# Dhia-naouali/dinov3-jax

Hardware: NVIDIA H100
Metric: global_crops_per_sec (higher is better)
Workload: dtype bf16

## Files before the change

dinov3-jax_b200/csrc/api.cu:

```cuda
#include <algorithm>
#include <atomic>
#include <cstdio>
#include <cstring>
#include "d3_internal.h"

namespace d3 {

static thread_local char g_err[512] = "";
static int g_sm_count = 0;
static std::atomic<long long> g_launches{0};
typedef CUresult (*EncodeTiledFn)(CUtensorMap*, CUtensorMapDataType, cuuint32_t, void*, const cuuint64_t*,
                                  const cuuint64_t*, const cuuint32_t*, const cuuint32_t*, CUtensorMapInterleave,
                                  CUtensorMapSwizzle, CUtensorMapL2promotion, CUtensorMapFloatOOBfill);
static EncodeTiledFn g_encode = nullptr;

int set_error(int code, const char* msg) {
  snprintf(g_err, sizeof(g_err), "%s", msg ? msg : "");
  return code;
}
int sm_count() { return g_sm_count > 0 ? g_sm_count : 132; }
void count_launch(int n) { g_launches.fetch_add(n, std::memory_order_relaxed); }

int encode_tensor_map_2d_bf16(CUtensorMap* map, const void* ptr, const cuuint64_t dims[2],
                              const cuuint64_t strides[1], const cuuint32_t box[2], const cuuint32_t estr[2]) {
// ... 69 lines not shown
    float tot = 0.f;
    for (int k = 0; k < slabs; ++k) tot += ws[k * stride + i];
    dst[r * ld + c] += tot;
  }
}
int slab_combine(const float* ws, int slabs, long long stride, long long rows, int cols, float* dst, long long ld,
                 cudaStream_t st) {
  if (!dst || rows <= 0 || cols <= 0) return D3_OK;
  const long long n = rows * cols;
  const int blocks = (int)std::min<long long>((n + 255) / 256, (long long)sm_count() * 8);
  slab_combine_kernel<<<blocks, 256, 0, st>>>(ws, slabs, stride, rows, cols, dst, ld);
  cudaError_t e = cudaPeekAtLastError();
  if (e != cudaSuccess) return set_error(D3_ERR_CUDA, cudaGetErrorString(e));
  count_launch();
  return D3_OK;
}

}

using namespace d3;

extern "C" {

int d3_abi_version(void) { return 7; }
const char* d3_last_error(void) { return g_err; }
long long d3_launch_count(void) { return g_launches.load(); }
void d3_reset_launch_count(void) { g_launches.store(0); }

int d3_init(int device) {
  cudaError_t e = cudaSetDevice(device);
  if (e != cudaSuccess) return set_error(D3_ERR_CUDA, cudaGetErrorString(e));
  cudaDeviceProp prop;
  e = cudaGetDeviceProperties(&prop, device);
  if (e != cudaSuccess) return set_error(D3_ERR_CUDA, cudaGetErrorString(e));
  if (prop.major != 9 || prop.minor != 0) {
    char buf[128];
    snprintf(buf, sizeof(buf), "device %d is sm_%d%d; this library only has sm_90a code (no fallback)", device,
             prop.major, prop.minor);
    return set_error(D3_ERR_DEVICE, buf);
  }
  g_sm_count = prop.multiProcessorCount;
  {
    cudaMemPool_t pool;
    if (cudaDeviceGetDefaultMemPool(&pool, device) == cudaSuccess) {
      uint64_t keep = UINT64_MAX;
      cudaMemPoolSetAttribute(pool, cudaMemPoolAttrReleaseThreshold, &keep);
    }
  }
  if (!g_encode) {
    void* fn = nullptr;
    cudaDriverEntryPointQueryResult q;
    e = cudaGetDriverEntryPoint("cuTensorMapEncodeTiled", &fn, cudaEnableDefault, &q);
    if (e != cudaSuccess || !fn) return set_error(D3_ERR_CUDA, "cannot resolve cuTensorMapEncodeTiled");
    g_encode = reinterpret_cast<EncodeTiledFn>(fn);
  }
  return D3_OK;
}

static int epilogue_from_abi(const d3_gemm_epilogue* ep, GemmEpilogue& g) {
  if ((ep->flags & D3_EP_ACCUM) && !(ep->flags & D3_EP_OUT_F32)) return set_error(D3_ERR_ARG, "ACCUM needs fp32 out");
  g.bias = ep->bias; g.gamma = ep->gamma; g.resid = ep->resid;
  g.aux_in = reinterpret_cast<const __nv_bfloat16*>(ep->aux_in);
  g.aux_out = reinterpret_cast<__nv_bfloat16*>(ep->aux_out);
  g.out = ep->out; g.ld_out = ep->ld_out; g.ld_aux = ep->ld_aux; g.ld_resid = ep->ld_resid;
  g.flags = ep->flags & 0x3FF; g.alpha = ep->alpha;
  for (int i = 0; i < 8; ++i) g.sc_peer[i] = ep->sc_peer[i];
  g.sc_off = ep->sc_off; g.sc_shard = ep->sc_shard; g.sc_world = ep->sc_world;
  if (g.flags & EP_SCATTER)
    for (int i = 0; i < g.sc_world && i < 8; ++i)
      if (!g.sc_peer[i]) return set_error(D3_ERR_ARG, "scatter flag without peer pointers");
  if ((g.flags & EP_BIAS) && !g.bias) return set_error(D3_ERR_ARG, "bias flag without pointer");
  if ((g.flags & EP_GAMMA) && !g.gamma) return set_error(D3_ERR_ARG, "gamma flag without pointer");
  if ((g.flags & EP_RESID) && !g.resid) return set_error(D3_ERR_ARG, "resid flag without pointer");
  if ((g.flags & EP_STORE_PRE) && !g.aux_out) return set_error(D3_ERR_ARG, "store_pre flag without pointer");
  if ((g.flags & EP_MUL_DGELU) && !g.aux_in) return set_error(D3_ERR_ARG, "mul_dgelu flag without pointer");
  return D3_OK;
}

int d3_gemm_bf16(const void* A, int lda, int a_major, const void* B, int ldb, int b_major, int M, int N, int K,
                 const d3_gemm_epilogue* ep, int tile_n, int split_k, void* stream) {
  if (!A || !B || !ep || !ep->out) return set_error(D3_ERR_ARG, "d3_gemm_bf16: null pointer");
  if (tile_n != 0 && tile_n != 64 && tile_n != 128 && tile_n != 256 && tile_n != 512) return set_error(D3_ERR_ARG, "tile_n");
  if (split_k < 0) return set_error(D3_ERR_ARG, "split_k");
  GemmEpilogue g;
  const int rc = epilogue_from_abi(ep, g);
  if (rc) return rc;
  return gemm_bf16(A, lda, a_major, B, ldb, b_major, M, N, K, g, tile_n, split_k, reinterpret_cast<cudaStream_t>(stream));
}

int d3_gemm_e4m3(const void* A_u8, int lda, const float* sa, const void* B_u8, int ldb, const float* sb, int M, int N,
                 int K, const d3_gemm_epilogue* ep, void* stream) {
  if (!A_u8 || !B_u8 || !sa || !sb || !ep || !ep->out) return set_error(D3_ERR_ARG, "d3_gemm_e4m3: null pointer");
  GemmEpilogue g;
  const int rc = epilogue_from_abi(ep, g);
  if (rc) return rc;
  return gemm_e4m3(A_u8, lda, sa, B_u8, ldb, sb, M, N, K, g, reinterpret_cast<cudaStream_t>(stream));
}

}
```

dinov3-jax_b200/csrc/attention.cu:

```cuda
#include "ptx.cuh"
#include <climits>
#include <cstdlib>
#include "d3_internal.h"

namespace d3 {

constexpr float LOG2E = 1.4426950408889634f;
constexpr int SMEM_ALIGN = 1024;

__device__ __forceinline__ uint8_t* smem_base_1024(uint8_t* raw) {
  return reinterpret_cast<uint8_t*>((reinterpret_cast<uintptr_t>(raw) + 1023) & ~uintptr_t(1023));
}

struct AttnShape {
  int G;
  int span;
  int n_crops;
  int N;
  int nkb;
  int D;
  int H;
  float scale;
  const float* sin_t;
  const float* cos_t;
  int prefix;
};

__device__ __forceinline__ uint32_t sw128_offset(int row, int col) {
  return (uint32_t)(row * 128 + ((((col >> 3) ^ (row & 7)) & 7) << 4) + (col & 7) * 2);
}

struct RowInfo { int g, klo, khi; bool ok; };
__device__ __forceinline__ RowInfo row_info(const AttnShape& sh, int c, int q) {
  RowInfo ri;
  ri.g = min(q / sh.N, sh.G - 1);
  ri.klo = ri.g * sh.N;
  ri.khi = ri.klo + sh.N;
  ri.ok = (q < sh.span) && (c * sh.G + ri.g < sh.n_crops);
  return ri;
}

template <int NI, int NO>
__device__ __forceinline__ void online_softmax(float (&s)[4 * NI], float (&o)[NO], float (&m)[2], float (&l)[2],
                                               const RowInfo (&ri)[2], int k0, int c2, float cs) {
  const int kb0 = k0 + c2;
  const bool full = k0 >= max(ri[0].klo, ri[1].klo) && k0 + 8 * NI <= min(ri[0].khi, ri[1].khi);
  float mx[2] = {-3.0e38f, -3.0e38f};
#pragma unroll
  for (int i = 0; i < NI; ++i)
#pragma unroll
    for (int j = 0; j < 4; ++j) {
      const int hh = j >> 1, kk = kb0 + 8 * i + (j & 1);
      if (full || (kk >= ri[hh].klo && kk < ri[hh].khi)) mx[hh] = fmaxf(mx[hh], s[4 * i + j]);
    }
  float corr[2], ms[2];
#pragma unroll
  for (int hh = 0; hh < 2; ++hh) {
    mx[hh] = fmaxf(mx[hh], __shfl_xor_sync(0xffffffffu, mx[hh], 1));
    mx[hh] = fmaxf(mx[hh], __shfl_xor_sync(0xffffffffu, mx[hh], 2));
    const float mn = fmaxf(m[hh], mx[hh]);
    corr[hh] = ex2_approx((m[hh] - mn) * cs);
    m[hh] = mn;
    ms[hh] = mn * cs;
    l[hh] *= corr[hh];
  }
#pragma unroll
  for (int i = 0; i < NI; ++i)
#pragma unroll
    for (int j = 0; j < 4; ++j) {
      const int hh = j >> 1, kk = kb0 + 8 * i + (j & 1);
      const float p = (full || (kk >= ri[hh].klo && kk < ri[hh].khi)) ? ex2_approx(fmaf(s[4 * i + j], cs, -ms[hh])) : 0.f;
      s[4 * i + j] = p;
      l[hh] += p;
      if (i < NO / 4) o[4 * i + j] *= corr[hh];
    }
}

template <int NO>
__device__ __forceinline__ void store_o_lse(const float (&o)[NO], float (&l)[2], const float (&m)[2], const RowInfo (&ri)[2],
                                            const AttnShape& sh, int c, int h, int row_base, int wq0, int r_in, int c2,
                                            __nv_bfloat16* O, float* LSE) {
#pragma unroll
  for (int hh = 0; hh < 2; ++hh) {
// ... 146 lines not shown
  const FwdRing ring(sQ + 16384);
  uint64_t* bar_q = ring.end();

  const int wg = threadIdx.x >> 7, t = threadIdx.x & 127;
  const int qt = blockIdx.x, h = blockIdx.y, c = blockIdx.z;
  const int q0 = qt * 128, row_base = c * sh.N, nkb = (sh.N + 127) >> 7;
  const int n_wg = (q0 + 64 < sh.N) ? 2 : 1;
  if (threadIdx.x == 0) {
    tma_prefetch_desc(&tmQKV);
    ring.init(4 * n_wg);
    mbar_init(bar_q, 1);
    fence_mbar_init();
  }
  __syncthreads();
  if (ring_producer(wg, [&] {
        mbar_expect_tx(bar_q, 16384);
        tma_load_2d(&tmQKV, bar_q, sQ, h * 64, row_base + q0);
        ring.fill(nkb, [&](uint64_t* bar, uint8_t* dst, int b) {
          tma_load_2d(&tmQKV, bar, dst, sh.D + h * 64, row_base + b * 128);
          tma_load_2d(&tmQKV, bar, dst + 16384, 2 * sh.D + h * 64, row_base + b * 128);
        });
      }))
    return;
  const int wq0 = q0 + wg * 64;
  if (wq0 >= sh.N) return;
  mbar_wait(bar_q, 0);

  const int r_in = 16 * (t >> 5) + ((t & 31) >> 2), c2 = 2 * (t & 3);
  RowInfo ri[2];
  ri[0] = row_info(sh, c, wq0 + r_in);
  ri[1] = row_info(sh, c, wq0 + r_in + 8);
  const float cs = sh.scale * LOG2E;
  float m[2] = {-3.0e38f, -3.0e38f}, l[2] = {0.f, 0.f};
  float o[32];
#pragma unroll
  for (int i = 0; i < 32; ++i) o[i] = 0.f;
  const uint64_t qd = gmma_desc_sw128(smem_u32(sQ + wg * 8192), 16, 1024);

#pragma unroll 1
  for (int b = 0; b < nkb; ++b) {
    const uint8_t* sK = ring.wait(b);
    float s[64];
    const uint64_t kd = gmma_desc_sw128(smem_u32(sK), 16, 1024);
    fence_regs(o);
    wgmma_fence();
#pragma unroll
    for (int k = 0; k < 4; ++k) wgmma_m64n128k16_ss<0, 0>(s, qd + 2 * k, kd + 2 * k, k > 0 ? 1u : 0u);
    wgmma_commit();
    wgmma_wait<0>();
    fence_regs(s);
    online_softmax<16>(s, o, m, l, ri, b * 128, c2, cs);
    uint32_t a[8][4];
#pragma unroll
    for (int kk = 0; kk < 8; ++kk)
#pragma unroll
      for (int e = 0; e < 4; ++e) a[kk][e] = pack_bf16(s[8 * kk + 2 * e], s[8 * kk + 2 * e + 1]);
    const uint64_t vd = gmma_desc_sw128(smem_u32(sK + 16384), 8192, 1024);
    fence_regs(o);
    wgmma_fence();
#pragma unroll
    for (int kk = 0; kk < 8; ++kk) wgmma_m64n64k16_rs<1>(o, a[kk], vd + 128 * kk, 1u);
    wgmma_commit();
    wgmma_wait<0>();
    fence_regs(o);
    ring.release(b);
  }
  store_o_lse(o, l, m, ri, sh, c, h, row_base, wq0, r_in, c2, O, LSE);
}

template <int HD>
__global__ void attn_delta_kernel(const __nv_bfloat16* __restrict__ O, const __nv_bfloat16* __restrict__ dO,
                                  float* __restrict__ delta, long T, int N, int D, int H) {
  constexpr int LANES = HD / 8;
  static_assert(LANES == 8 || LANES == 16, "head_dim 64 or 128");
  const long g = blockIdx.x * (long)blockDim.x + threadIdx.x;
  const int per_row = D >> 3;
  const bool ok = g < T * per_row;
  float s = 0.f;
  long row = 0;
  int c8 = 0;
  if (ok) {
    row = g / per_row;
    c8 = (int)(g % per_row);
    const uint4 a = *reinterpret_cast<const uint4*>(O + row * D + c8 * 8);
    const uint4 b = *reinterpret_cast<const uint4*>(dO + row * D + c8 * 8);
    const float2 a0 = unpack_bf16(a.x), a1 = unpack_bf16(a.y), a2 = unpack_bf16(a.z), a3 = unpack_bf16(a.w);
    const float2 b0 = unpack_bf16(b.x), b1 = unpack_bf16(b.y), b2 = unpack_bf16(b.z), b3 = unpack_bf16(b.w);
    s = a0.x * b0.x + a0.y * b0.y + a1.x * b1.x + a1.y * b1.y + a2.x * b2.x + a2.y * b2.y + a3.x * b3.x + a3.y * b3.y;
  }
  if (LANES == 16) s += __shfl_xor_sync(0xffffffffu, s, 8);
  s += __shfl_xor_sync(0xffffffffu, s, 4);
  s += __shfl_xor_sync(0xffffffffu, s, 2);
  s += __shfl_xor_sync(0xffffffffu, s, 1);
  if (ok && (c8 & (LANES - 1)) == 0) delta[((row / N) * H + (c8 >> (LANES == 16 ? 4 : 3))) * N + (row % N)] = s;
}

template <int NA>
__device__ __forceinline__ void store_grad_rows(float (&a)[NA], const AttnShape& sh, int c, int row_base, int tile_row0,
                                                int r_in, int c2, int h, int third, bool rope, __nv_bfloat16* dQKV) {
  constexpr int HD = 2 * NA;
#pragma unroll
  for (int hh = 0; hh < 2; ++hh) {
    const int row = tile_row0 + r_in + 8 * hh;
    const RowInfo ri = row_info(sh, c, row);
    if (!ri.ok) continue;
    const int tok = row - ri.klo;
    float v[NA / 2];
#pragma unroll
    for (int i = 0; i < NA / 4; ++i) { v[2 * i] = a[4 * i + 2 * hh]; v[2 * i + 1] = a[4 * i + 2 * hh + 1]; }
    if (rope && sh.sin_t && tok >= sh.prefix) {
      const float* sn = sh.sin_t + (size_t)(tok - sh.prefix) * HD;
      const float* cn = sh.cos_t + (size_t)(tok - sh.prefix) * HD;
#pragma unroll
      for (int i = 0; i < NA / 8; ++i)
#pragma unroll
        for (int j = 0; j < 2; ++j) {
          const int d = 8 * i + c2 + j;
          const float lo = v[2 * i + j], hi = v[2 * (i + NA / 8) + j];
          v[2 * i + j] = lo * cn[d] + hi * sn[d];
          v[2 * (i + NA / 8) + j] = hi * cn[d] - lo * sn[d];
        }
    }
    __nv_bfloat16* dst = dQKV + (size_t)(row_base + row) * (3 * sh.D) + third * sh.D + h * HD + c2;
#pragma unroll
    for (int i = 0; i < NA / 4; ++i) *reinterpret_cast<uint32_t*>(dst + 8 * i) = pack_bf16(v[2 * i], v[2 * i + 1]);
  }
}

__device__ __forceinline__ void row_stats(const AttnShape& sh, const float* __restrict__ LSE, const float* __restrict__ Delta,
                                          int c, int h, int q, float& lse2, float& dl) {
  const RowInfo ri = row_info(sh, c, q);
  const size_t stat = ((size_t)(c * sh.G + ri.g) * sh.H + h) * sh.N + (ri.ok ? q - ri.klo : 0);
  lse2 = ri.ok ? LSE[stat] * LOG2E : 0.f;
  dl = ri.ok ? Delta[stat] : 0.f;
}

__device__ __forceinline__ void p_ds_tile(const AttnShape& sh, const float* __restrict__ LSE, const float* __restrict__ Delta,
                                          int c, int h, int q0, int kt, const uint8_t* sQw, const uint8_t* sDOw,
                                          const uint8_t* sK, const uint8_t* sV, int r_in, int c2, float (&s)[64],
                                          float (&dp)[64]) {
  const float cs = sh.scale * LOG2E;
  const uint64_t qd = gmma_desc_sw128(smem_u32(sQw), 16, 1024);
  const uint64_t dod = gmma_desc_sw128(smem_u32(sDOw), 16, 1024);
  const uint64_t kd = gmma_desc_sw128(smem_u32(sK), 16, 1024);
  const uint64_t vd = gmma_desc_sw128(smem_u32(sV), 16, 1024);
  wgmma_fence();
#pragma unroll
  for (int k = 0; k < 4; ++k) {
    wgmma_m64n128k16_ss<0, 0>(s, qd + 2 * k, kd + 2 * k, k > 0 ? 1u : 0u);
    wgmma_m64n128k16_ss<0, 0>(dp, dod + 2 * k, vd + 2 * k, k > 0 ? 1u : 0u);
  }
  wgmma_commit();
  wgmma_wait<0>();
  fence_regs(s);
  fence_regs(dp);
#pragma unroll
  for (int hh = 0; hh < 2; ++hh) {
    const int q = q0 + r_in + 8 * hh;
    const RowInfo ri = row_info(sh, c, q);
    float lse2, dl;
    row_stats(sh, LSE, Delta, c, h, q, lse2, dl);
    const int lo = ri.ok ? ri.klo - kt * 128 : 0, hi = ri.ok ? ri.khi - kt * 128 : 0;
#pragma unroll
    for (int i = 0; i < 16; ++i)
#pragma unroll
      for (int j = 0; j < 2; ++j) {
        const int e = 4 * i + 2 * hh + j, col = 8 * i + c2 + j;
        const bool ok = col >= lo && col < hi;
        const float p = ok ? ex2_approx(fmaf(s[e], cs, -lse2)) : 0.f;
        dp[e] = ok ? (p * sh.scale) * (dp[e] - dl) : 0.f;
        s[e] = p;
      }
  }
}

__device__ __forceinline__ void stash_p_ds(const float (&s)[64], const float (&dp)[64], uint8_t* sP, uint8_t* sDS, int row,
// ... 641 lines not shown
      wgmma_fence();
#pragma unroll
      for (int kk = 0; kk < 4; ++kk) wgmma_m64n128k16_rs<1>(dq, da[kk], kd + 128 * kk, 1u);
      wgmma_commit();
      wgmma_wait<0>();
      fence_regs(dq);
      fence_frag(da);
    }
    ring.release(kt);
  }
  store_grad_rows(dq, sh, c, row_base, wq0, r_in, c2, h, 0, true, dQKV);
}

static int make_map(CUtensorMap* map, const void* ptr, long rows, int cols, int ld, int box_rows) {
  cuuint64_t dims[2] = {(cuuint64_t)cols, (cuuint64_t)rows};
  cuuint64_t strides[1] = {(cuuint64_t)ld * 2};
  cuuint32_t box[2] = {64, (cuuint32_t)box_rows};
  cuuint32_t estr[2] = {1, 1};
  return encode_tensor_map_2d_bf16(map, ptr, dims, strides, box, estr);
}

constexpr int ATTN_MAX_TOKENS = 32768;
constexpr int ATTN_FWD_RESIDENT_SPAN = 448;
constexpr int ATTN_BWD_RESIDENT_SPAN = 256;

static int attn_shape(AttnShape* s, int n_crops, int N, int D, int H) {
  if (D != H * 64 && D != H * 128) return set_error(D3_ERR_ARG, "attention: head_dim must be 64 or 128");
  if (N <= 0 || n_crops <= 0) return set_error(D3_ERR_ARG, "attention: empty problem");
  if (N > ATTN_MAX_TOKENS) return set_error(D3_ERR_ARG, "attention: N > 32768 tokens per crop");
  if ((long)n_crops * N > INT_MAX) return set_error(D3_ERR_ARG, "attention: n_crops * N must be below 2^31 token rows");
  s->N = N; s->D = D; s->H = H; s->n_crops = n_crops;
  s->scale = (D == H * 64) ? 0.125f : 0.08838834764831845f;
  s->sin_t = nullptr; s->cos_t = nullptr; s->prefix = 0;
  s->G = (N <= 64) ? (128 / N) : 1;
  if (s->G > n_crops) s->G = n_crops;
  s->span = s->G * N;
  s->nkb = (s->span + 63) / 64;
  return D3_OK;
}

static int tile_grid(const AttnShape& s, dim3* grid) {
  const int groups = (s.n_crops + s.G - 1) / s.G;
  if (s.H > 65535 || groups > 65535) return set_error(D3_ERR_ARG, "attention: H and crop groups must be <= 65535");
  *grid = dim3((s.span + 127) / 128, s.H, groups);
  return D3_OK;
}

template <auto kernel, class... Args>
static int launch(dim3 grid, int threads, int smem, int smem_max, cudaStream_t st, const Args&... args) {
  static const cudaError_t cfg = cudaFuncSetAttribute(kernel, cudaFuncAttributeMaxDynamicSharedMemorySize, smem_max);
  (void)cfg;
  kernel<<<grid, threads, smem, st>>>(args...);
  D3_CHECK_LAUNCH();
  return D3_OK;
}

}

using namespace d3;

extern "C" {

int d3_attn_fwd(const void* qkv, void* o, float* lse, int n_crops, int N, int D, int H, void* stream) {
  AttnShape s;
  int rc = attn_shape(&s, n_crops, N, D, H);
  if (rc) return rc;
  dim3 grid;
  if ((rc = tile_grid(s, &grid))) return rc;
  const long T = (long)n_crops * N;
  cudaStream_t st = reinterpret_cast<cudaStream_t>(stream);
  __nv_bfloat16* out = (__nv_bfloat16*)o;
  CUtensorMap tqkv;
  if ((rc = make_map(&tqkv, qkv, T, 3 * D, 3 * D, 128))) return rc;
  if (D == H * 128)
    return launch<attn_fwd_hd128_kernel>(grid, RING_THREADS, HD128_FWD_SMEM, HD128_FWD_SMEM, st, tqkv, out, lse, s);
  if (s.span > ATTN_FWD_RESIDENT_SPAN)
    return launch<attn_fwd_stream_kernel>(grid, RING_THREADS, FWD_STREAM_SMEM, FWD_STREAM_SMEM, st, tqkv, out, lse, s);
  CUtensorMap tkv;
  if ((rc = make_map(&tkv, qkv, T, 3 * D, 3 * D, 64))) return rc;
  return launch<attn_fwd_kernel>(grid, 256, fwd_smem(s.nkb), fwd_smem((ATTN_FWD_RESIDENT_SPAN + 63) / 64), st, tqkv, tkv,
                                 out, lse, s);
}

int d3_attn_bwd(const void* qkv, const void* o, const void* d_o, const float* lse, float* delta_scratch, void* dqkv,
                int n_crops, int N, int D, int H, const float* rope_sin, const float* rope_cos, int rope_prefix,
                void* stream) {
  AttnShape s;
  int rc = attn_shape(&s, n_crops, N, D, H);
  if (rc) return rc;
  if ((rope_sin == nullptr) != (rope_cos == nullptr)) return set_error(D3_ERR_ARG, "d3_attn_bwd: sin/cos tables");
  if (!delta_scratch) return set_error(D3_ERR_ARG, "d3_attn_bwd: delta scratch buffer");
  const bool hd128 = D == H * 128;
  const bool streamed = s.span > ATTN_BWD_RESIDENT_SPAN;
  dim3 grid;
  if ((hd128 || streamed) && (rc = tile_grid(s, &grid))) return rc;
  s.sin_t = rope_sin; s.cos_t = rope_cos; s.prefix = rope_prefix;
  const long T = (long)n_crops * N;
  cudaStream_t st = reinterpret_cast<cudaStream_t>(stream);
  const long threads = T * (D / 8);
  if (hd128)
    attn_delta_kernel<128><<<(int)((threads + 255) / 256), 256, 0, st>>>((const __nv_bfloat16*)o, (const __nv_bfloat16*)d_o,
                                                                       delta_scratch, T, N, D, H);
  else
    attn_delta_kernel<64><<<(int)((threads + 255) / 256), 256, 0, st>>>((const __nv_bfloat16*)o, (const __nv_bfloat16*)d_o,
                                                                      delta_scratch, T, N, D, H);
  D3_CHECK_LAUNCH();
  CUtensorMap tqkv, tdo;
  if ((rc = make_map(&tqkv, qkv, T, 3 * D, 3 * D, 128))) return rc;
  if ((rc = make_map(&tdo, d_o, T, D, D, 128))) return rc;
  __nv_bfloat16* dq = (__nv_bfloat16*)dqkv;
  if (hd128) {
    if ((rc = launch<attn_bwd_dkdv_hd128_kernel>(grid, RING_THREADS, HD128_BWD_SMEM, HD128_BWD_SMEM, st, tqkv, tdo, lse,
                                                 delta_scratch, dq, s)))
      return rc;
    return launch<attn_bwd_dq_hd128_kernel>(grid, RING_THREADS, HD128_BWD_SMEM, HD128_BWD_SMEM, st, tqkv, tdo, lse,
                                            delta_scratch, dq, s);
  }
  if (streamed) {
    if ((rc = launch<attn_bwd_dkdv_kernel>(grid, RING_THREADS, DKDV_SMEM, DKDV_SMEM, st, tqkv, tdo, lse, delta_scratch, dq,
                                           s)))
      return rc;
    return launch<attn_bwd_dq_kernel>(grid, RING_THREADS, DQ_SMEM, DQ_SMEM, st, tqkv, tdo, lse, delta_scratch, dq, s);
  }
  return launch<attn_bwd_fused_kernel>(dim3(H, (n_crops + s.G - 1) / s.G), 256, bwd_fused_smem((s.span + 127) / 128),
                                       bwd_fused_smem(ATTN_BWD_RESIDENT_SPAN / 128), st, tqkv, tdo, lse, delta_scratch,
                                       dq, s);
}

}
```

dinov3-jax_b200/csrc/d3_internal.h:

```cpp
#pragma once
#include <cuda.h>
#include <cuda_runtime.h>
#include <cuda_bf16.h>
#include <stdint.h>
#include "../../include/dinov3_b200.h"

namespace d3 {

enum : int {
  EP_BIAS = D3_EP_BIAS,
  EP_GELU = D3_EP_GELU,
  EP_STORE_PRE = D3_EP_STORE_PRE,
  EP_MUL_DGELU = D3_EP_MUL_DGELU,
  EP_GAMMA = D3_EP_GAMMA,
  EP_RESID = D3_EP_RESID,
  EP_OUT_F32 = D3_EP_OUT_F32,
  EP_ACCUM = D3_EP_ACCUM,
  EP_SCATTER = D3_EP_SCATTER,
  EP_GELU_ERF = D3_EP_GELU_ERF,
  EP_SLOW = 1 << 30,
  EP_SLABS = 1 << 27,
};

struct GemmEpilogue {
  const float* bias;
  const float* gamma;
  const float* resid;
  const __nv_bfloat16* aux_in;
  __nv_bfloat16* aux_out;
  void* out;
  int ld_out, ld_aux, ld_resid;
  int flags;
  float alpha;
  float* sc_peer[8];
  long long sc_off;
  int sc_shard, sc_world;
};

int set_error(int code, const char* msg);
int sm_count();
void count_launch(int n = 1);
int encode_tensor_map_2d_bf16(CUtensorMap* map, const void* ptr, const cuuint64_t dims[2],
                              const cuuint64_t strides[1], const cuuint32_t box[2], const cuuint32_t estr[2]);
int encode_tensor_map_2d(CUtensorMap* map, const void* ptr, int elt_bytes, cuuint64_t cols, cuuint64_t rows,
                         cuuint64_t row_stride_bytes, cuuint32_t box_cols, cuuint32_t box_rows, int swizzle_bytes);
int encode_tensor_map_2d_u8(CUtensorMap* map, const void* ptr, cuuint64_t cols, cuuint64_t rows, cuuint64_t ld_bytes,
                            cuuint32_t box_cols, cuuint32_t box_rows);

float* slab_workspace(size_t floats, cudaStream_t st);
void slab_release(float* ws, cudaStream_t st);
int slab_combine(const float* ws, int slabs, long long stride, long long rows, int cols, float* dst, long long ld,
                 cudaStream_t st);

int gemm_bf16(const void* A, int lda, int a_mn, const void* B, int ldb, int b_mn, int M, int N, int K,
              GemmEpilogue ep, int tile_n, int split_k, cudaStream_t stream);
int gemm_e4m3(const void* A, int lda, const float* sa, const void* B, int ldb, const float* sb, int M, int N, int K,
              GemmEpilogue ep, cudaStream_t stream);

#define D3_CHECK_LAUNCH()                                               \
  do {                                                                  \
    cudaError_t e__ = cudaPeekAtLastError();                            \
    if (e__ != cudaSuccess) return d3::set_error(D3_ERR_CUDA, cudaGetErrorString(e__)); \
    d3::count_launch();                                                 \
  } while (0)

}
```

dinov3-jax_b200/csrc/elementwise.cu:

```cuda
#include "ptx.cuh"
#include "d3_internal.h"
#include "layernorm.cuh"

namespace d3 {

__global__ void im2col_kernel(const __nv_bfloat16* __restrict__ img, __nv_bfloat16* __restrict__ out, int n, int H,
                              int W, int p, int ld) {
  const int Hp = H / p, Wp = W / p;
  const int rowlen = p * 3;
  const long total = (long)n * Hp * Wp * p;
  for (long w = blockIdx.x * (long)blockDim.x / 32 + threadIdx.x / 32; w < total; w += (long)gridDim.x * blockDim.x / 32) {
    const int a = (int)(w % p);
    long r = w / p;
    const int j = (int)(r % Wp);
    const int i = (int)((r / Wp) % Hp);
    const long c = r / ((long)Wp * Hp);
    const __nv_bfloat16* src = img + ((c * H + (long)i * p + a) * W + (long)j * p) * 3;
    __nv_bfloat16* dst = out + r * (long)ld + (long)a * rowlen;
    for (int e = threadIdx.x & 31; e < rowlen; e += 32) dst[e] = src[e];
    if (a == p - 1)
      for (int e = p * rowlen + (threadIdx.x & 31); e < ld; e += 32) out[r * (long)ld + e] = __float2bfloat16(0.f);
  }
}

__global__ void assemble_tokens_kernel(const float* __restrict__ tok, const float* __restrict__ cls,
                                       const float* __restrict__ storage, const float* __restrict__ mask_token,
                                       const uint8_t* __restrict__ masks, float* __restrict__ X, int n, int P, int R,
                                       int D) {
  const int N = P + 1 + R;
  const long rows = (long)n * N;
  const int D4 = D / 4;
  for (long r = blockIdx.x; r < rows; r += gridDim.x) {
    const long c = r / N;
    const int t = (int)(r % N);
    const float4* src;
    if (t == 0) src = reinterpret_cast<const float4*>(cls);
    else if (t <= R) src = reinterpret_cast<const float4*>(storage + (long)(t - 1) * D);
    else if (masks && masks[c * P + (t - 1 - R)]) src = reinterpret_cast<const float4*>(mask_token);
    else src = reinterpret_cast<const float4*>(tok + (c * P + (t - 1 - R)) * (long)D);
    float4* dst = reinterpret_cast<float4*>(X + r * (long)D);
    for (int e = threadIdx.x; e < D4; e += blockDim.x) dst[e] = src[e];
  }
}
__global__ void assemble_tokens_bwd_kernel(const float* __restrict__ dX, const uint8_t* __restrict__ masks,
                                           __nv_bfloat16* __restrict__ dTok, float* __restrict__ ws, int n, int P, int R,
                                           int D) {
  const int col = blockIdx.x * blockDim.x + threadIdx.x;
  const int N = P + 1 + R;
  const long slab = ((long)n + gridDim.y - 1) / gridDim.y;
  const long c0 = blockIdx.y * slab, c1 = min((long)n, c0 + slab);
  if (col >= D) return;
  float acc_cls = 0.f, acc_mask = 0.f;
  float* slab_ws = ws + (long)blockIdx.y * (2 + R) * D;
  for (int t = 1; t <= R; ++t) {
    float acc = 0.f;
    for (long c = c0; c < c1; ++c) acc += dX[c * N * (long)D + (long)t * D + col];
    slab_ws[(long)(1 + t) * D + col] = acc;
  }
  for (long c = c0; c < c1; ++c) {
    const float* row = dX + c * N * (long)D + col;
    acc_cls += row[0];
    for (int t = 0; t < P; ++t) {
      const float g = row[(long)(1 + R + t) * D];
      const bool m = masks && masks[c * P + t];
      if (m) acc_mask += g;
      dTok[(c * P + t) * (long)D + col] = __float2bfloat16(m ? 0.f : g);
    }
  }
  slab_ws[col] = acc_cls;
  slab_ws[D + col] = acc_mask;
}


template <int VPL, typename OutT>
__global__ void __launch_bounds__(256)
layernorm_fwd_kernel(const float* __restrict__ x, const float* __restrict__ scale, const float* __restrict__ bias,
                     OutT* __restrict__ y, float* __restrict__ mean_out, float* __restrict__ rstd_out, int T, float eps,
                     int width) {
  const int D = VPL > 0 ? VPL * 128 : width;
  const int warps = blockDim.x >> 5, lane = threadIdx.x & 31;
  for (long row = (long)blockIdx.x * warps + (threadIdx.x >> 5); row < T; row += (long)gridDim.x * warps) {
    const float4* xr = reinterpret_cast<const float4*>(x + row * (long)D);
    float4 v[VPL > 0 ? VPL : 1];
// ... 397 lines not shown
  }

  float* slab = reinterpret_cast<float*>(ring);
  const int ct = threadIdx.x;
#define LNR_REDUCE(ACC, DST, Q)                                                                      \
  {                                                                                                  \
    float* dst__ = (DST);                                                                            \
    asm volatile("bar.sync 1, %0;" ::"n"(32 * LNR_CONSUMERS) : "memory");                           \
    if (dst__) {                                                                                     \
      _Pragma("unroll") for (int c = 0; c < VPL; ++c)                                                \
        *reinterpret_cast<float4*>(slab + warp * D + (c * 32 + lane) * 4) =                          \
            make_float4(ACC[c][0], ACC[c][1], ACC[c][2], ACC[c][3]);                                 \
    }                                                                                                \
    asm volatile("bar.sync 1, %0;" ::"n"(32 * LNR_CONSUMERS) : "memory");                           \
    if (dst__) {                                                                                     \
      for (int e = ct; e < D; e += 32 * LNR_CONSUMERS) {                                             \
        float tot = 0.f;                                                                             \
        _Pragma("unroll") for (int w = 0; w < LNR_CONSUMERS; ++w) tot += slab[w * D + e];            \
        ws[((long)blockIdx.x * 4 + (Q)) * D + e] = tot;                                              \
      }                                                                                              \
    }                                                                                                \
  }
  LNR_REDUCE(ads, dscale, 0)
  LNR_REDUCE(adb, dscale ? dbias : nullptr, 1)
  LNR_REDUCE(tdg, (tail && uB) ? ls_dgamma : nullptr, 2)
  LNR_REDUCE(tdb, tail ? ls_dbias : nullptr, 3)
#undef LNR_REDUCE
}

__global__ void ls_gamma_from_wgrad_kernel(const __nv_bfloat16* __restrict__ W, const float* __restrict__ dW,
                                           const float* __restrict__ bias, const float* __restrict__ dbias,
                                           const float* __restrict__ gamma, float* __restrict__ ws, int K, int N) {
  __shared__ float acc[8][64];
  const int lane = threadIdx.x & 31, wy = threadIdx.x >> 5;
  const int col = blockIdx.x * 64 + lane * 2;
  const int slab = (K + gridDim.y - 1) / gridDim.y;
  const int r0 = blockIdx.y * slab, r1 = min(K, r0 + slab);
  float s0 = 0.f, s1 = 0.f;
  if (col < N) {
    for (int i = r0 + wy; i < r1; i += 8) {
      const float2 w = unpack_bf16(*reinterpret_cast<const uint32_t*>(W + (long)i * N + col));
      const float2 g = *reinterpret_cast<const float2*>(dW + (long)i * N + col);
      s0 += w.x * g.x; s1 += w.y * g.y;
    }
  }
  acc[wy][lane * 2] = s0; acc[wy][lane * 2 + 1] = s1;
  __syncthreads();
  if (threadIdx.x < 64) {
    const int c = blockIdx.x * 64 + threadIdx.x;
    if (c < N) {
      float tot = 0.f;
#pragma unroll
      for (int k = 0; k < 8; ++k) tot += acc[k][threadIdx.x];
      if (blockIdx.y == 0) tot += bias[c] * dbias[c];
      const float g = gamma[c];
      if (g != 0.f) ws[(long)blockIdx.y * N + c] = tot / g;
    }
  }
}

__global__ void rope_kernel(__nv_bfloat16* __restrict__ qkv, const float* __restrict__ sin_t,
                            const float* __restrict__ cos_t, long T, int Ntok, int prefix, int D, int hd, int inverse) {
  const int half = hd / 2;
  const int groups = half / 8;
  const int H = D / hd;
  const int items_per_row = 2 * H * groups;
  const long total = T * (long)items_per_row;
  for (long w = blockIdx.x * (long)blockDim.x + threadIdx.x; w < total; w += (long)gridDim.x * blockDim.x) {
    const long row = w / items_per_row;
    int r = (int)(w % items_per_row);
    const int t = (int)(row % Ntok);
    if (t < prefix) continue;
    const int which = r / (H * groups);
    r -= which * H * groups;
    const int head = r / groups, i0 = (r % groups) * 8;
    const float* sp = sin_t + (long)(t - prefix) * hd + i0;
    const float* cp = cos_t + (long)(t - prefix) * hd + i0;
    float sn[8], cs[8];
    *reinterpret_cast<float4*>(sn) = *reinterpret_cast<const float4*>(sp);
    *reinterpret_cast<float4*>(sn + 4) = *reinterpret_cast<const float4*>(sp + 4);
    *reinterpret_cast<float4*>(cs) = *reinterpret_cast<const float4*>(cp);
    *reinterpret_cast<float4*>(cs + 4) = *reinterpret_cast<const float4*>(cp + 4);
    __nv_bfloat16* base = qkv + row * (long)(3 * D) + which * D + head * hd + i0;
    const uint4 lo = *reinterpret_cast<const uint4*>(base);
    const uint4 hi = *reinterpret_cast<const uint4*>(base + half);
    const uint32_t lw[4] = {lo.x, lo.y, lo.z, lo.w}, hw[4] = {hi.x, hi.y, hi.z, hi.w};
    uint32_t ol[4], oh[4];
#pragma unroll
    for (int j = 0; j < 4; ++j) {
      const float2 a = unpack_bf16(lw[j]), b = unpack_bf16(hw[j]);
      float y1a, y1b, y2a, y2b;
      if (!inverse) {
        y1a = a.x * cs[2 * j] - b.x * sn[2 * j];          y2a = b.x * cs[2 * j] + a.x * sn[2 * j];
        y1b = a.y * cs[2 * j + 1] - b.y * sn[2 * j + 1];  y2b = b.y * cs[2 * j + 1] + a.y * sn[2 * j + 1];
      } else {
        y1a = a.x * cs[2 * j] + b.x * sn[2 * j];          y2a = b.x * cs[2 * j] - a.x * sn[2 * j];
        y1b = a.y * cs[2 * j + 1] + b.y * sn[2 * j + 1];  y2b = b.y * cs[2 * j + 1] - a.y * sn[2 * j + 1];
      }
      ol[j] = pack_bf16(y1a, y1b);
      oh[j] = pack_bf16(y2a, y2b);
    }
    *reinterpret_cast<uint4*>(base) = make_uint4(ol[0], ol[1], ol[2], ol[3]);
    *reinterpret_cast<uint4*>(base + half) = make_uint4(oh[0], oh[1], oh[2], oh[3]);
  }
}

__global__ void token_rows_kernel(const long long* __restrict__ idx, int* __restrict__ rows, int count, int P, int prefix,
                                  int mode) {
  const int i = blockIdx.x * blockDim.x + threadIdx.x;
  if (i >= count) return;
  if (mode == 0) {
    const long long m = idx[i];
    rows[i] = (int)(m / P * (P + prefix) + prefix + m % P);
  } else {
    rows[i] = i * (P + prefix);
  }
}
__global__ void gather_rows_kernel(const float* __restrict__ src, const int* __restrict__ rows,
                                   __nv_bfloat16* __restrict__ dst_bf16, float* __restrict__ dst_f32, int R, int D) {
  for (int r = blockIdx.x; r < R; r += gridDim.x) {
    const float* s = src + (long)rows[r] * D;
    for (int e = threadIdx.x; e < D; e += blockDim.x) {
      const float v = s[e];
      if (dst_bf16) dst_bf16[(long)r * D + e] = __float2bfloat16(v);
      if (dst_f32) dst_f32[(long)r * D + e] = v;
    }
  }
}
template <typename InT>
__global__ void scatter_add_rows_kernel(const InT* __restrict__ src, const int* __restrict__ rows,
                                        float* __restrict__ dst, int R, int D) {
  for (int r = blockIdx.x; r < R; r += gridDim.x) {
    float* d = dst + (long)rows[r] * D;
    for (int e = threadIdx.x; e < D; e += blockDim.x) {
      float v;
      if constexpr (sizeof(InT) == 2) v = __bfloat162float(src[(long)r * D + e]); else v = src[(long)r * D + e];
      d[e] += v;
    }
  }
}

__global__ void l2norm_fwd_kernel(const float* __restrict__ u, __nv_bfloat16* __restrict__ y, float* __restrict__ nrm,
                                  int R, int C, float eps) {
  const int warps = blockDim.x >> 5, lane = threadIdx.x & 31;
  for (long row = (long)blockIdx.x * warps + (threadIdx.x >> 5); row < R; row += (long)gridDim.x * warps) {
    const float* ur = u + row * C;
    float s = 0.f;
    for (int e = lane; e < C; e += 32) s += ur[e] * ur[e];
    s = warp_sum(s);
    const float n = sqrtf(s);
    const float inv = 1.f / (n + eps);
    if (lane == 0) nrm[row] = n;
    for (int e = lane; e < C; e += 32) y[row * C + e] = __float2bfloat16(ur[e] * inv);
  }
}
__global__ void l2norm_bwd_kernel(const __nv_bfloat16* __restrict__ g, const float* __restrict__ u,
                                  const float* __restrict__ nrm, __nv_bfloat16* __restrict__ du, int R, int C, float eps) {
  const int warps = blockDim.x >> 5, lane = threadIdx.x & 31;
  for (long row = (long)blockIdx.x * warps + (threadIdx.x >> 5); row < R; row += (long)gridDim.x * warps) {
    const float* ur = u + row * C;
    const __nv_bfloat16* gr = g + row * C;
    float dot = 0.f;
    for (int e = lane; e < C; e += 32) dot += ur[e] * __bfloat162float(gr[e]);
    dot = warp_sum(dot);
    const float n = nrm[row];
    const float inv = 1.f / (n + eps);
    const float coef = (n > 0.f) ? dot * inv * inv / n : 0.f;
    for (int e = lane; e < C; e += 32)
      du[row * C + e] = __float2bfloat16(__bfloat162float(gr[e]) * inv - ur[e] * coef);
  }
}

__global__ void ls_act_bwd_kernel(const float* __restrict__ dX, const __nv_bfloat16* __restrict__ u,
                                  const float* __restrict__ gamma, __nv_bfloat16* __restrict__ du,
                                  float* __restrict__ ws, int T, int D, int use_gelu) {
  const int col = (blockIdx.x * blockDim.x + threadIdx.x) * 4;
  const long slab = ((long)T + gridDim.y - 1) / gridDim.y;
  const long r0 = blockIdx.y * slab, r1 = min((long)T, r0 + slab);
  if (col >= D) return;
  float gm[4], ag[4] = {0.f, 0.f, 0.f, 0.f}, ab[4] = {0.f, 0.f, 0.f, 0.f};
  load4(gamma + col, gm);
  for (long r = r0; r < r1; ++r) {
    float o[4];
    load4(dX + r * D + col, o);
    *reinterpret_cast<uint2*>(du + r * D + col) = ls_tail4(o, gm, true, u + r * D + col, use_gelu, ag, ab);
  }
// ... 606 lines not shown
```

dinov3-jax_b200/csrc/gemm_tc.cu:

```cuda
#include <cstdlib>
#include <cstring>
#include "ptx.cuh"
#include "d3_internal.h"

namespace d3 {

constexpr int BM = 128;
constexpr int BK = 64;
constexpr int GEMM_THREADS = 384;

constexpr int EPI_RUNTIME = -1;
constexpr int EPI_FLAGS = EP_BIAS | EP_GELU | EP_STORE_PRE | EP_MUL_DGELU | EP_GAMMA | EP_RESID | EP_OUT_F32 | EP_ACCUM |
                          EP_SLABS | EP_GELU_ERF;

template <int EF>
constexpr bool kStaged = EF != EPI_RUNTIME && (EF & (EP_SLABS | EP_ACCUM)) == 0;

template <int EF>
__device__ __forceinline__ bool epi_has(const GemmEpilogue& ep, int f) {
  return EF == EPI_RUNTIME ? (ep.flags & f) != 0 : (EF & f) != 0;
}

__device__ __forceinline__ float gelu_grad_epi(float u) {
  const float u2 = __fmul_rn(u, u);
  const float t = tanh_approx(__fmul_rn(u, fmaf(0.0356774081363001f, u2, 0.7978845608028654f)));
  const float dz = fmaf(0.1070322244089003f, u2, 0.7978845608028654f);
  return fmaf(__fmul_rn(__fmul_rn(0.5f, u), fmaf(-t, t, 1.0f)), dz, __fmul_rn(0.5f, __fadd_rn(1.0f, t)));
}

__device__ __forceinline__ float gelu_erf_epi(float u) {
  return __fmul_rn(__fmul_rn(0.5f, u), __fadd_rn(1.0f, erff(__fmul_rn(u, 0.70710678118654752f))));
}

template <int EF>
__device__ __forceinline__ float epi_value(const GemmEpilogue& ep, float acc, float bias, float u, float gamma,
                                           float resid, float old, float& pre) {
  float v = __fmul_rn(acc, ep.alpha);
  if (epi_has<EF>(ep, EP_BIAS)) v = __fadd_rn(v, bias);
  pre = v;
  if (epi_has<EF>(ep, EP_GELU)) v = gelu_tanh_fast(v);
  if (epi_has<EF>(ep, EP_GELU_ERF)) v = gelu_erf_epi(v);
  if (epi_has<EF>(ep, EP_MUL_DGELU)) v = __fmul_rn(v, gelu_grad_epi(u));
  if (epi_has<EF>(ep, EP_GAMMA)) v = __fmul_rn(v, gamma);
  if (epi_has<EF>(ep, EP_RESID)) v = __fadd_rn(v, resid);
  if (epi_has<EF>(ep, EP_ACCUM)) v = __fadd_rn(v, old);
  return v;
}

__device__ __forceinline__ float2 ld_pair(const float* p, bool vec, bool two) {
  if (vec) return *reinterpret_cast<const float2*>(p);
  return make_float2(p[0], two ? p[1] : 0.f);
}
__device__ __forceinline__ float2 ld_pair(const __nv_bfloat16* p, bool vec, bool two) {
  if (vec) return unpack_bf16(*reinterpret_cast<const uint32_t*>(p));
  return make_float2(__bfloat162float(p[0]), two ? __bfloat162float(p[1]) : 0.f);
}
__device__ __forceinline__ void st_pair(float* p, float a, float b, bool vec, bool two) {
  if (vec) {
    *reinterpret_cast<float2*>(p) = make_float2(a, b);
  } else {
    p[0] = a;
    if (two) p[1] = b;
  }
}
__device__ __forceinline__ void st_pair(__nv_bfloat16* p, float a, float b, bool vec, bool two) {
  if (vec) {
    *reinterpret_cast<uint32_t*>(p) = pack_bf16(a, b);
  } else {
    p[0] = __float2bfloat16(a);
    if (two) p[1] = __float2bfloat16(b);
  }
}

template <int BN>
__device__ __forceinline__ void epilogue_tile_runtime(const GemmEpilogue& ep, float (&acc)[2][BN / 2], int m0, int n0,
                                                      int M, int N, size_t slab_row0, int r_in, int c_in) {
  float* const out_f = reinterpret_cast<float*>(ep.out);
  __nv_bfloat16* const out_h = reinterpret_cast<__nv_bfloat16*>(ep.out);
  const bool aligned = (ep.flags & EP_SLOW) == 0;
#pragma unroll
  for (int mh = 0; mh < 2; ++mh)
#pragma unroll
    for (int h = 0; h < 2; ++h) {
      const size_t row = (size_t)(m0 + mh * 64 + r_in + 8 * h);
      if (row >= (size_t)M) continue;
      const size_t orow = slab_row0 + row;
#pragma unroll
      for (int i = 0; i < BN / 8; ++i) {
        const int n = n0 + 8 * i + c_in;
        if (n >= N) break;
        const bool two = n + 1 < N, vec = aligned && two;
        float2 b{}, u{}, g{}, x{}, o{};
        if (epi_has<EPI_RUNTIME>(ep, EP_BIAS)) b = ld_pair(ep.bias + n, vec, two);
        if (epi_has<EPI_RUNTIME>(ep, EP_MUL_DGELU)) u = ld_pair(ep.aux_in + row * ep.ld_aux + n, vec, two);
        if (epi_has<EPI_RUNTIME>(ep, EP_GAMMA)) g = ld_pair(ep.gamma + n, vec, two);
        if (epi_has<EPI_RUNTIME>(ep, EP_RESID)) x = ld_pair(ep.resid + row * ep.ld_resid + n, vec, two);
        if (epi_has<EPI_RUNTIME>(ep, EP_ACCUM)) o = ld_pair(out_f + orow * ep.ld_out + n, vec, two);
        float p0, p1;
        const float v0 = epi_value<EPI_RUNTIME>(ep, acc[mh][4 * i + 2 * h], b.x, u.x, g.x, x.x, o.x, p0);
        const float v1 = epi_value<EPI_RUNTIME>(ep, acc[mh][4 * i + 2 * h + 1], b.y, u.y, g.y, x.y, o.y, p1);
        if (epi_has<EPI_RUNTIME>(ep, EP_SCATTER)) {
          const unsigned long long g_idx = (unsigned long long)ep.sc_off + orow * ep.ld_out + n;
          const unsigned long long shard = (unsigned long long)ep.sc_shard;
          const unsigned r = (unsigned)(g_idx / shard);
          float* const dst = ep.sc_peer[r] + (g_idx - r * shard);
          if (!two) atomicAdd(dst, v0);
          else atomicAdd(reinterpret_cast<float2*>(dst), make_float2(v0, v1));
          continue;
        }
        if (epi_has<EPI_RUNTIME>(ep, EP_STORE_PRE)) st_pair(ep.aux_out + row * ep.ld_aux + n, p0, p1, vec, two);
        if (epi_has<EPI_RUNTIME>(ep, EP_OUT_F32)) st_pair(out_f + orow * ep.ld_out + n, v0, v1, vec, two);
        else st_pair(out_h + orow * ep.ld_out + n, v0, v1, vec, two);
      }
    }
}

constexpr int STG_BOX = 64 * 128;
constexpr int STG_BYTES = 3 * STG_BOX;
__device__ __forceinline__ uint32_t sw128(int r, int byte) {
  return r * 128 + ((((byte >> 4) ^ r) & 7) << 4) + (byte & 15);
}

template <int MH, int BN, int EF>
__device__ __forceinline__ void epilogue_tile(const GemmEpilogue& ep, const CUtensorMap* tm_out,
                                              const CUtensorMap* tm_pre, float (&acc)[MH][BN / 2], const float* s_bias,
                                              const float* s_gamma, uint8_t* stg, int& seq, int bar, int t, int m0,
                                              int n0, int M, int N, size_t slab_row0, int r_in, int c_in) {
  constexpr bool STAGED = kStaged<EF>;
  constexpr bool F32 = (EF & EP_OUT_F32) != 0;
  constexpr int OUT_BOXES = F32 ? 2 : 1;
  constexpr int CHUNK = (OUT_BOXES + ((EF & EP_STORE_PRE) ? 1 : 0)) * STG_BOX;
  constexpr int NBUF = STG_BYTES / CHUNK;
  static_assert(NBUF >= 1, "a chunk must fit the staging area");
  float* const out_f = reinterpret_cast<float*>(ep.out);
  __nv_bfloat16* const out_h = reinterpret_cast<__nv_bfloat16*>(ep.out);
#pragma unroll
  for (int mh = 0; mh < MH; ++mh)
#pragma unroll
    for (int cb = 0; cb < BN / 64; ++cb) {
      const int row0 = m0 + mh * 64, col0 = n0 + cb * 64;
      if (row0 >= M || col0 >= N) continue;
      float2 xr[2][8], xo[2][8];
      uint32_t xu[2][8];
#pragma unroll
      for (int h = 0; h < 2; ++h) {
        const size_t row = (size_t)row0 + r_in + 8 * h;
#pragma unroll
        for (int i = 0; i < 8; ++i) {
          const int n = col0 + 8 * i + c_in;
          if (row < (size_t)M && n < N) {
            if (epi_has<EF>(ep, EP_RESID))
              xr[h][i] = *reinterpret_cast<const float2*>(ep.resid + row * ep.ld_resid + n);
            if (epi_has<EF>(ep, EP_MUL_DGELU))
              xu[h][i] = *reinterpret_cast<const uint32_t*>(ep.aux_in + row * ep.ld_aux + n);
            if (epi_has<EF>(ep, EP_ACCUM))
              xo[h][i] = *reinterpret_cast<const float2*>(out_f + (slab_row0 + row) * ep.ld_out + n);
          }
        }
      }
      uint8_t* const buf = stg + (seq % NBUF) * CHUNK;
      if constexpr (STAGED) {
        if (t == 0) tma_store_wait_read<NBUF - 1>();
        named_bar_sync(bar, 128);
      }
#pragma unroll
      for (int h = 0; h < 2; ++h) {
        const int r = r_in + 8 * h;
        const size_t row = (size_t)row0 + r;
#pragma unroll
        for (int i = 0; i < 8; ++i) {
          const int cl = cb * 64 + 8 * i + c_in;
          const int n = n0 + cl;
          const float2 b = epi_has<EF>(ep, EP_BIAS) ? *reinterpret_cast<const float2*>(s_bias + cl) : float2{};
          const float2 g = epi_has<EF>(ep, EP_GAMMA) ? *reinterpret_cast<const float2*>(s_gamma + cl) : float2{};
          const float2 u = epi_has<EF>(ep, EP_MUL_DGELU) ? unpack_bf16(xu[h][i]) : float2{};
          float p0, p1;
          const float v0 = epi_value<EF>(ep, acc[mh][4 * (cl >> 3) + 2 * h], b.x, u.x, g.x, xr[h][i].x, xo[h][i].x, p0);
          const float v1 = epi_value<EF>(ep, acc[mh][4 * (cl >> 3) + 2 * h + 1], b.y, u.y, g.y, xr[h][i].y, xo[h][i].y,
                                         p1);
          if constexpr (STAGED) {
            if (epi_has<EF>(ep, EP_STORE_PRE))
              *reinterpret_cast<uint32_t*>(buf + OUT_BOXES * STG_BOX + sw128(r, 16 * i + 2 * c_in)) = pack_bf16(p0, p1);
            if constexpr (F32) {
              *reinterpret_cast<float2*>(buf + (i >> 2) * STG_BOX + sw128(r, 32 * (i & 3) + 4 * c_in)) =
                  make_float2(v0, v1);
            } else {
              *reinterpret_cast<uint32_t*>(buf + sw128(r, 16 * i + 2 * c_in)) = pack_bf16(v0, v1);
            }
          } else if (row < (size_t)M && n < N) {
            if (epi_has<EF>(ep, EP_STORE_PRE)) st_pair(ep.aux_out + row * ep.ld_aux + n, p0, p1, true, true);
            if constexpr (F32) st_pair(out_f + (slab_row0 + row) * ep.ld_out + n, v0, v1, true, true);
            else st_pair(out_h + (slab_row0 + row) * ep.ld_out + n, v0, v1, true, true);
          }
        }
      }
      if constexpr (STAGED) {
        fence_proxy_async_smem();
        named_bar_sync(bar, 128);
        if (t == 0) {
          tma_store_2d(tm_out, buf, col0, row0);
          if (F32 && col0 + 32 < N) tma_store_2d(tm_out, buf + STG_BOX, col0 + 32, row0);
          if constexpr ((EF & EP_STORE_PRE) != 0) tma_store_2d(tm_pre, buf + OUT_BOXES * STG_BOX, col0, row0);
          tma_store_commit();
        }
        ++seq;
      }
    }
}

template <int BN, bool STAGED>
struct Cfg {
  static constexpr bool WIDE = BN == 256;
  static constexpr int STAGES = (BN == 256 ? 4 : BN == 128 ? 6 : 8) - (STAGED ? 1 : 0);
  static constexpr int A_BYTES = BM * BK * 2;
  static constexpr int B_BYTES = BN * BK * 2;
  static constexpr int STAGE_BYTES = A_BYTES + B_BYTES;
  static constexpr int BAR_BYTES = 256;
  static constexpr int VEC_BYTES = (WIDE ? 1 : 2) * 2 * BN * 4;
  static constexpr int VEC_END = STAGES * STAGE_BYTES + BAR_BYTES + VEC_BYTES;
  static constexpr int STG_OFF = (VEC_END + 1023) / 1024 * 1024;
  static constexpr int SMEM_BYTES = (STAGED ? STG_OFF + 2 * STG_BYTES : VEC_END) + 1024;
  static_assert(SMEM_BYTES <= 227 * 1024, "over the opt-in shared-memory limit");
};

struct WorkRange { int m0, n0, kb0, kb1, sp; };
template <int BN>
__device__ __forceinline__ WorkRange work_item(int w, int rank, int num_n, int num_tiles, int num_k, int splits) {
  const int tile = w % num_tiles, sp = w / num_tiles;
  const int per = (num_k + splits - 1) / splits;
  WorkRange r;
  if constexpr (BN == 256) {
    r.n0 = (tile % num_n) * BN;
    r.m0 = (2 * (tile / num_n) + rank) * BM;
  } else {
    r.n0 = (2 * (tile % num_n) + rank) * BN;
    r.m0 = (tile / num_n) * BM;
  }
  r.kb0 = sp * per;
  r.kb1 = min(num_k, r.kb0 + per);
  r.sp = sp;
  return r;
}

template <int MH, int BN, int A_MN, int B_MN>
__device__ __forceinline__ void mma_kblock(float (&acc)[MH][BN / 2], uint32_t sa, uint32_t sb, bool first) {
  const uint64_t bd = B_MN ? gmma_desc_sw128(sb, 8192, 1024) : gmma_desc_sw128(sb, 16, 1024);
  constexpr uint64_t a_adv = A_MN ? (2048 >> 4) : (32 >> 4);
  constexpr uint64_t b_adv = B_MN ? (2048 >> 4) : (32 >> 4);
#pragma unroll
  for (int k = 0; k < BK / 16; ++k) {
    const uint32_t sc = (first && k == 0) ? 0u : 1u;
#pragma unroll
    for (int mh = 0; mh < MH; ++mh) {
      const uint64_t ad = A_MN ? gmma_desc_sw128(sa + mh * 8192, 8192, 1024) : gmma_desc_sw128(sa + mh * 8192, 16, 1024);
      if constexpr (BN == 256) wgmma_m64n256k16_ss<A_MN, B_MN>(acc[mh], ad + k * a_adv, bd + k * b_adv, sc);
      else if constexpr (BN == 128) wgmma_m64n128k16_ss<A_MN, B_MN>(acc[mh], ad + k * a_adv, bd + k * b_adv, sc);
      else wgmma_m64n64k16_ss<A_MN, B_MN>(acc[mh], ad + k * a_adv, bd + k * b_adv, sc);
    }
  }
}

template <int MH, int BN>
__device__ __forceinline__ void mma_khalf_e4m3(float (&acc)[MH][BN / 2], uint32_t sa, uint32_t sb, int h) {
  static_assert(BN == 64, "the e4m3 GEMM runs 128 x 64 tiles");
  const uint64_t bd = gmma_desc_sw128(sb, 16, 1024);
#pragma unroll
  for (int k = 0; k < 2; ++k) {
#pragma unroll
    for (int mh = 0; mh < MH; ++mh) {
      const uint64_t ad = gmma_desc_sw128(sa + mh * 8192, 16, 1024);
      wgmma_m64n64k32_e4m3(acc[mh], ad + (2 * h + k) * (32 >> 4), bd + (2 * h + k) * (32 >> 4), k == 0 ? 0u : 1u);
    }
  }
}

template <int MH, int BN>
__device__ __forceinline__ void add_acc(float (&acc)[MH][BN / 2], const float (&part)[MH][BN / 2]) {
#pragma unroll
  for (int mh = 0; mh < MH; ++mh)
#pragma unroll
    for (int i = 0; i < BN / 2; ++i) acc[mh][i] = __fadd_rn(acc[mh][i], part[mh][i]);
}

template <int BN, int A_MN, int B_MN, int EF, bool E4M3 = false>
__global__ void __launch_bounds__(GEMM_THREADS, 1)
gemm_kernel(const __grid_constant__ CUtensorMap tmA, const __grid_constant__ CUtensorMap tmB,
            const __grid_constant__ CUtensorMap tmO, const __grid_constant__ CUtensorMap tmP, const GemmEpilogue ep,
            int M, int N, int K, int splits, const float* scale_a, const float* scale_b) {
  static_assert(!E4M3 || (BN == 64 && !A_MN && !B_MN), "e4m3: 128 x 64 tiles, both operands K-major");
  constexpr int KB = E4M3 ? 128 : BK;
// ... 25 lines not shown
  cluster_sync();

  const int num_m = (M + BM - 1) / BM;
  const int num_n = WIDE ? (N + BN - 1) / BN : ((N + BN - 1) / BN + 1) / 2;
  const int num_k = (K + KB - 1) / KB;
  const int num_tiles = (WIDE ? (num_m + 1) / 2 : num_m) * num_n;
  const int num_work = num_tiles * splits;

  if (wg == 0) {
    setmaxnreg_dec<40>();
    if (threadIdx.x < 32 && elect_one()) {
      int stage = 0;
      uint32_t phase = 0;
      for (int w = cluster; w < num_work; w += num_clusters) {
        const WorkRange wr = work_item<BN>(w, rank, num_n, num_tiles, num_k, splits);
        for (int kb = wr.kb0; kb < wr.kb1; ++kb) {
          mbar_wait(&empty_bar[stage], phase ^ 1);
          uint8_t* sa = smem + stage * C::STAGE_BYTES;
          uint8_t* sb = sa + C::A_BYTES;
          mbar_expect_tx(&full_bar[stage], C::STAGE_BYTES);
          if constexpr (WIDE) {
#pragma unroll
            for (int i = 0; i < 2; ++i) {
              if (A_MN) tma_load_2d(&tmA, &full_bar[stage], sa + i * 8192, wr.m0 + i * 64, kb * KB);
              else tma_load_2d(&tmA, &full_bar[stage], sa + i * 8192, kb * KB, wr.m0 + i * 64);
            }
            if (B_MN) {
#pragma unroll
              for (int i = 2 * rank; i < 2 * rank + 2; ++i)
                tma_load_2d_multicast(&tmB, &full_bar[stage], sb + i * 8192, wr.n0 + i * 64, kb * KB, 0b11);
            } else {
              tma_load_2d_multicast(&tmB, &full_bar[stage], sb + rank * 16384, kb * KB, wr.n0 + rank * 128, 0b11);
            }
          } else {
            if (A_MN) {
              tma_load_2d_multicast(&tmA, &full_bar[stage], sa + rank * 8192, wr.m0 + rank * 64, kb * KB, 0b11);
            } else {
              tma_load_2d_multicast(&tmA, &full_bar[stage], sa + rank * 8192, kb * KB, wr.m0 + rank * 64, 0b11);
            }
            if (B_MN) {
#pragma unroll
              for (int i = 0; i < BN / 64; ++i) tma_load_2d(&tmB, &full_bar[stage], sb + i * 8192, wr.n0 + i * 64, kb * KB);
            } else {
              tma_load_2d(&tmB, &full_bar[stage], sb, kb * KB, wr.n0);
            }
          }
          if (++stage == C::STAGES) { stage = 0; phase ^= 1; }
        }
      }
    }
  } else {
    setmaxnreg_inc<232>();
    const int cw = wg - 1;
    const int t = threadIdx.x & 127;
    const int r_in = 16 * (t >> 5) + ((t & 31) >> 2);
    const int c_in = 2 * (t & 3);
    float* const s_bias = vecs + (WIDE ? 0 : cw * 2 * BN);
    float* const s_gamma = s_bias + BN;
    constexpr bool stage_vecs = EF != EPI_RUNTIME && (EF & (EP_BIAS | EP_GAMMA)) != 0;
    constexpr int VEC_THREADS = WIDE ? 256 : 128;
    const int vt = WIDE ? threadIdx.x - 128 : t;
    uint8_t* const stg = smem + C::STG_OFF + cw * STG_BYTES;
    const uint32_t peer_empty = mapa_shared(smem_u32(empty_bar), rank ^ 1);
    int stg_seq = 0;
    int stage = 0;
    uint32_t phase = 0;
    int j = 0;
    for (int w = cluster; w < num_work; w += num_clusters, ++j) {
      const WorkRange wr = work_item<BN>(w, rank, num_n, num_tiles, num_k, splits);
      const int nkb = wr.kb1 > wr.kb0 ? wr.kb1 - wr.kb0 : 0;
      if (!WIDE && (j & 1) != cw) {
        stage += nkb;
        phase ^= (stage / C::STAGES) & 1;
        stage %= C::STAGES;
        continue;
      }
      if constexpr (stage_vecs) {
        named_bar_sync(3 + cw * !WIDE, VEC_THREADS);
        if (vt < BN && wr.n0 + vt < N) {
          if constexpr ((EF & EP_BIAS) != 0) cp_async_4(s_bias + vt, ep.bias + wr.n0 + vt);
          if constexpr ((EF & EP_GAMMA) != 0) cp_async_4(s_gamma + vt, ep.gamma + wr.n0 + vt);
        }
      }
      if (!WIDE && j > 0) named_bar_sync(1 + cw, 256);
      float acc[MH][BN / 2];
#pragma unroll
      for (int mh = 0; mh < MH; ++mh)
#pragma unroll
        for (int i = 0; i < BN / 2; ++i) acc[mh][i] = 0.f;
      if constexpr (E4M3) {
        float part[MH][BN / 2];
        for (int kb = wr.kb0; kb < wr.kb1; ++kb) {
          mbar_wait(&full_bar[stage], phase);
          const uint32_t sa = smem_u32(smem + stage * C::STAGE_BYTES);
#pragma unroll
          for (int h = 0; h < 2; ++h) {
#pragma unroll
            for (int mh = 0; mh < MH; ++mh) fence_regs(part[mh]);
            wgmma_fence();
            mma_khalf_e4m3<MH, BN>(part, sa, sa + C::A_BYTES, h);
            wgmma_commit();
            wgmma_wait<0>();
#pragma unroll
            for (int mh = 0; mh < MH; ++mh) fence_regs(part[mh]);
            if (h == 1 && t == 0) { mbar_arrive(&empty_bar[stage]); mbar_arrive_cluster(peer_empty + 8 * stage); }
            add_acc<MH, BN>(acc, part);
          }
          if (++stage == C::STAGES) { stage = 0; phase ^= 1; }
        }
        if (!WIDE && w + num_clusters < num_work) named_bar_arrive(1 + (cw ^ 1), 256);
#pragma unroll
        for (int mh = 0; mh < MH; ++mh)
#pragma unroll
          for (int h = 0; h < 2; ++h) {
            const int row = wr.m0 + mh * 64 + r_in + 8 * h;
            const float s_row = row < M ? scale_a[row] : 0.f;
#pragma unroll
            for (int i = 0; i < BN / 8; ++i) {
              const int n = wr.n0 + 8 * i + c_in;
              const float s0 = n < N ? scale_b[n] : 0.f, s1 = n + 1 < N ? scale_b[n + 1] : 0.f;
              acc[mh][4 * i + 2 * h] = __fmul_rn(__fmul_rn(acc[mh][4 * i + 2 * h], s_row), s0);
              acc[mh][4 * i + 2 * h + 1] = __fmul_rn(__fmul_rn(acc[mh][4 * i + 2 * h + 1], s_row), s1);
            }
          }
      } else {
        int prev = -1;
        for (int kb = wr.kb0; kb < wr.kb1; ++kb) {
          mbar_wait(&full_bar[stage], phase);
          const uint32_t sa = smem_u32(smem + stage * C::STAGE_BYTES);
#pragma unroll
          for (int mh = 0; mh < MH; ++mh) fence_regs(acc[mh]);
          wgmma_fence();
          mma_kblock<MH, BN, A_MN, B_MN>(acc, sa + (WIDE ? cw * 8192 : 0), sa + C::A_BYTES, kb == wr.kb0);
          wgmma_commit();
#pragma unroll
          for (int mh = 0; mh < MH; ++mh) fence_regs(acc[mh]);
          if (prev >= 0) {
            wgmma_wait<1>();
            if (t == 0) { mbar_arrive(&empty_bar[prev]); mbar_arrive_cluster(peer_empty + 8 * prev); }
          }
          prev = stage;
          if (++stage == C::STAGES) { stage = 0; phase ^= 1; }
        }
        if (!WIDE && w + num_clusters < num_work) named_bar_arrive(1 + (cw ^ 1), 256);
        wgmma_wait<0>();
#pragma unroll
        for (int mh = 0; mh < MH; ++mh) fence_regs(acc[mh]);
        if (prev >= 0 && t == 0) { mbar_arrive(&empty_bar[prev]); mbar_arrive_cluster(peer_empty + 8 * prev); }
      }
      if constexpr (stage_vecs) {
        cp_async_wait_all();
        named_bar_sync(3 + cw * !WIDE, VEC_THREADS);
      }
      if (nkb <= 0) continue;
      const size_t slab_row0 = epi_has<EF>(ep, EP_SLABS) ? (size_t)wr.sp * M : 0;
      if constexpr (EF == EPI_RUNTIME) {
        epilogue_tile_runtime<BN>(ep, acc, wr.m0, wr.n0, M, N, slab_row0, r_in, c_in);
      } else {
        epilogue_tile<MH, BN, EF>(ep, &tmO, &tmP, acc, s_bias, s_gamma, stg, stg_seq, 5 + cw, t,
                                  wr.m0 + (WIDE ? cw * 64 : 0), wr.n0, M, N, slab_row0, r_in, c_in);
      }
    }
    if (staged && t == 0) tma_store_wait_all();
  }
  cluster_sync();
}

static int make_operand_map(CUtensorMap* map, const void* ptr, int mn, int k, int ld, int is_mn_major, int box_mn) {
  cuuint64_t dims[2], strides[1];
  cuuint32_t box[2], estr[2] = {1, 1};
  if (is_mn_major) {
    dims[0] = (cuuint64_t)mn; dims[1] = (cuuint64_t)k; box[0] = 64; box[1] = 64;
  } else {
    dims[0] = (cuuint64_t)k; dims[1] = (cuuint64_t)mn; box[0] = 64; box[1] = (cuuint32_t)box_mn;
  }
  strides[0] = (cuuint64_t)ld * 2;
  return encode_tensor_map_2d_bf16(map, ptr, dims, strides, box, estr);
}

template <int BN, int A_MN, int B_MN, int EF, bool E4M3 = false>
static int launch(const CUtensorMap& ta, const CUtensorMap& tb, const GemmEpilogue& ep, int M, int N, int K,
                  int splits, cudaStream_t stream, const float* scale_a = nullptr, const float* scale_b = nullptr) {
  using C = Cfg<BN, kStaged<EF>>;
  auto kern = gemm_kernel<BN, A_MN, B_MN, EF, E4M3>;
  cudaLaunchAttribute attr{};
  attr.id = cudaLaunchAttributeClusterDimension;
  attr.val.clusterDim.x = 2;
  attr.val.clusterDim.y = 1;
  attr.val.clusterDim.z = 1;
  cudaLaunchConfig_t cfg{};
  cfg.blockDim = dim3(GEMM_THREADS);
  cfg.dynamicSmemBytes = C::SMEM_BYTES;
  cfg.stream = stream;
  cfg.attrs = &attr;
  cfg.numAttrs = 1;
  static int max_clusters = 0;
  if (max_clusters == 0) {
    cudaError_t e = cudaFuncSetAttribute(kern, cudaFuncAttributeMaxDynamicSharedMemorySize, C::SMEM_BYTES);
    if (e != cudaSuccess) return set_error(D3_ERR_CUDA, cudaGetErrorString(e));
    cfg.gridDim = dim3(2 * sm_count());
    e = cudaOccupancyMaxActiveClusters(&max_clusters, kern, &cfg);
    if (e != cudaSuccess) return set_error(D3_ERR_CUDA, cudaGetErrorString(e));
    if (max_clusters < 1) return set_error(D3_ERR_CUDA, "gemm: no 2-CTA cluster fits on the device");
  }
  CUtensorMap to{}, tp{};
  if constexpr (kStaged<EF>) {
    const int elt = (EF & EP_OUT_F32) ? 4 : 2;
    int rc = encode_tensor_map_2d(&to, ep.out, elt, N, M, (cuuint64_t)ep.ld_out * elt, 128 / elt, 64, 128);
    if (rc) return rc;
    if constexpr ((EF & EP_STORE_PRE) != 0) {
      rc = encode_tensor_map_2d(&tp, ep.aux_out, 2, N, M, (cuuint64_t)ep.ld_aux * 2, 64, 64, 128);
      if (rc) return rc;
    }
  }
  const int num_m = (M + BM - 1) / BM, num_n = (N + BN - 1) / BN;
  const int work = (BN == 256 ? (num_m + 1) / 2 * num_n : num_m * ((num_n + 1) / 2)) * splits;
  cfg.gridDim = dim3(2 * (work < max_clusters ? work : max_clusters));
  cudaError_t e = cudaLaunchKernelEx(&cfg, kern, ta, tb, to, tp, ep, M, N, K, splits, scale_a, scale_b);
  if (e == cudaSuccess) e = cudaPeekAtLastError();
  if (e != cudaSuccess) return set_error(D3_ERR_CUDA, cudaGetErrorString(e));
  count_launch();
  return D3_OK;
}

template <int BN>
static int dispatch(int a_mn, int b_mn, const CUtensorMap& ta, const CUtensorMap& tb, const GemmEpilogue& ep, int M,
                    int N, int K, int splits, cudaStream_t s) {
  if (!(ep.flags & (EP_SLOW | EP_SCATTER)) && N % 2 == 0) {
    const int f = ep.flags & EPI_FLAGS;
#define D3_EPI(A, B, F) \
    if (a_mn == A && b_mn == B && f == (F)) return launch<BN, A, B, (F)>(ta, tb, ep, M, N, K, splits, s);
    D3_EPI(0, 1, 0)
    D3_EPI(0, 1, EP_BIAS)
    D3_EPI(0, 1, EP_BIAS | EP_OUT_F32)
    D3_EPI(0, 1, EP_BIAS | EP_GELU)
    D3_EPI(0, 1, EP_BIAS | EP_GELU | EP_STORE_PRE)
    D3_EPI(0, 1, EP_BIAS | EP_GAMMA | EP_RESID | EP_OUT_F32)
    D3_EPI(0, 1, EP_BIAS | EP_STORE_PRE | EP_GAMMA | EP_RESID | EP_OUT_F32)
    D3_EPI(0, 1, EP_BIAS | EP_GELU | EP_GAMMA | EP_RESID | EP_OUT_F32)
    D3_EPI(0, 1, EP_BIAS | EP_GELU | EP_STORE_PRE | EP_GAMMA | EP_RESID | EP_OUT_F32)
    D3_EPI(0, 1, EP_OUT_F32)
    D3_EPI(0, 1, EP_BIAS | EP_GELU_ERF)
    D3_EPI(0, 0, 0)
    D3_EPI(0, 0, EP_MUL_DGELU)
    D3_EPI(0, 0, EP_OUT_F32)
    D3_EPI(1, 1, EP_OUT_F32 | EP_SLABS)
    D3_EPI(1, 1, EP_OUT_F32 | EP_ACCUM)
#undef D3_EPI
  }
  if constexpr (BN == 256) {
    return dispatch<128>(a_mn, b_mn, ta, tb, ep, M, N, K, splits, s);
  } else {
    if (!a_mn && !b_mn) return launch<BN, 0, 0, EPI_RUNTIME>(ta, tb, ep, M, N, K, splits, s);
    if (!a_mn && b_mn) return launch<BN, 0, 1, EPI_RUNTIME>(ta, tb, ep, M, N, K, splits, s);
    if (a_mn && !b_mn) return launch<BN, 1, 0, EPI_RUNTIME>(ta, tb, ep, M, N, K, splits, s);
    return launch<BN, 1, 1, EPI_RUNTIME>(ta, tb, ep, M, N, K, splits, s);
  }
}

int gemm_bf16(const void* A, int lda, int a_mn, const void* B, int ldb, int b_mn, int M, int N, int K,
              GemmEpilogue ep, int tile_n, int split_k, cudaStream_t stream) {
  if (M <= 0 || N <= 0 || K <= 0) return set_error(D3_ERR_ARG, "gemm: empty problem");
  if ((lda % 8) || (ldb % 8) || (reinterpret_cast<uintptr_t>(A) & 15) || (reinterpret_cast<uintptr_t>(B) & 15))
    return set_error(D3_ERR_ARG, "gemm: operands must be 16-byte aligned with ld % 8 == 0");
  const int sms = sm_count();
  const int num_k = (K + BK - 1) / BK;
  int bn = tile_n >= 256 ? 256 : tile_n;
  if (tile_n == 0) {
    const int cand[2] = {128, 64};
    long best = -1;
    for (int i = 0; i < 2; ++i) {
      const long tiles = (long)((M + BM - 1) / BM) * ((N + cand[i] - 1) / cand[i]);
      const long waves = (tiles + sms - 1) / sms;
      const long cost = waves * (cand[i] + 24);
      if (best < 0 || cost < best) { best = cost; bn = cand[i]; }
    }
  }
  const bool plain_f32 = (ep.flags & EP_OUT_F32) && !(ep.flags & (EP_BIAS | EP_GELU | EP_STORE_PRE | EP_MUL_DGELU |
                                                                  EP_GAMMA | EP_RESID | EP_GELU_ERF));
  int splits = 1;
  if (split_k >= 1) {
    splits = split_k;
  } else if (plain_f32 && (ep.flags & EP_ACCUM)) {
    const int unit_n = bn < 128 ? bn : 128;
    const long units = (long)((M + BM - 1) / BM) * ((N + unit_n - 1) / unit_n);
    if (units <= sms && num_k >= 16) {
      splits = units * 2 <= sms ? (int)(sms / units) : 1;
      if (splits < (num_k + 63) / 64) splits = (num_k + 63) / 64;
      if (splits > num_k / 4) splits = num_k / 4;
      if (splits < 1) splits = 1;
    }
  }
  if (tile_n == 0 && a_mn && b_mn) bn = 256;
  if (ep.flags & EP_SCATTER) {
    if (!plain_f32) return set_error(D3_ERR_ARG, "gemm: SCATTER needs a plain fp32 output");
    if (ep.sc_world < 1 || ep.sc_world > 8 || ep.sc_shard <= 0 || (ep.sc_shard % 4) || (ep.sc_off % 4) || (ep.ld_out % 4))
      return set_error(D3_ERR_ARG, "gemm: SCATTER needs 1..8 ranks and 4-element aligned shard / offset / ld_out");
    if ((unsigned long long)ep.sc_off + (unsigned long long)(M - 1) * ep.ld_out + N > (unsigned long long)ep.sc_shard * ep.sc_world)
      return set_error(D3_ERR_ARG, "gemm: SCATTER output exceeds the sharded range");
  }
  if (splits > 1) {
    if (!plain_f32) return set_error(D3_ERR_ARG, "gemm: split-K needs a plain fp32 output");
    if (!(ep.flags & EP_ACCUM)) return set_error(D3_ERR_ARG, "gemm: split-K accumulates into out (set ACCUM, zero it first)");
    if (splits > num_k) splits = num_k;
  }
  if (ep.flags & EP_SCATTER) ep.flags &= ~EP_ACCUM;
  const int out_elt = (ep.flags & EP_OUT_F32) ? 4 : 2;
  bool aligned = ((uintptr_t)ep.out % 16 == 0) && ((ep.ld_out * out_elt) % 16 == 0);
  if (ep.flags & EP_BIAS) aligned = aligned && ((uintptr_t)ep.bias % 16 == 0);
  if (ep.flags & EP_GAMMA) aligned = aligned && ((uintptr_t)ep.gamma % 16 == 0);
  if (ep.flags & EP_RESID) aligned = aligned && ((uintptr_t)ep.resid % 16 == 0) && (ep.ld_resid % 4 == 0);
  if (ep.flags & EP_STORE_PRE) aligned = aligned && ((uintptr_t)ep.aux_out % 16 == 0) && (ep.ld_aux % 8 == 0);
  if (ep.flags & EP_MUL_DGELU) aligned = aligned && ((uintptr_t)ep.aux_in % 16 == 0) && (ep.ld_aux % 8 == 0);
  if (!aligned) ep.flags |= EP_SLOW;

  CUtensorMap ta, tb;
  int rc = make_operand_map(&ta, A, M, K, lda, a_mn, 64);
  if (rc) return rc;
  rc = make_operand_map(&tb, B, N, K, ldb, b_mn, bn < 128 ? bn : 128);
  if (rc) return rc;
  float* ws = nullptr;
  GemmEpilogue out_ep = ep;
  if (splits > 1 && !(ep.flags & EP_SCATTER)) {
    ws = slab_workspace((size_t)splits * M * N, stream);
    if (!ws) return D3_ERR_CUDA;
    ep.out = ws;
    ep.ld_out = N;
    ep.flags = (ep.flags & ~(EP_ACCUM | EP_SLOW)) | EP_SLABS | (N % 4 ? EP_SLOW : 0);
  }
  switch (bn) {
    case 256: rc = dispatch<256>(a_mn, b_mn, ta, tb, ep, M, N, K, splits, stream); break;
    case 128: rc = dispatch<128>(a_mn, b_mn, ta, tb, ep, M, N, K, splits, stream); break;
    case 64: rc = dispatch<64>(a_mn, b_mn, ta, tb, ep, M, N, K, splits, stream); break;
    default: rc = set_error(D3_ERR_ARG, "gemm: bad tile N");
  }
  if (ws) {
    if (!rc) rc = slab_combine(ws, splits, (long long)M * N, M, N, reinterpret_cast<float*>(out_ep.out), out_ep.ld_out, stream);
    slab_release(ws, stream);
  }
  return rc;
}

static int dispatch_e4m3(const CUtensorMap& ta, const CUtensorMap& tb, const GemmEpilogue& ep, int M, int N, int K,
                         const float* sa, const float* sb, cudaStream_t s) {
  if (!(ep.flags & EP_SLOW) && N % 2 == 0) {
    const int f = ep.flags & EPI_FLAGS;
#define D3_EPI(F) \
    if (f == (F)) return launch<64, 0, 0, (F), true>(ta, tb, ep, M, N, K, 1, s, sa, sb);
    D3_EPI(0)
    D3_EPI(EP_BIAS)
    D3_EPI(EP_BIAS | EP_GELU)
    D3_EPI(EP_BIAS | EP_GELU | EP_STORE_PRE)
    D3_EPI(EP_BIAS | EP_GAMMA | EP_RESID | EP_OUT_F32)
    D3_EPI(EP_BIAS | EP_STORE_PRE | EP_GAMMA | EP_RESID | EP_OUT_F32)
    D3_EPI(EP_BIAS | EP_GELU | EP_GAMMA | EP_RESID | EP_OUT_F32)
    D3_EPI(EP_BIAS | EP_GELU | EP_STORE_PRE | EP_GAMMA | EP_RESID | EP_OUT_F32)
    D3_EPI(EP_MUL_DGELU)
    D3_EPI(EP_OUT_F32)
    D3_EPI(EP_OUT_F32 | EP_ACCUM)
#undef D3_EPI
  }
  return launch<64, 0, 0, EPI_RUNTIME, true>(ta, tb, ep, M, N, K, 1, s, sa, sb);
}

int gemm_e4m3(const void* A, int lda, const float* sa, const void* B, int ldb, const float* sb, int M, int N, int K,
              GemmEpilogue ep, cudaStream_t stream) {
  if (M <= 0 || N <= 0 || K <= 0) return set_error(D3_ERR_ARG, "gemm_e4m3: empty problem");
  if (K % 16) return set_error(D3_ERR_ARG, "gemm_e4m3: K must be a multiple of 16");
  if ((lda % 16) || (ldb % 16) || (reinterpret_cast<uintptr_t>(A) & 15) || (reinterpret_cast<uintptr_t>(B) & 15))
    return set_error(D3_ERR_ARG, "gemm_e4m3: operands must be 16-byte aligned with ld % 16 == 0");
  if (ep.flags & (EP_SCATTER | EP_GELU_ERF)) return set_error(D3_ERR_ARG, "gemm_e4m3: SCATTER / GELU_ERF not supported");
  const int out_elt = (ep.flags & EP_OUT_F32) ? 4 : 2;
  bool aligned = ((uintptr_t)ep.out % 16 == 0) && ((ep.ld_out * out_elt) % 16 == 0);
  if (ep.flags & EP_BIAS) aligned = aligned && ((uintptr_t)ep.bias % 16 == 0);
  if (ep.flags & EP_GAMMA) aligned = aligned && ((uintptr_t)ep.gamma % 16 == 0);
  if (ep.flags & EP_RESID) aligned = aligned && ((uintptr_t)ep.resid % 16 == 0) && (ep.ld_resid % 4 == 0);
  if (ep.flags & EP_STORE_PRE) aligned = aligned && ((uintptr_t)ep.aux_out % 16 == 0) && (ep.ld_aux % 8 == 0);
  if (ep.flags & EP_MUL_DGELU) aligned = aligned && ((uintptr_t)ep.aux_in % 16 == 0) && (ep.ld_aux % 8 == 0);
  if (!aligned) ep.flags |= EP_SLOW;
  CUtensorMap ta, tb;
  int rc = encode_tensor_map_2d_u8(&ta, A, K, M, lda, 128, 64);
  if (rc) return rc;
  rc = encode_tensor_map_2d_u8(&tb, B, K, N, ldb, 128, 64);
  if (rc) return rc;
  return dispatch_e4m3(ta, tb, ep, M, N, K, sa, sb, stream);
}

}
```

dinov3-jax_b200/dinov3_jax/_native.py:

```python
from __future__ import annotations

import ctypes as C
import os
from pathlib import Path

import torch

_LIB = None
_INIT_DEVICE = None

PKG_ROOT = Path(__file__).resolve().parent.parent
LIB_PATH = PKG_ROOT / "libdinov3_b200.so"

EP_BIAS, EP_GELU, EP_STORE_PRE, EP_MUL_DGELU, EP_GAMMA, EP_RESID, EP_OUT_F32, EP_ACCUM = 1, 2, 4, 8, 16, 32, 64, 128
EP_SCATTER, EP_GELU_ERF = 256, 512


class NativeError(RuntimeError):
    pass


class GemmEpilogue(C.Structure):
    _fields_ = [
        ("bias", C.c_void_p), ("gamma", C.c_void_p), ("resid", C.c_void_p), ("aux_in", C.c_void_p),
        ("aux_out", C.c_void_p), ("out", C.c_void_p),
        ("ld_out", C.c_int), ("ld_aux", C.c_int), ("ld_resid", C.c_int), ("flags", C.c_int), ("alpha", C.c_float),
        ("sc_peer", C.c_void_p * 8), ("sc_off", C.c_longlong), ("sc_shard", C.c_int), ("sc_world", C.c_int),
    ]


P, I, LL, F = C.c_void_p, C.c_int, C.c_longlong, C.c_float
SIGNATURES = {
    "d3_init": [I],
    "d3_gemm_bf16": [P, I, I, P, I, I, I, I, I, C.POINTER(GemmEpilogue), I, I, P],
    "d3_quant_rows_e4m3": [P, I, I, I, P, I, P, P],
    "d3_quant_cols_e4m3_t": [P, I, I, I, P, I, P, P],
    "d3_gemm_e4m3": [P, I, P, P, I, P, I, I, I, C.POINTER(GemmEpilogue), P],
    "d3_scatter_add_peers": [P, LL, P, I, LL, I, F, P],
    "d3_allreduce_peers": [P, I, P, LL, I, P],
    "d3_im2col": [P, P, I, I, I, I, I, P],
    "d3_assemble_tokens": [P, P, P, P, P, P, I, I, I, I, P],
    "d3_assemble_tokens_bwd": [P, P, P, P, P, P, I, I, I, I, P],
    "d3_layernorm_fwd": [P, P, P, P, I, P, P, I, I, F, P],
    "d3_layernorm_tokens_out": [P, P, P, P, P, F, I, I, I, I, I, I, P, P, P, I, I, P],
    "d3_layernorm_bwd_ls": [P, I, P, P, P, P, P, P, P, P, I, I, P, P, I, P, P, P, P],
    "d3_ls_gamma_from_wgrad": [P, P, P, P, P, P, I, I, P],
    "d3_rope": [P, P, P, LL, I, I, I, I, I, P],
    "d3_attn_fwd": [P, P, P, I, I, I, I, P],
    "d3_attn_bwd": [P, P, P, P, P, P, I, I, I, I, P, P, I, P],
    "d3_token_rows": [P, P, I, I, I, I, P],
    "d3_gather_rows": [P, P, P, P, I, I, P],
    "d3_scatter_add_rows": [P, I, P, P, I, I, P],
    "d3_l2norm_fwd": [P, P, P, I, I, F, P],
    "d3_l2norm_bwd": [P, P, P, P, I, I, F, P],
    "d3_ls_act_bwd": [P, P, P, P, P, P, I, I, I, P],
    "d3_colsum_bf16": [P, P, LL, I, I, P],
    "d3_cast_f32_bf16": [P, P, LL, P],
    "d3_swiglu_fwd": [P, P, LL, I, P],
    "d3_swiglu_bwd": [P, P, P, LL, I, P],
    "d3_absmax": [P, LL, P, P],
    "d3_colmax": [P, P, I, I, P],
    "d3_sinkhorn_colsum": [P, P, F, P, P, I, I, P],
    "d3_sinkhorn_rowsum": [P, P, F, P, P, P, I, I, P],
    "d3_sinkhorn_probs": [P, P, F, P, P, P, P, I, I, P],
    "d3_colsum_f32": [P, P, I, I, P],
    "d3_center_update": [P, P, P, F, F, P, I, P],
    "d3_ce_fwd_bwd": [P, F, P, P, F, P, P, P, P, P, P, P, P, P, P, I, I, P],
    "d3_gram_diff": [P, P, P, LL, I, F, P, I, I, P],
    "d3_resize_tokens_bicubic": [P, P, I, I, I, I, I, I, I, P],
    "d3_dwconv7_layernorm": [P, P, P, P, P, F, P, I, I, I, I, P],
    "d3_layernorm_patchify2": [P, P, P, F, P, I, I, I, I, P],
    "d3_pool_tokens": [P, P, I, I, I, I, I, P],
    "d3_resize_tokens_bilinear_aa": [P, P, I, I, I, I, I, I, I, P],
    "d3_koleo_fwd_bwd_rows": [P, P, P, P, P, P, P, I, I, I, I, F, F, F, P],
    "d3_aug_resized_crop": [P, I, I, I, P, I, P, I, P],
    "d3_aug_color": [P, P, I, I, P, P],
    "d3_aug_blur": [P, P, P, P, I, I, P],
    "d3_aug_finish": [P, P, P, I, I, C.POINTER(C.c_float), C.POINTER(C.c_float), P],
    "d3_aug_resized_crop_f32": [P, I, I, I, P, I, P, I, I, P],
    "d3_aug_color_images": [P, I, I, I, P, P, P, P],
    "d3_aug_solarize": [P, P, I, I, P],
    "d3_aug_local_windows": [P, I, I, P, P, I, I, P, P, P, P, P],
    "d3_eval_resize_crop": [P, P, I, I, I, I, C.POINTER(C.c_float), C.POINTER(C.c_float), P, I, P],
    "d3_knn_normalize": [P, I, I, I, P, P, I, P],
    "d3_topk_merge": [P, LL, I, I, I, P, P, I, I, I, P],
    "d3_knn_vote": [P, P, I, I, P, I, C.POINTER(C.c_int), I, F, I, P, P],
    "d3_train_resized_crop": [P, P, P, I, I, I, C.POINTER(C.c_float), C.POINTER(C.c_float), P, I, P],
    "d3_linear_inputs": [C.POINTER(C.c_void_p), I, I, I, P, I, P],
    "d3_linear_xent_fwd_bwd": [P, I, P, I, I, I, I, P, P, I, P],
    "d3_sumsq": [P, LL, P, P],
    "d3_ema": [P, P, P, LL, LL, F, P],
    "d3_adamw_ema": [P, P, P, P, P, P, P, LL, P, I, LL, P, F, F, F, F, F, F, F, I, F, P],
    "d3_sgd_momentum": [P, P, P, P, LL, I, P, I, F, F, I, P],
}
NO_ARG_SYMBOLS = ["d3_last_error", "d3_abi_version", "d3_launch_count", "d3_reset_launch_count"]


def lib() -> C.CDLL:
    global _LIB
    if _LIB is None:
        path = os.environ.get("DINOV3_B200_LIB", str(LIB_PATH))
        if not os.path.exists(path):
            raise NativeError(
                f"{path} not found: build it with `python __graft_entry__.py` (nvcc, sm_90a). "
                "There is no CPU / PyTorch fallback for the training hot path.")
        _LIB = C.CDLL(path)
        _LIB.d3_last_error.restype = C.c_char_p
        _LIB.d3_launch_count.restype = C.c_longlong
        for name, args in SIGNATURES.items():
            fn = getattr(_LIB, name)
            fn.argtypes = args
            fn.restype = C.c_int
    return _LIB


def check(rc: int, what: str = "") -> None:
    if rc != 0:
        raise NativeError(f"{what} failed ({rc}): {lib().d3_last_error().decode()}")


def init(device: int | None = None) -> C.CDLL:
    global _INIT_DEVICE
    l = lib()
    if not torch.cuda.is_available():
        raise NativeError("no CUDA device: the dinov3 GPU engine has no CPU fallback")
    if device is None:
        device = torch.cuda.current_device()
    if _INIT_DEVICE != device:
        check(l.d3_init(int(device)), "d3_init")
        _INIT_DEVICE = device
    return l

# ... 16 lines not shown
```

dinov3-jax_b200/dinov3_jax/engine/core.py:

```python
from __future__ import annotations

import math
import os

import torch

from .. import ops
from .config import EngineConfig
from .forward import CropSet, HeadBufs, Net, Stream, backbone_fwd, block_fwd, dgrad, head_fwd
from .forward import rope_tables
from .gram import GramAnchor
from .losses import SinkhornBufs, SmallReduce, sinkhorn, softmax_center
from .params import FrozenStore, ParamStore, backbone_spec, head_spec

f32, bf16 = torch.float32, torch.bfloat16


class Engine:

    def __init__(self, cfg: EngineConfig, B: int, device="cuda", max_masked: int | None = None, comm=None,
                 centering: str = "sinkhorn_knopp", center_momentum: float = 0.9, remat: bool = False,
                 distill: EngineConfig | None = None, fp8: bool = False):
        for c in (cfg, distill):
            if c is not None:
# ... 205 lines not shown
        ops.colsum_bf16(r(hb.dUb), gv("mlp/layers_2/bias"))
        ops.gemm(r(hb.H1), r(hb.dUb), gw("mlp/layers_2/kernel"), a_mn=True, b_mn=True, accum=True)
        ops.gemm(r(hb.dUb), w("mlp/layers_2/kernel"), r(hb.dUa), dgelu_of=r(hb.Ua))
        ops.colsum_bf16(r(hb.dUa), gv("mlp/layers_0/bias"))
        ops.gemm(r(hb.A0), r(hb.dUa), gw("mlp/layers_0/kernel"), a_mn=True, b_mn=True, accum=True)
        ops.gemm(r(hb.dUa), w("mlp/layers_0/kernel"), r(hb.dA0))
        self.fsdp.grads_ready(module, "head")

    def _ls_tail(self, i: int):
        cfg, bb, st = self.cfg, self.params.mods["backbone"], self.student
        p = f"blocks_{i}/"
        par = (i & 1) if self.wgrad_overlap else 0
        if self.wgrad_overlap and self._ev_done_live[par]:
            torch.cuda.current_stream().wait_event(self._ev_done[par])
            self._ev_done_live[par] = False
        out_bias = "mlp/w3/bias" if self.swiglu else "mlp/Dense_1/bias"
        return dict(ls_gamma=bb.vec(p + "ls2/gamma"), ls_u=st.b(st.U2, i), ls_gelu=cfg.mlp_second_act and not self.swiglu,
                    ls_du=self.dU2[par], ls_dgamma=bb.gv(p + "ls2/gamma"), ls_dbias=bb.gv(p + out_bias))

    def _block_bwd(self, i: int, dX, dXprev):
        cfg, bb, st = self.cfg, self.params.mods["backbone"], self.student
        D, H = cfg.embed_dim, cfg.heads
        p = f"blocks_{i}/"
        v, w, gw, gv = (lambda n: bb.vec(p + n)), (lambda n: bb.w(p + n)), (lambda n: bb.gw(p + n)), (lambda n: bb.gv(p + n))
        m1, r1, m2, r2 = st.b(st.stats, i)
        par = (i & 1) if self.wgrad_overlap else 0
        dU2, dU1, dP, dQKV = self.dU2[par], self.dU1[par], self.dP[par], self.dQKV[par]
        main = torch.cuda.current_stream()
        dg = lambda dy, n, out, **ep: dgrad(self.student_net, dy, w(n), out, **ep)
        if self.remat:
            block_fwd(self.student_net, st, i)
            t = self._ls_tail(i)
            ops.ls_act_bwd(dX, t["ls_u"], t["ls_gamma"], t["ls_du"], t["ls_dgamma"], t["ls_dbias"], t["ls_gelu"])

        def on_wstream(slot, fn):
            if not self.wgrad_overlap:
                fn()
                return
            ev = self._ev_in[par][slot]
            ev.record(main)
            self.wstream.wait_event(ev)
            with torch.cuda.stream(self.wstream):
                fn()

        big = ("mlp/w3/kernel", "mlp/w1/kernel", "mlp/w2/kernel", "attn/qkv/kernel") if self.swiglu else \
              ("mlp/Dense_1/kernel", "mlp/Dense_0/kernel", "attn/qkv/kernel")
        fused = big if self.fsdp.push else ()
        inv_world = 1.0 / self.fsdp.world

        def wgrad(slot, a, b, name):
            spec = self.fsdp.scatter_spec("backbone", f"blocks_{i}", p + name) if name in fused else None
            on_wstream(slot, lambda: ops.gemm(a, b, gw(name), a_mn=True, b_mn=True, accum=True, scatter=spec,
                                              alpha=inv_world if spec else 1.0))
        if self.swiglu:
            Hs = cfg.swiglu_hidden
            X12, dX12 = st.b(st.U1, i), dU1
            wgrad(0, st.b(st.Hh, i), dU2, "mlp/w3/kernel")
            dg(dU2, "mlp/w3/kernel", self.dH)
            ops.swiglu_bwd(X12, self.dH, dX12)
            wgrad(1, st.b(st.Z, i), dX12[:, :Hs], "mlp/w1/kernel")
            wgrad(1, st.b(st.Z, i), dX12[:, Hs:], "mlp/w2/kernel")
            on_wstream(1, lambda: (ops.colsum_bf16(dX12[:, :Hs], gv("mlp/w1/bias")), ops.colsum_bf16(dX12[:, Hs:], gv("mlp/w2/bias"))))
            dg(dX12[:, :Hs], "mlp/w1/kernel", self.dZ32)
            dg(dX12[:, Hs:], "mlp/w2/kernel", self.dZ32, accum=True)
            dZ = self.dZ32
        else:
            wgrad(0, st.b(st.Hh, i), dU2, "mlp/Dense_1/kernel")
            dg(dU2, "mlp/Dense_1/kernel", dU1, dgelu_of=st.b(st.U1, i))
            wgrad(1, st.b(st.Z, i), dU1, "mlp/Dense_0/kernel")
            on_wstream(1, lambda: ops.colsum_bf16(dU1, gv("mlp/Dense_0/bias")))
            dg(dU1, "mlp/Dense_0/kernel", self.dZ)
            dZ = self.dZ
        ls1 = dict(ls_u=st.b(st.Pa, i), ls_dgamma=gv("ls1/gamma")) if self.fp8 else {}
        ops.layernorm_bwd_ls(dZ, st.b(st.Xmid, i), m2, r2, v("norm2/scale"), self.dXmid, dx_add=dX,
                             dscale=gv("norm2/scale"), dbias=gv("norm2/bias"),
                             ls_gamma=v("ls1/gamma"), ls_du=dP, ls_dbias=gv("attn/proj/bias"), **ls1)

        def proj_wgrad():
            ops.gemm(st.b(st.O, i), dP, gw("attn/proj/kernel"), a_mn=True, b_mn=True, accum=True)
            if not self.fp8:
                ops.ls_gamma_from_wgrad(w("attn/proj/kernel"), gw("attn/proj/kernel"), v("attn/proj/bias"),
                                        gv("attn/proj/bias"), v("ls1/gamma"), gv("ls1/gamma"))
        on_wstream(2, proj_wgrad)
        dg(dP, "attn/proj/kernel", self.dO)
        for cs, lse, delta in zip(st.sets, st.b(st.LSE, i), self.delta):
            sl = slice(cs.row0, cs.row0 + cs.T)
            ops.attn_bwd(st.b(st.QKV, i)[sl], st.b(st.O, i)[sl], self.dO[sl], lse, delta, dQKV[sl], cs.n, cs.N, D, H,
                         rope_sin=cs.sin, rope_cos=cs.cos, rope_prefix=cfg.prefix)
        wgrad(3, st.b(st.Y, i), dQKV, "attn/qkv/kernel")

        def qkv_bias_grad():
            if cfg.mask_k_bias:
                gb = gv("attn/qkv/bias")
                ops.colsum_bf16(dQKV[:, :D], gb[:D])
                ops.colsum_bf16(dQKV[:, 2 * D:], gb[2 * D:])
            else:
                ops.colsum_bf16(dQKV, gv("attn/qkv/bias"))
        on_wstream(3, qkv_bias_grad)
        dg(dQKV, "attn/qkv/kernel", self.dY)
        tail = self._ls_tail(i - 1) if (i > 0 and not self.remat) else {}
        ops.layernorm_bwd_ls(self.dY, st.X[i], m1, r1, v("norm1/scale"), dXprev, dx_add=self.dXmid,
                             dscale=gv("norm1/scale"), dbias=gv("norm1/bias"), **tail)
        scattered = tuple(p + n for n in fused)
        if self.wgrad_overlap:
            if self.fsdp.push:
                on_wstream(0, lambda: self.fsdp.grads_ready("backbone", f"blocks_{i}", scattered=scattered))
                self._ev_done[par].record(self.wstream)
            else:
                self._ev_done[par].record(self.wstream)
                self.fsdp.grads_ready("backbone", f"blocks_{i}", also_after=self._ev_done[par])
            self._ev_done_live[par] = True
        else:
            self.fsdp.grads_ready("backbone", f"blocks_{i}", scattered=scattered)

    def _gather_schedule(self):
        items = []
        for teacher in ((False,) if self.distill is not None else (True, False)):
            bb = self.params.mods["backbone"].layout
            items += [("backbone", u, teacher) for u in bb.units]
            for m in (("dino_head", "ibot_head") if teacher else ("dino_head", "ibot_head")):
                items += [(m, u, teacher) for u in self.params.mods[m].layout.units]
        return items

    def set_batch(self, batch: dict):
        dev = self.device
        to = lambda t, dt=None: t.to(device=dev, dtype=dt, non_blocking=True)
        self.g_img = to(batch["collated_global_crops"], bf16).contiguous()
        self.l_img = to(batch["collated_local_crops"], bf16).contiguous()
        masks = batch["collated_masks"]
        self.masks_u8.copy_(masks.to(torch.uint8) if masks.dtype != torch.uint8 else masks, non_blocking=True)
        idx = batch["mask_indices_list"]
        self.M = int(idx.shape[0])
        assert self.M <= self.max_masked, f"M={self.M} exceeds max_masked={self.max_masked}"
        self.mask_idx[: self.M].copy_(idx, non_blocking=True)
        ops.token_rows(self.mask_idx, self.rows_masked_t, self.M, self.s_sets[0].P, 0, prefix=self.cfg.prefix)
        if self.distill is not None:
            ops.token_rows(self.mask_idx, self.rows_masked_tt, self.M, self.s_sets[0].P, 0, prefix=self.distill.prefix)
        if self._gram is not None:
            self._gram.set_batch(batch, self.rows_masked_t, self.M, self.masks_u8)

    def teacher_pass(self, teacher_temp: float):
        ng, M, T_ = self.cfg.n_global * self.B, self.M, self.teacher
        Dt = self.t_net.cfg.embed_dim
        backbone_fwd(self.t_net, T_, [self.g_img], [None])
        ops.gather_rows(T_.Xn, self.rows_cls_t, ng, Dt, dst_bf16=self.h_t_dino.A0)
        ops.gather_rows(T_.Xn, self.rows_masked_tt, M, Dt, dst_bf16=self.h_t_ibot.A0)
        head_fwd(self.t_net, self.h_t_dino, "dino_head", ng, stash=False)
        head_fwd(self.t_net, self.h_t_ibot, "ibot_head", M, stash=False)
        heads = [(self.h_t_dino.logits[:ng], self.sk_dino), (self.h_t_ibot.logits[:M], self.sk_ibot)]
        if self.centering == "sinkhorn_knopp":
            sinkhorn(heads, teacher_temp, 3, self.reduce)
        else:
            for (L, sk), center in zip(heads, (self.center_dino, self.center_ibot)):
                softmax_center(L, sk, center, teacher_temp, self.center_momentum, self.reduce)
        if self._gram is not None:
            self._gram.teacher_targets(T_, self.g_img, self.params.mods["backbone"])

    def forward_backward(self, teacher_temp: float):
        cfg, B, M = self.cfg, self.B, self.M
        D = cfg.embed_dim
        ng = cfg.n_global * B
        self.metrics.zero_()
        for st in self.params.mods.values():
            st.zero_grads()
        self.fsdp.begin_step()
        self.fsdp.prefetch(self._gather_schedule())
        if self.fwd_overlap:
            main = torch.cuda.current_stream()
            self._ev_fwd[0].record(main)
            self.tstream.wait_event(self._ev_fwd[0])
            with torch.cuda.stream(self.tstream):
# ... 112 lines not shown
```

dinov3-jax_b200/dinov3_jax/engine/forward.py:

```python
from __future__ import annotations

import math

import torch

from .. import ops
from .config import EngineConfig

f32, bf16, u8 = torch.float32, torch.bfloat16, torch.uint8


def rope_tables(Hp: int, Wp: int, head_dim: int, base: float, device):
    dt = torch.float64
    periods = base ** (2.0 * torch.arange(head_dim // 4, dtype=dt) / (head_dim // 2))
    ch = torch.arange(0.5, Hp, dtype=dt) / Hp
    cw = torch.arange(0.5, Wp, dtype=dt) / Wp
    coords = torch.stack(torch.meshgrid(ch, cw, indexing="ij"), dim=-1).reshape(-1, 2)
    coords = 2.0 * coords - 1.0
    ang = 2 * math.pi * coords[:, :, None] / periods[None, None, :]
    ang = ang.reshape(ang.shape[0], -1)
    ang = torch.cat([ang, ang], dim=-1)
    return (torch.sin(ang).to(f32).to(device).contiguous(), torch.cos(ang).to(f32).to(device).contiguous())


# ... 14 lines not shown

class Stream:

    def __init__(self, cfg: EngineConfig, sets, device, stash: bool, remat: bool = False, fp8: bool = False):
        D, Hd, L = cfg.embed_dim, cfg.ffn_width, cfg.depth
        swiglu = cfg.ffn_layer == "swiglu"
        self.sets = sets
        T = self.T = sum(s.T for s in sets)
        self.stash = stash
        self.per_block = stash and not remat
        nb = L if self.per_block else 1
        e = lambda *shape, dt=bf16: torch.empty(*shape, dtype=dt, device=device)
        self.X = [e(T, D, dt=f32) for _ in range(L + 1)] if stash else [e(T, D, dt=f32), e(T, D, dt=f32)]
        self.Xmid = [e(T, D, dt=f32) for _ in range(nb)]
        self.Y = [e(T, D) for _ in range(nb)]
        self.QKV = [e(T, 3 * D) for _ in range(nb)]
        self.O = [e(T, D) for _ in range(nb)]
        self.Z = [e(T, D) for _ in range(nb)]
        self.Hh = [e(T, Hd) for _ in range(nb)]
        self.Xn = e(T, D, dt=f32) if stash else self.X[(L + 1) % 2]
        self.Pa = None
        self.X12 = e(T, 2 * Hd) if (swiglu and not stash) else None
        self.LSE = [[e(s.n, cfg.heads, s.N, dt=f32) for s in sets] for _ in range(nb)]
        if stash:
            self.U1 = [e(T, 2 * Hd if swiglu else Hd) for _ in range(nb)]
            self.U2 = [e(T, D) for _ in range(nb)]
            self.Pa = [e(T, D) for _ in range(nb)] if fp8 else None
            self.stats = [[e(T, dt=f32) for _ in range(4)] for _ in range(nb)]
            self.fstats = [e(T, dt=f32), e(T, dt=f32)]

    def x_in(self, i):
        return self.X[i] if self.stash else self.X[i % 2]

    def x_out(self, i):
        return self.X[i + 1] if self.stash else self.X[(i + 1) % 2]

    def b(self, lst, i):
        return lst[i] if self.per_block else lst[0]


class HeadBufs:
    def __init__(self, cfg: EngineConfig, module: str, R: int, device, stash: bool):
        D = cfg.embed_dim
        Hh, Bn, K = cfg.head_dims(module)
        e = lambda *shape, dt=bf16: torch.empty(*shape, dtype=dt, device=device)
        self.A0 = e(R, D)
        self.H1, self.H2 = e(R, Hh), e(R, Hh)
        self.U3 = e(R, Bn, dt=f32)
        self.nrm = e(R, dt=f32)
        self.Yn = e(R, Bn)
        self.logits = e(R, K, dt=f32)
        if stash:
            self.Ua, self.Ub = e(R, Hh), e(R, Hh)
            self.dS = e(R, K)
            self.dYn, self.dU3 = e(R, Bn), e(R, Bn)
            self.dUb, self.dUa = e(R, Hh), e(R, Hh)
            self.dA0 = e(R, D, dt=f32)


class Net:

    def __init__(self, cfg: EngineConfig, mods: dict, teacher: bool, fsdp=None, fp8: bool = False):
        self.cfg, self.mods, self.teacher, self.fsdp = cfg, mods, teacher, fsdp
        self.fp8 = bool(fp8)
        self._scratch = {}

    def acquire(self, module: str, unit: str):
        if self.fsdp is not None:
            self.fsdp.acquire(module, unit, self.teacher)

    def scratch(self, key: str, shape, dtype, device):
        n = math.prod(shape)
        b = self._scratch.get(key)
        if b is None or b.numel() < n:
            b = self._scratch[key] = torch.empty(n, dtype=dtype, device=device)
        return b[:n].view(*shape)


def _e4m3_rows(net: Net, which: str, x):
    R, C = x.shape
    return ops.quant_rows(x, net.scratch("q" + which, (R, C), u8, x.device), net.scratch("s" + which, (R,), f32, x.device))


def linear(net: Net, x, W, out, **ep):
    if not net.fp8:
        return ops.gemm(x, W, out, b_mn=True, **ep)
    qx, sx = _e4m3_rows(net, "a", x)
    K, Nn = W.shape
    qw, sw = ops.quant_cols_t(W, net.scratch("qb", (Nn, K), u8, W.device), net.scratch("sb", (Nn,), f32, W.device))
    return ops.gemm_e4m3(qx, sx, qw, sw, out, **ep)


def dgrad(net: Net, dy, W, out, **ep):
    if not net.fp8:
        return ops.gemm(dy, W, out, **ep)
    qd, sd = _e4m3_rows(net, "a", dy)
    qw, sw = _e4m3_rows(net, "b", W)
    return ops.gemm_e4m3(qd, sd, qw, sw, out, **ep)


def embed(net: Net, st: Stream, images, masks_list):
    cfg, bb, teacher = net.cfg, net.mods["backbone"], net.teacher
    net.acquire("backbone", "embed")
    X0 = st.x_in(0)
    Wpe = bb.w("patch_embed/proj/kernel", teacher)
    for cs, img, masks in zip(st.sets, images, masks_list):
        tok = st.b(st.Xmid, 0)[cs.row0: cs.row0 + cs.n * cs.P]
        ops.im2col(img, cs.patches, cfg.patch)
        ops.gemm(cs.patches, Wpe, tok, b_mn=True, bias=bb.vec("patch_embed/proj/bias", teacher))
        ops.assemble_tokens(tok, bb.vec("cls_token", teacher), bb.vec("mask_token", teacher), masks,
                            X0[cs.row0: cs.row0 + cs.T], cs.n, cs.P, cfg.embed_dim,
                            storage=bb.vec("storage_tokens", teacher) if cfg.n_storage else None)


def block_fwd(net: Net, st: Stream, i: int):
    cfg, bb, teacher = net.cfg, net.mods["backbone"], net.teacher
    D, H = cfg.embed_dim, cfg.heads
    net.acquire("backbone", f"blocks_{i}")
    p = f"blocks_{i}/"
    v = lambda n: bb.vec(p + n, teacher)
    lin = lambda x, n, out, **ep: linear(net, x, bb.w(p + n, teacher), out, **ep)
    X, Xmid, Xo = st.x_in(i), st.b(st.Xmid, i), st.x_out(i)
    Y, QKV, O, Z, Hh = st.b(st.Y, i), st.b(st.QKV, i), st.b(st.O, i), st.b(st.Z, i), st.b(st.Hh, i)
    stats = st.b(st.stats, i) if st.stash else [None] * 4
    ops.layernorm_fwd(X, v("norm1/scale"), v("norm1/bias"), Y, stats[0], stats[1], cfg.ln_eps)
    lin(Y, "attn/qkv/kernel", QKV, bias=v("attn/qkv/bias") if cfg.qkv_bias else None)
    lses = st.b(st.LSE, i)
    for cs, lse in zip(st.sets, lses):
        q = QKV[cs.row0: cs.row0 + cs.T]
        ops.rope(q, cs.sin, cs.cos, cs.N, cfg.prefix, D, cfg.head_dim)
        ops.attn_fwd(q, O[cs.row0: cs.row0 + cs.T], lse if st.stash else None, cs.n, cs.N, D, H)
    lin(O, "attn/proj/kernel", Xmid, bias=v("attn/proj/bias"), gamma=v("ls1/gamma"), resid=X,
        store_pre=st.b(st.Pa, i) if st.Pa is not None else None)
    ops.layernorm_fwd(Xmid, v("norm2/scale"), v("norm2/bias"), Z, stats[2], stats[3], cfg.ln_eps)
    if cfg.ffn_layer == "swiglu":
        Hs = cfg.swiglu_hidden
        X12 = st.b(st.U1, i) if st.stash else st.X12
        lin(Z, "mlp/w1/kernel", X12[:, :Hs], bias=v("mlp/w1/bias"))
        lin(Z, "mlp/w2/kernel", X12[:, Hs:], bias=v("mlp/w2/bias"))
        ops.swiglu_fwd(X12, Hh)
        lin(Hh, "mlp/w3/kernel", Xo, bias=v("mlp/w3/bias"), store_pre=st.b(st.U2, i) if st.stash else None,
            gamma=v("ls2/gamma"), resid=Xmid)
        return
    lin(Z, "mlp/Dense_0/kernel", Hh, bias=v("mlp/Dense_0/bias"), gelu=True, store_pre=st.b(st.U1, i) if st.stash else None)
    lin(Hh, "mlp/Dense_1/kernel", Xo, bias=v("mlp/Dense_1/bias"), gelu=cfg.mlp_second_act,
        store_pre=st.b(st.U2, i) if st.stash else None, gamma=v("ls2/gamma"), resid=Xmid)


def backbone_fwd(net: Net, st: Stream, images, masks_list):
    cfg, bb, teacher = net.cfg, net.mods["backbone"], net.teacher
    embed(net, st, images, masks_list)
    for i in range(cfg.depth):
        block_fwd(net, st, i)
    XL = st.x_in(cfg.depth)
    net.acquire("backbone", "norm")
    fs = st.fstats if st.stash else [None, None]
    ops.layernorm_fwd(XL, bb.vec("norm/scale", teacher), bb.vec("norm/bias", teacher), st.Xn, fs[0], fs[1], cfg.ln_eps)


def head_fwd(net: Net, hb: HeadBufs, module: str, R: int, stash: bool):
    hd, teacher = net.mods[module], net.teacher
    w = lambda n: hd.w(n, teacher)
    v = lambda n: hd.vec(n, teacher)
    r = lambda t: t[:R]
    net.acquire(module, "head")
    if R == 0:
        return
    ops.gemm(r(hb.A0), w("mlp/layers_0/kernel"), r(hb.H1), b_mn=True, bias=v("mlp/layers_0/bias"), gelu=True,
             store_pre=r(hb.Ua) if stash else None)
    ops.gemm(r(hb.H1), w("mlp/layers_2/kernel"), r(hb.H2), b_mn=True, bias=v("mlp/layers_2/bias"), gelu=True,
             store_pre=r(hb.Ub) if stash else None)
    ops.gemm(r(hb.H2), w("mlp/layers_4/kernel"), r(hb.U3), b_mn=True, bias=v("mlp/layers_4/bias"))
    ops.l2norm_fwd(r(hb.U3), r(hb.Yn), r(hb.nrm), 1e-12)
    ops.gemm(r(hb.Yn), w("last_layer/kernel"), r(hb.logits), b_mn=True)
```

dinov3-jax_b200/dinov3_jax/ops.py:

```python
from __future__ import annotations

import ctypes as C
import math

import torch

from . import _native as N

bf16 = torch.bfloat16
f32 = torch.float32

PROFILE: list | None = None


def _ld(t: torch.Tensor) -> int:
    assert t.dim() == 2 and t.stride(1) == 1, "expect 2-D row-major (unit inner stride)"
    return t.stride(0)


def _epilogue(out, Nn, bias, gelu, gelu_erf, store_pre, dgelu_of, gamma, resid, accum, alpha, scatter):
    flags = 0
    ep = N.GemmEpilogue()
    ep.out = out.data_ptr(); ep.ld_out = _ld(out)
    if out.dtype == f32:
        flags |= N.EP_OUT_F32
    if bias is not None:
        assert bias.dtype == f32 and bias.numel() == Nn
        flags |= N.EP_BIAS; ep.bias = bias.data_ptr()
    if gelu:
        flags |= N.EP_GELU
    if gelu_erf:
        flags |= N.EP_GELU_ERF
    if store_pre is not None:
        assert store_pre.dtype == bf16 and store_pre.shape == out.shape
        flags |= N.EP_STORE_PRE; ep.aux_out = store_pre.data_ptr(); ep.ld_aux = _ld(store_pre)
    if dgelu_of is not None:
        assert dgelu_of.dtype == bf16 and dgelu_of.shape == out.shape and store_pre is None
        flags |= N.EP_MUL_DGELU; ep.aux_in = dgelu_of.data_ptr(); ep.ld_aux = _ld(dgelu_of)
    if gamma is not None:
        assert gamma.dtype == f32 and gamma.numel() == Nn
        flags |= N.EP_GAMMA; ep.gamma = gamma.data_ptr()
    if resid is not None:
        assert resid.dtype == f32 and resid.shape == out.shape
        flags |= N.EP_RESID; ep.resid = resid.data_ptr(); ep.ld_resid = _ld(resid)
    if accum:
        assert out.dtype == f32
        flags |= N.EP_ACCUM
    if scatter is not None:
        peers, sc_off, sc_shard = scatter
        assert out.dtype == f32 and out.is_contiguous() and 1 <= len(peers) <= 8
        flags |= N.EP_SCATTER
        for i, ptr in enumerate(peers):
            ep.sc_peer[i] = ptr
        ep.sc_off, ep.sc_shard, ep.sc_world = int(sc_off), int(sc_shard), len(peers)
    ep.flags = flags
    ep.alpha = float(alpha)
    return ep


def gemm(A: torch.Tensor, B: torch.Tensor, out: torch.Tensor, *, a_mn: bool = False, b_mn: bool = False,
         bias: torch.Tensor | None = None, gelu: bool = False, gelu_erf: bool = False,
         store_pre: torch.Tensor | None = None,
         dgelu_of: torch.Tensor | None = None, gamma: torch.Tensor | None = None,
         resid: torch.Tensor | None = None, accum: bool = False, alpha: float = 1.0, tile_n: int = 0,
         split_k: int = 0, scatter=None) -> torch.Tensor:
    l = N.init()
    assert A.dtype == bf16 and B.dtype == bf16
    M, K = (A.shape[1], A.shape[0]) if a_mn else (A.shape[0], A.shape[1])
    Nn, Kb = (B.shape[1], B.shape[0]) if b_mn else (B.shape[0], B.shape[1])
    assert K == Kb, f"contraction mismatch {K} vs {Kb}"
    assert out.shape[0] == M and out.shape[1] == Nn and out.dtype in (bf16, f32)
    ep = _epilogue(out, Nn, bias, gelu, gelu_erf, store_pre, dgelu_of, gamma, resid, accum, alpha, scatter)
    if PROFILE is not None:
        e0, e1 = torch.cuda.Event(enable_timing=True), torch.cuda.Event(enable_timing=True)
        e0.record()
    N.check(l.d3_gemm_bf16(N.ptr(A), _ld(A), int(a_mn), N.ptr(B), _ld(B), int(b_mn), M, Nn, K, C.byref(ep),
                           int(tile_n), int(split_k), N.stream_ptr()), "d3_gemm_bf16")
    if PROFILE is not None:
        e1.record()
        PROFILE.append(("gemm", 2.0 * M * Nn * K, e0, e1, (M, Nn, K, int(a_mn), int(b_mn))))
    return out


def quant_rows(x: torch.Tensor, q: torch.Tensor, scale: torch.Tensor):
    l = N.init()
    R, Cc = x.shape
    assert x.dtype == bf16 and q.dtype == torch.uint8 and scale.dtype == f32 and scale.is_contiguous()
    assert q.shape[0] == R and q.shape[1] >= Cc and scale.numel() == R
    N.check(l.d3_quant_rows_e4m3(N.ptr(x), _ld(x), R, Cc, N.ptr(q), _ld(q), N.ptr(scale), N.stream_ptr()),
            "d3_quant_rows_e4m3")
    return q, scale


def quant_cols_t(W: torch.Tensor, qt: torch.Tensor, scale: torch.Tensor):
    l = N.init()
    R, Cc = W.shape
    assert W.dtype == bf16 and qt.dtype == torch.uint8 and scale.dtype == f32 and scale.is_contiguous()
    assert qt.shape[0] == Cc and qt.shape[1] >= R and scale.numel() == Cc
    N.check(l.d3_quant_cols_e4m3_t(N.ptr(W), _ld(W), R, Cc, N.ptr(qt), _ld(qt), N.ptr(scale), N.stream_ptr()),
            "d3_quant_cols_e4m3_t")
    return qt, scale


def gemm_e4m3(A: torch.Tensor, sa: torch.Tensor, B: torch.Tensor, sb: torch.Tensor, out: torch.Tensor, *,
              bias: torch.Tensor | None = None, gelu: bool = False, store_pre: torch.Tensor | None = None,
              dgelu_of: torch.Tensor | None = None, gamma: torch.Tensor | None = None,
              resid: torch.Tensor | None = None, accum: bool = False, alpha: float = 1.0) -> torch.Tensor:
    l = N.init()
    assert A.dtype == torch.uint8 and B.dtype == torch.uint8 and sa.dtype == f32 and sb.dtype == f32
    M, K = A.shape
    Nn, Kb = B.shape
    assert K == Kb, f"contraction mismatch {K} vs {Kb}"
    assert sa.numel() == M and sb.numel() == Nn and sa.is_contiguous() and sb.is_contiguous()
    assert out.shape[0] == M and out.shape[1] == Nn and out.dtype in (bf16, f32)
    ep = _epilogue(out, Nn, bias, gelu, False, store_pre, dgelu_of, gamma, resid, accum, alpha, None)
    if PROFILE is not None:
        e0, e1 = torch.cuda.Event(enable_timing=True), torch.cuda.Event(enable_timing=True)
        e0.record()
    N.check(l.d3_gemm_e4m3(N.ptr(A), _ld(A), N.ptr(sa), N.ptr(B), _ld(B), N.ptr(sb), M, Nn, K, C.byref(ep),
                           N.stream_ptr()), "d3_gemm_e4m3")
    if PROFILE is not None:
        e1.record()
        PROFILE.append(("gemm_e4m3", 2.0 * M * Nn * K, e0, e1, (M, Nn, K, 0, 0)))
    return out


def _p(t):
    return None if t is None else t.data_ptr()


def _s():
    return torch.cuda.current_stream().cuda_stream


def im2col(img: torch.Tensor, out: torch.Tensor, patch: int) -> torch.Tensor:
    n, H, W, c = img.shape
    assert c == 3 and img.dtype == bf16 and img.is_contiguous() and out.dtype == bf16 and out.stride(1) == 1
    N.check(N.init().d3_im2col(_p(img), _p(out), out.stride(0), n, H, W, patch, _s()), "d3_im2col")
    return out


def assemble_tokens(tok, cls, mask_token, masks_u8, X, n, P, D, storage=None):
    assert tok.dtype == f32 and X.dtype == f32 and (masks_u8 is None or masks_u8.dtype == torch.uint8)
    R = 0 if storage is None else storage.numel() // D
    N.check(N.init().d3_assemble_tokens(_p(tok), _p(cls), _p(storage), _p(mask_token), _p(masks_u8), _p(X), n, P, R, D, _s()),
            "d3_assemble_tokens")
    return X


def assemble_tokens_bwd(dX, masks_u8, dTok, dcls, dmask, n, P, D, dstorage=None):
    assert dX.dtype == f32 and dTok.dtype == bf16 and dcls.dtype == f32
    R = 0 if dstorage is None else dstorage.numel() // D
    N.check(N.init().d3_assemble_tokens_bwd(_p(dX), _p(masks_u8), _p(dTok), _p(dcls), _p(dstorage), _p(dmask), n, P, R, D,
                                            _s()), "d3_assemble_tokens_bwd")


def layernorm_fwd(x, scale, bias, y, mean=None, rstd=None, eps=1e-6):
    T, D = x.shape
    assert x.dtype == f32 and x.is_contiguous() and y.shape == x.shape and y.is_contiguous()
    N.check(N.init().d3_layernorm_fwd(_p(x), _p(scale), _p(bias), _p(y), int(y.dtype == f32), _p(mean), _p(rstd), T, D,
# ... 34 lines not shown
    N.check(N.init().d3_scatter_add_peers(_p(src), src.numel(), arr, len(peers), int(off), int(shard), float(alpha), _s()),
            "d3_scatter_add_peers")


GRAM_MODES = {(False, False): 0, (True, False): 1, (False, True): 2}


def gram_diff(Ss, St, G, mode: int, inv_count: float, loss, block: int = 0):
    assert Ss.dtype == f32 and St.dtype == f32 and Ss.is_contiguous() and St.is_contiguous() and Ss.numel() == St.numel()
    assert G is None or (G.dtype == bf16 and G.is_contiguous() and G.numel() == Ss.numel())
    N.check(N.init().d3_gram_diff(_p(Ss), _p(St), _p(G), Ss.numel(), int(mode), float(inv_count), _p(loss), int(Ss.shape[0]),
                                  int(block), _s()), "d3_gram_diff")


def resize_tokens_bicubic(src, dst, n, Hs, Ws, Hd, Wd, D, antialias: bool):
    assert src.dtype == f32 and dst.dtype == f32 and src.is_contiguous() and dst.is_contiguous()
    assert src.numel() == n * Hs * Ws * D and dst.numel() == n * Hd * Wd * D
    N.check(N.init().d3_resize_tokens_bicubic(_p(src), _p(dst), n, Hs, Ws, Hd, Wd, D, int(bool(antialias)), _s()),
            "d3_resize_tokens_bicubic")


def dwconv7_layernorm(X, w, wb, scale, bias, Y, eps=1e-6):
    n, H, W, Cc = X.shape
    assert X.dtype == f32 and X.is_contiguous() and Y.dtype == bf16 and Y.is_contiguous() and Y.shape == (n * H * W, Cc)
    assert w.dtype == f32 and w.is_contiguous() and w.shape == (49, Cc)
    N.check(N.init().d3_dwconv7_layernorm(_p(X), _p(w), _p(wb), _p(scale), _p(bias), float(eps), _p(Y), n, H, W, Cc, _s()),
            "d3_dwconv7_layernorm")
    return Y


def layernorm_patchify2(X, scale, bias, Y, eps=1e-6):
    n, H, W, Cc = X.shape
    assert X.dtype == f32 and X.is_contiguous() and Y.dtype == bf16 and Y.is_contiguous()
    assert Y.shape == (n * (H // 2) * (W // 2), 4 * Cc)
    N.check(N.init().d3_layernorm_patchify2(_p(X), _p(scale), _p(bias), float(eps), _p(Y), n, H, W, Cc, _s()),
            "d3_layernorm_patchify2")
    return Y


def pool_tokens(X, out, copy_tokens: bool = True):
    n, P, Cc = X.shape
    assert X.dtype == f32 and X.is_contiguous() and out.dtype == f32 and out.is_contiguous()
    assert out.dim() == 3 and out.shape[0] == n and out.shape[2] == Cc
    N.check(N.init().d3_pool_tokens(_p(X), _p(out), n, P, Cc, out.shape[1], int(bool(copy_tokens)), _s()), "d3_pool_tokens")
    return out


def resize_tokens_bilinear_aa(src, dst, Hd, Wd, prefix: int = 0):
    n, Hs, Ws, Cc = src.shape
    assert src.dtype == f32 and dst.dtype == f32 and src.is_contiguous() and dst.is_contiguous()
    assert dst.shape == (n, prefix + Hd * Wd, Cc)
    N.check(N.init().d3_resize_tokens_bilinear_aa(_p(src), _p(dst), n, Hs, Ws, Hd, Wd, Cc, int(prefix), _s()),
            "d3_resize_tokens_bilinear_aa")
    return dst


def allreduce_peers(peers, out, n, op="sum"):
    assert out.dtype == f32 and out.is_contiguous() and out.numel() >= n
    arr = (C.c_void_p * len(peers))(*peers)
    N.check(N.init().d3_allreduce_peers(arr, len(peers), _p(out), int(n), {"sum": 0, "max": 1}[op], _s()), "d3_allreduce_peers")


def ls_gamma_from_wgrad(W, dW, bias, dbias, gamma, dgamma):
    K, Nn = W.shape
    assert W.dtype == bf16 and dW.dtype == f32 and W.is_contiguous() and dW.is_contiguous()
    N.check(N.init().d3_ls_gamma_from_wgrad(_p(W), _p(dW), _p(bias), _p(dbias), _p(gamma), _p(dgamma), K, Nn, _s()),
            "d3_ls_gamma_from_wgrad")


def rope(qkv, sin_t, cos_t, tokens_per_crop, prefix, D, head_dim, inverse=False):
    T = qkv.shape[0]
    assert qkv.dtype == bf16 and qkv.shape[1] == 3 * D and qkv.is_contiguous() and sin_t.dtype == f32
    N.check(N.init().d3_rope(_p(qkv), _p(sin_t), _p(cos_t), T, tokens_per_crop, prefix, D, head_dim, int(inverse),
                             _s()), "d3_rope")
    return qkv


def attn_fwd(qkv, o, lse, n_crops, Ntok, D, H):
    assert qkv.dtype == bf16 and o.dtype == bf16 and qkv.is_contiguous() and o.is_contiguous()
    N.check(N.init().d3_attn_fwd(_p(qkv), _p(o), _p(lse), n_crops, Ntok, D, H, _s()), "d3_attn_fwd")
    return o


def attn_bwd(qkv, o, do, lse, delta, dqkv, n_crops, Ntok, D, H, rope_sin=None, rope_cos=None, rope_prefix=0):
    assert all(t.dtype == bf16 and t.is_contiguous() for t in (qkv, o, do, dqkv))
    N.check(N.init().d3_attn_bwd(_p(qkv), _p(o), _p(do), _p(lse), _p(delta), _p(dqkv), n_crops, Ntok, D, H,
                                 _p(rope_sin), _p(rope_cos), rope_prefix, _s()), "d3_attn_bwd")
    return dqkv


def token_rows(mask_indices, rows, count, P, mode, prefix=1):
    assert rows.dtype == torch.int32 and (mask_indices is None or mask_indices.dtype == torch.int64)
    N.check(N.init().d3_token_rows(_p(mask_indices), _p(rows), count, P, prefix, mode, _s()), "d3_token_rows")
    return rows


def gather_rows(src, rows, R, D, dst_bf16=None, dst_f32=None):
    assert src.dtype == f32 and rows.dtype == torch.int32
    N.check(N.init().d3_gather_rows(_p(src), _p(rows), _p(dst_bf16), _p(dst_f32), R, D, _s()), "d3_gather_rows")


def scatter_add_rows(src, rows, dst, R, D):
    assert dst.dtype == f32
    N.check(N.init().d3_scatter_add_rows(_p(src), int(src.dtype == f32), _p(rows), _p(dst), R, D, _s()),
            "d3_scatter_add_rows")


def l2norm_fwd(u, y, nrm, eps=1e-12):
    R, Cc = u.shape
    assert u.dtype == f32 and y.dtype == bf16
    N.check(N.init().d3_l2norm_fwd(_p(u), _p(y), _p(nrm), R, Cc, eps, _s()), "d3_l2norm_fwd")
    return y


def l2norm_bwd(g, u, nrm, du, eps=1e-12):
    R, Cc = u.shape
    assert g.dtype == bf16 and du.dtype == bf16
    N.check(N.init().d3_l2norm_bwd(_p(g), _p(u), _p(nrm), _p(du), R, Cc, eps, _s()), "d3_l2norm_bwd")
    return du


def ls_act_bwd(dX, u, gamma, du, dgamma, dbias, use_gelu: bool):
    T, D = dX.shape
    assert dX.dtype == f32 and u.dtype == bf16 and du.dtype == bf16
    N.check(N.init().d3_ls_act_bwd(_p(dX), _p(u), _p(gamma), _p(du), _p(dgamma), _p(dbias), T, D, int(use_gelu), _s()),
            "d3_ls_act_bwd")


def colsum_bf16(x, out):
    T, Nn = x.shape
    assert x.dtype == bf16 and out.dtype == f32
    N.check(N.init().d3_colsum_bf16(_p(x), _p(out), T, Nn, x.stride(0), _s()), "d3_colsum_bf16")


def cast_f32_bf16(src, dst):
    assert src.dtype == f32 and dst.dtype == bf16 and src.numel() == dst.numel()
    N.check(N.init().d3_cast_f32_bf16(_p(src), _p(dst), src.numel(), _s()), "d3_cast_f32_bf16")


def absmax(L, out):
    N.check(N.init().d3_absmax(_p(L), L.numel(), _p(out), _s()), "d3_absmax")


def colmax(L, cm):
    R, K = L.shape
    N.check(N.init().d3_colmax(_p(L), _p(cm), R, K, _s()), "d3_colmax")


def sinkhorn_colsum(L, mx, temp, a, s):
    R, K = L.shape
    N.check(N.init().d3_sinkhorn_colsum(_p(L), _p(mx), temp, _p(a), _p(s), R, K, _s()), "d3_sinkhorn_colsum")


def sinkhorn_rowsum(L, mx, temp, s, btot, a):
    R, K = L.shape
    N.check(N.init().d3_sinkhorn_rowsum(_p(L), _p(mx), temp, _p(s), _p(btot), _p(a), R, K, _s()), "d3_sinkhorn_rowsum")


def sinkhorn_probs(L, mx, temp, s, a, btot, Q):
    R, K = L.shape
    N.check(N.init().d3_sinkhorn_probs(_p(L), _p(mx), temp, _p(s), _p(a), _p(btot), _p(Q), R, K, _s()),
            "d3_sinkhorn_probs")


def colsum_f32(L, out):
    R, K = L.shape
    N.check(N.init().d3_colsum_f32(_p(L), _p(out), R, K, _s()), "d3_colsum_f32")


def center_update(center, colsum, total_rows, momentum, temp, s_out):
    N.check(N.init().d3_center_update(_p(center), _p(colsum), _p(total_rows), momentum, temp, _p(s_out), center.numel(), _s()),
# ... 156 lines not shown
```

include/dinov3_b200.h:

```cpp
#ifndef DINOV3_B200_H
#define DINOV3_B200_H
#ifdef __cplusplus
extern "C" {
#endif

typedef enum {
  D3_OK = 0,
  D3_ERR_ARG = -1,
  D3_ERR_CUDA = -2,
  D3_ERR_DEVICE = -3,
} d3_status;

int d3_init(int device);
const char* d3_last_error(void);
int d3_abi_version(void);
long long d3_launch_count(void);
void d3_reset_launch_count(void);

enum {
  D3_EP_BIAS = 1,
  D3_EP_GELU = 2,
  D3_EP_STORE_PRE = 4,
  D3_EP_MUL_DGELU = 8,
  D3_EP_GAMMA = 16,
  D3_EP_RESID = 32,
  D3_EP_OUT_F32 = 64,
  D3_EP_ACCUM = 128,
  D3_EP_SCATTER = 256,
  D3_EP_GELU_ERF = 512,
};
typedef struct {
  const float* bias;
  const float* gamma;
  const float* resid;
  const void* aux_in;
  void* aux_out;
  void* out;
  int ld_out, ld_aux, ld_resid;
  int flags;
  float alpha;
  float* sc_peer[8];
  long long sc_off;
  int sc_shard, sc_world;
} d3_gemm_epilogue;
int d3_gemm_bf16(const void* A, int lda, int a_major, const void* B, int ldb, int b_major, int M, int N, int K,
                 const d3_gemm_epilogue* ep, int tile_n, int split_k, void* stream);

int d3_quant_rows_e4m3(const void* src_bf16, int ld, int R, int C, void* dst_u8, int ld_dst, float* scale,
                       void* stream);
int d3_quant_cols_e4m3_t(const void* src_bf16, int ld, int R, int C, void* dst_u8, int ld_dst, float* scale,
                         void* stream);
int d3_gemm_e4m3(const void* A_u8, int lda, const float* sa, const void* B_u8, int ldb, const float* sb, int M, int N,
                 int K, const d3_gemm_epilogue* ep, void* stream);

int d3_im2col(const void* img_bf16 , void* out_bf16 ,
              int ld_out, int n, int H, int W, int p, void* stream);
int d3_assemble_tokens(const float* tok , const float* cls , const float* storage ,
                       const float* mask_token , const unsigned char* masks ,
                       float* X , int n, int P, int R, int D, void* stream);
int d3_assemble_tokens_bwd(const float* dX, const unsigned char* masks, void* dTok_bf16 ,
                           float* dcls , float* dstorage , float* dmask_token ,
                           int n, int P, int R, int D, void* stream);

int d3_layernorm_fwd(const float* x , const float* scale, const float* bias, void* y, int y_is_f32,
                     float* mean , float* rstd, int T, int D, float eps, void* stream);
int d3_layernorm_tokens_out(const float* X, const float* scale, const float* bias, const float* pre_scale,
                            const float* pre_bias, float eps, int n, int N, int R, int Hp, int Wp, int D, void* cls,
                            void* storage, void* patches, int out_f32, int channels_first, void* stream);
int d3_layernorm_bwd_ls(const void* dy, int dy_is_f32, const float* x, const float* mean, const float* rstd,
                        const float* scale, const float* dx_add , float* dx,
                        float* dscale , float* dbias , int T, int D,
                        const float* ls_gamma , const void* ls_u_bf16 , int ls_gelu,
                        void* ls_du_bf16 , float* ls_dgamma , float* ls_dbias ,
                        void* stream);
int d3_ls_gamma_from_wgrad(const void* W_bf16, const float* dW, const float* bias, const float* dbias,
                           const float* gamma, float* dgamma, int K, int N, void* stream);

int d3_scatter_add_peers(const float* src, long long n, float* const* peers , int world,
                         long long off, int shard, float alpha, void* stream);

int d3_allreduce_peers(const float* const* peers , int world, float* out, long long n, int op,
                       void* stream);

int d3_rope(void* qkv_bf16, const float* sin_t , const float* cos_t, long long T, int tokens_per_crop,
            int prefix, int D, int head_dim, int inverse, void* stream);

int d3_attn_fwd(const void* qkv_bf16 , void* o_bf16 , float* lse ,
                int n_crops, int N, int D, int H, void* stream);
int d3_attn_bwd(const void* qkv_bf16, const void* o_bf16, const void* do_bf16, const float* lse,
                float* delta_scratch , void* dqkv_bf16 , int n_crops, int N, int D, int H,
                const float* rope_sin, const float* rope_cos, int rope_prefix, void* stream);

int d3_token_rows(const long long* mask_indices , int* rows , int count,
                  int P, int prefix ,
                  int mode , void* stream);
int d3_gather_rows(const float* src , const int* rows, void* dst_bf16 , float* dst_f32 ,
                   int R, int D, void* stream);
int d3_scatter_add_rows(const void* src, int src_is_f32, const int* rows, float* dst , int R, int D, void* stream);

int d3_l2norm_fwd(const float* u , void* y_bf16, float* nrm , int R, int C, float eps, void* stream);
int d3_l2norm_bwd(const void* g_bf16, const float* u, const float* nrm, void* du_bf16, int R, int C, float eps,
                  void* stream);

int d3_ls_act_bwd(const float* dX , const void* u_bf16, const float* gamma, void* du_bf16, float* dgamma,
                  float* dbias, int T, int D, int use_gelu, void* stream);
int d3_colsum_bf16(const void* x_bf16 , float* out , long long T, int N, int ld,
                   void* stream);
int d3_cast_f32_bf16(const float* src, void* dst_bf16, long long n, void* stream);

int d3_swiglu_fwd(const void* x12_bf16 , void* h_bf16 , long long T, int Hs, void* stream);
int d3_swiglu_bwd(const void* x12_bf16, const void* dh_bf16 , void* dx12_bf16 , long long T, int Hs,
                  void* stream);

int d3_absmax(const float* L, long long n, float* out , void* stream);
int d3_colmax(const float* L , float* cm , int R, int K, void* stream);
int d3_sinkhorn_colsum(const float* L , const float* mx, float temp, const float* a ,
                       float* s , int R, int K, void* stream);
int d3_sinkhorn_rowsum(const float* L, const float* mx, float temp, const float* s, const float* btot ,
                       float* a , int R, int K, void* stream);
int d3_sinkhorn_probs(const float* L, const float* mx, float temp, const float* s, const float* a, const float* btot,
                      float* Q , int R, int K, void* stream);

int d3_colsum_f32(const float* L , float* out , int R, int K, void* stream);
int d3_center_update(float* center , const float* colsum , const float* total_rows ,
                     float momentum, float temp, float* s_out , int K, void* stream);

int d3_ce_fwd_bwd(const float* S , float student_temp, const float* Lt ,
                  const float* mx, float teacher_temp, const float* s_t , const float* a_t ,
                  const float* btot, const int* t0, const int* t1, const float* wm, const float* wg, const int* slot,
                  float* metric, void* dS_bf16, int Rs, int K, void* stream);

int d3_gram_diff(const float* Ss, const float* St, void* G_bf16, long long n_elems, int mode, float inv_count, float* loss,
                 int n, int block, void* stream);

int d3_resize_tokens_bicubic(const float* src, float* dst, int n, int Hs, int Ws, int Hd, int Wd, int D, int antialias,
                             void* stream);

int d3_dwconv7_layernorm(const float* X, const float* w, const float* wb, const float* scale, const float* bias, float eps,
                         void* Y_bf16, int n, int H, int W, int C, void* stream);
int d3_layernorm_patchify2(const float* X, const float* scale, const float* bias, float eps, void* Y_bf16, int n, int H,
                           int W, int C, void* stream);
int d3_pool_tokens(const float* X, float* out, int n, int P, int C, int rows, int copy_tokens, void* stream);
int d3_resize_tokens_bilinear_aa(const float* src, float* dst, int n, int Hs, int Ws, int Hd, int Wd, int C, int prefix,
                                 void* stream);

int d3_koleo_fwd_bwd_rows(const float* x , float* xn_scratch , float* nrm_scratch ,
                          int* nn_scratch , float* coef_scratch , float* metric, float* dx ,
                          int B, int D, int row0, int nrows, float eps, float w_metric, float w_grad, void* stream);

int d3_sumsq(const float* g, long long n, float* out , void* stream);
int d3_adamw_ema(float* p, const float* g, float* m, float* v, float* teacher, void* p_bf16, void* t_bf16,
                 long long n_bf16, const void* segs, int nseg, long long n, const float* sumsq ,
                 float max_norm, float lr, float last_layer_lr, float wd, float b1, float b2, float eps, int step,
                 float momentum, void* stream);
int d3_ema(float* teacher, const float* student, void* t_bf16, long long n_bf16, long long n, float momentum,
           void* stream);

int d3_aug_resized_crop(const void* src_u8 , int n_img, int H, int W, const void* crops ,
                        int n_crops, float* out , int S, void* stream);
int d3_aug_color(float* x , const void* crops, int n_crops, int S,
                 float* gray_sum , void* stream);
int d3_aug_blur(const float* x, float* tmp, float* y, const void* blur ,
                int n_crops, int S, void* stream);
int d3_aug_finish(const float* x, void* out_bf16 , const void* crops, int n_crops, int S,
                  const float* mean3 , const float* std3 , void* stream);
int d3_aug_resized_crop_f32(const float* src , int n_img, int H, int W, const void* crops,
                            int n_crops, float* out , int S, int clamp, void* stream);
int d3_aug_color_images(const void* src_u8 , int n_img, int H, int W, const void* recs ,
                        float* x , float* gray_sum , void* stream);
int d3_aug_solarize(float* x , const void* crops, int n_crops, int S, void* stream);
int d3_aug_local_windows(const float* base , int n_base, int M, const void* crops, const void* blur,
                         int n_crops, int L, float* win, float* tmp, float* y ,
                         float* gray_sum , void* stream);

// ... 22 lines not shown
```

Measured before the change: 543.3.

## Fuse RoPE into QKV GEMM epilogue and attention delta into dO GEMM

Adds an attention-aware GEMM epilogue that applies rotary embedding to Q/K columns directly after the QKV projection, and computes the backward delta (rowsum of O·dO) in the epilogue of the dgrad GEMM producing dO. This removes the separate rope and delta kernels and their extra read/write passes over QKV and O/dO. In exchange the GEMM epilogue carries more registers and prefetched sin/cos and O tiles, which can reduce occupancy or add epilogue latency. It also adds split API entry points for backward with a precomputed delta.

Result: no change. 548.2 (median of 6 runs) (+0.9%).

```diff
diff --git a/dinov3-jax_b200/csrc/api.cu b/dinov3-jax_b200/csrc/api.cu
--- a/dinov3-jax_b200/csrc/api.cu
+++ b/dinov3-jax_b200/csrc/api.cu
@@ -175,16 +175,51 @@
   if (!A || !B || !ep || !ep->out) return set_error(D3_ERR_ARG, "d3_gemm_bf16: null pointer");
   if (tile_n != 0 && tile_n != 64 && tile_n != 128 && tile_n != 256 && tile_n != 512) return set_error(D3_ERR_ARG, "tile_n");
   if (split_k < 0) return set_error(D3_ERR_ARG, "split_k");
-  GemmEpilogue g;
+  GemmEpilogue g{};
   const int rc = epilogue_from_abi(ep, g);
   if (rc) return rc;
   return gemm_bf16(A, lda, a_major, B, ldb, b_major, M, N, K, g, tile_n, split_k, reinterpret_cast<cudaStream_t>(stream));
 }
 
+int d3_gemm_bf16_attn(const void* A, int lda, int a_major, const void* B, int ldb, int b_major, int M, int N, int K,
+                      const d3_gemm_epilogue* ep, const d3_attn_epilogue* at, int tile_n, void* stream) {
+  if (!A || !B || !ep || !ep->out || !at) return set_error(D3_ERR_ARG, "d3_gemm_bf16_attn: null pointer");
+  if (tile_n != 0 && tile_n != 64 && tile_n != 128 && tile_n != 256 && tile_n != 512) return set_error(D3_ERR_ARG, "tile_n");
+  GemmEpilogue g{};
+  int rc = epilogue_from_abi(ep, g);
+  if (rc) return rc;
+  const bool rope = at->op == D3_ATTN_ROPE;
+  if (!rope && at->op != D3_ATTN_DELTA) return set_error(D3_ERR_ARG, "d3_gemm_bf16_attn: op");
+  if (at->D <= 0 || at->head_dim <= 0 || at->D % at->head_dim)
+    return set_error(D3_ERR_ARG, "d3_gemm_bf16_attn: D must be a multiple of head_dim");
+  const int width = rope ? 3 * at->D : at->D;
+  if (N != width || ep->ld_out != width || (g.flags & (EP_OUT_F32 | EP_ACCUM | EP_SCATTER)))
+    return set_error(D3_ERR_ARG, "d3_gemm_bf16_attn: out must be contiguous bf16 [M, 3D] (ROPE) / [M, D] (DELTA)");
+  if (!rope && !at->o) return set_error(D3_ERR_ARG, "d3_gemm_bf16_attn: DELTA without O");
+  if (reinterpret_cast<uintptr_t>(ep->out) % 16 || reinterpret_cast<uintptr_t>(at->o) % 16)
+    return set_error(D3_ERR_ARG, "d3_gemm_bf16_attn: out and O must be 16-byte aligned");
+  if (rope && (at->prefix < 0)) return set_error(D3_ERR_ARG, "d3_gemm_bf16_attn: prefix");
+  if (at->n_sets < 1 || at->n_sets > ATTN_EPI_SETS) return set_error(D3_ERR_ARG, "d3_gemm_bf16_attn: 1 to 4 crop sets");
+  AttnEpilogue& a = g.at;
+  a.op = at->op; a.n_sets = at->n_sets; a.D = at->D; a.H = at->D / at->head_dim; a.head_dim = at->head_dim;
+  a.prefix = at->prefix; a.o = reinterpret_cast<const __nv_bfloat16*>(at->o);
+  for (int s = 0; s < at->n_sets; ++s) {
+    const d3_crop_set& cs = at->sets[s];
+    if (cs.n_crops < 1 || cs.tokens_per_crop < 1 || cs.row0 < 0 ||
+        (long long)cs.n_crops * cs.tokens_per_crop > M - cs.row0)
+      return set_error(D3_ERR_ARG, "d3_gemm_bf16_attn: crop set outside the output rows");
+    if (rope && (!cs.sin_t || !cs.cos_t || at->prefix >= cs.tokens_per_crop))
+      return set_error(D3_ERR_ARG, "d3_gemm_bf16_attn: ROPE set without sin / cos tables or patch tokens");
+    if (!rope && !cs.delta) return set_error(D3_ERR_ARG, "d3_gemm_bf16_attn: DELTA set without its delta buffer");
+    a.set[s] = {cs.row0, cs.n_crops * cs.tokens_per_crop, cs.tokens_per_crop, cs.sin_t, cs.cos_t, cs.delta};
+  }
+  return gemm_bf16(A, lda, a_major, B, ldb, b_major, M, N, K, g, tile_n, 1, reinterpret_cast<cudaStream_t>(stream));
+}
+
 int d3_gemm_e4m3(const void* A_u8, int lda, const float* sa, const void* B_u8, int ldb, const float* sb, int M, int N,
                  int K, const d3_gemm_epilogue* ep, void* stream) {
   if (!A_u8 || !B_u8 || !sa || !sb || !ep || !ep->out) return set_error(D3_ERR_ARG, "d3_gemm_e4m3: null pointer");
-  GemmEpilogue g;
+  GemmEpilogue g{};
   const int rc = epilogue_from_abi(ep, g);
   if (rc) return rc;
   return gemm_e4m3(A_u8, lda, sa, B_u8, ldb, sb, M, N, K, g, reinterpret_cast<cudaStream_t>(stream));
diff --git a/dinov3-jax_b200/csrc/attention.cu b/dinov3-jax_b200/csrc/attention.cu
--- a/dinov3-jax_b200/csrc/attention.cu
+++ b/dinov3-jax_b200/csrc/attention.cu
@@ -1,4 +1,5 @@
 #include "ptx.cuh"
+#include "attn_epi.cuh"
 #include <climits>
 #include <cstdlib>
 #include "d3_internal.h"
@@ -311,16 +312,10 @@
   if (ok) {
     row = g / per_row;
     c8 = (int)(g % per_row);
-    const uint4 a = *reinterpret_cast<const uint4*>(O + row * D + c8 * 8);
-    const uint4 b = *reinterpret_cast<const uint4*>(dO + row * D + c8 * 8);
-    const float2 a0 = unpack_bf16(a.x), a1 = unpack_bf16(a.y), a2 = unpack_bf16(a.z), a3 = unpack_bf16(a.w);
-    const float2 b0 = unpack_bf16(b.x), b1 = unpack_bf16(b.y), b2 = unpack_bf16(b.z), b3 = unpack_bf16(b.w);
-    s = a0.x * b0.x + a0.y * b0.y + a1.x * b1.x + a1.y * b1.y + a2.x * b2.x + a2.y * b2.y + a3.x * b3.x + a3.y * b3.y;
-  }
-  if (LANES == 16) s += __shfl_xor_sync(0xffffffffu, s, 8);
-  s += __shfl_xor_sync(0xffffffffu, s, 4);
-  s += __shfl_xor_sync(0xffffffffu, s, 2);
-  s += __shfl_xor_sync(0xffffffffu, s, 1);
+    s = delta_dot8(*reinterpret_cast<const uint4*>(O + row * D + c8 * 8),
+                   *reinterpret_cast<const uint4*>(dO + row * D + c8 * 8));
+  }
+  s = delta_lane_sum<LANES>(s);
   if (ok && (c8 & (LANES - 1)) == 0) delta[((row / N) * H + (c8 >> (LANES == 16 ? 4 : 3))) * N + (row % N)] = s;
 }
 
@@ -1128,6 +1123,24 @@
                                  out, lse, s);
 }
 
+int d3_attn_delta(const void* o, const void* d_o, float* delta, int n_crops, int N, int D, int H, void* stream) {
+  AttnShape s;
+  int rc = attn_shape(&s, n_crops, N, D, H);
+  if (rc) return rc;
+  if (!o || !d_o || !delta) return set_error(D3_ERR_ARG, "d3_attn_delta: null pointer");
+  const long T = (long)n_crops * N;
+  cudaStream_t st = reinterpret_cast<cudaStream_t>(stream);
+  const long threads = T * (D / 8);
+  if (D == H * 128)
+    attn_delta_kernel<128><<<(int)((threads + 255) / 256), 256, 0, st>>>((const __nv_bfloat16*)o, (const __nv_bfloat16*)d_o,
+                                                                       delta, T, N, D, H);
+  else
+    attn_delta_kernel<64><<<(int)((threads + 255) / 256), 256, 0, st>>>((const __nv_bfloat16*)o, (const __nv_bfloat16*)d_o,
+                                                                      delta, T, N, D, H);
+  D3_CHECK_LAUNCH();
+  return D3_OK;
+}
+
 int d3_attn_bwd(const void* qkv, const void* o, const void* d_o, const float* lse, float* delta_scratch, void* dqkv,
                 int n_crops, int N, int D, int H, const float* rope_sin, const float* rope_cos, int rope_prefix,
                 void* stream) {
@@ -1136,6 +1149,21 @@
   if (rc) return rc;
   if ((rope_sin == nullptr) != (rope_cos == nullptr)) return set_error(D3_ERR_ARG, "d3_attn_bwd: sin/cos tables");
   if (!delta_scratch) return set_error(D3_ERR_ARG, "d3_attn_bwd: delta scratch buffer");
+  dim3 grid;
+  if ((D == H * 128 || s.span > ATTN_BWD_RESIDENT_SPAN) && (rc = tile_grid(s, &grid))) return rc;
+  if ((rc = d3_attn_delta(o, d_o, delta_scratch, n_crops, N, D, H, stream))) return rc;
+  return d3_attn_bwd_given_delta(qkv, d_o, lse, delta_scratch, dqkv, n_crops, N, D, H, rope_sin, rope_cos, rope_prefix,
+                                 stream);
+}
+
+int d3_attn_bwd_given_delta(const void* qkv, const void* d_o, const float* lse, const float* delta_scratch, void* dqkv,
+                            int n_crops, int N, int D, int H, const float* rope_sin, const float* rope_cos,
+                            int rope_prefix, void* stream) {
+  AttnShape s;
+  int rc = attn_shape(&s, n_crops, N, D, H);
+  if (rc) return rc;
+  if ((rope_sin == nullptr) != (rope_cos == nullptr)) return set_error(D3_ERR_ARG, "d3_attn_bwd: sin/cos tables");
+  if (!delta_scratch) return set_error(D3_ERR_ARG, "d3_attn_bwd: delta buffer");
   const bool hd128 = D == H * 128;
   const bool streamed = s.span > ATTN_BWD_RESIDENT_SPAN;
   dim3 grid;
@@ -1143,14 +1171,6 @@
   s.sin_t = rope_sin; s.cos_t = rope_cos; s.prefix = rope_prefix;
   const long T = (long)n_crops * N;
   cudaStream_t st = reinterpret_cast<cudaStream_t>(stream);
-  const long threads = T * (D / 8);
-  if (hd128)
-    attn_delta_kernel<128><<<(int)((threads + 255) / 256), 256, 0, st>>>((const __nv_bfloat16*)o, (const __nv_bfloat16*)d_o,
-                                                                       delta_scratch, T, N, D, H);
-  else
-    attn_delta_kernel<64><<<(int)((threads + 255) / 256), 256, 0, st>>>((const __nv_bfloat16*)o, (const __nv_bfloat16*)d_o,
-                                                                      delta_scratch, T, N, D, H);
-  D3_CHECK_LAUNCH();
   CUtensorMap tqkv, tdo;
   if ((rc = make_map(&tqkv, qkv, T, 3 * D, 3 * D, 128))) return rc;
   if ((rc = make_map(&tdo, d_o, T, D, D, 128))) return rc;
diff --git a/dinov3-jax_b200/csrc/attn_epi.cuh b/dinov3-jax_b200/csrc/attn_epi.cuh
--- /dev/null
+++ b/dinov3-jax_b200/csrc/attn_epi.cuh
@@ -0,0 +1,56 @@
+#pragma once
+#include "ptx.cuh"
+
+namespace d3 {
+
+__device__ __forceinline__ void rope_pair(float a, float b, float c, float s, bool inverse, bool first, float& y_lo,
+                                          float& y_hi) {
+  float bs = __fmul_rn(b, s), as = __fmul_rn(a, s);
+  if (inverse) as = -as; else bs = -bs;
+  y_lo = first ? __fadd_rn(__fmul_rn(a, c), bs) : __fmaf_rn(a, c, bs);
+  y_hi = __fmaf_rn(b, c, as);
+}
+
+__device__ __forceinline__ void rope_rotate2(uint32_t& lo, uint32_t& hi, float2 sn, float2 cs, bool inverse,
+                                             bool first) {
+  const float2 a = unpack_bf16(lo), b = unpack_bf16(hi);
+  float y1a, y1b, y2a, y2b;
+  rope_pair(a.x, b.x, cs.x, sn.x, inverse, first, y1a, y2a);
+  rope_pair(a.y, b.y, cs.y, sn.y, inverse, false, y1b, y2b);
+  lo = pack_bf16(y1a, y1b);
+  hi = pack_bf16(y2a, y2b);
+}
+
+__device__ __forceinline__ void rope_rotate8(uint4& lo, uint4& hi, const float (&sn)[8], const float (&cs)[8],
+                                             bool inverse) {
+  uint32_t lw[4] = {lo.x, lo.y, lo.z, lo.w}, hw[4] = {hi.x, hi.y, hi.z, hi.w};
+#pragma unroll
+  for (int j = 0; j < 4; ++j)
+    rope_rotate2(lw[j], hw[j], make_float2(sn[2 * j], sn[2 * j + 1]), make_float2(cs[2 * j], cs[2 * j + 1]), inverse,
+                 j == 0);
+  lo = make_uint4(lw[0], lw[1], lw[2], lw[3]);
+  hi = make_uint4(hw[0], hw[1], hw[2], hw[3]);
+}
+
+__device__ __forceinline__ float delta_dot8(const uint4& o, const uint4& d) {
+  const float2 a0 = unpack_bf16(o.x), a1 = unpack_bf16(o.y), a2 = unpack_bf16(o.z), a3 = unpack_bf16(o.w);
+  const float2 b0 = unpack_bf16(d.x), b1 = unpack_bf16(d.y), b2 = unpack_bf16(d.z), b3 = unpack_bf16(d.w);
+  float s = __fmaf_rn(a0.x, b0.x, __fmul_rn(a0.y, b0.y));
+  s = __fmaf_rn(a1.x, b1.x, s);
+  s = __fmaf_rn(a1.y, b1.y, s);
+  s = __fmaf_rn(a2.x, b2.x, s);
+  s = __fmaf_rn(a2.y, b2.y, s);
+  s = __fmaf_rn(a3.x, b3.x, s);
+  return __fmaf_rn(a3.y, b3.y, s);
+}
+
+template <int LANES>
+__device__ __forceinline__ float delta_lane_sum(float s) {
+  static_assert(LANES == 8 || LANES == 16, "head_dim 64 or 128");
+  if (LANES == 16) s = __fadd_rn(s, __shfl_xor_sync(0xffffffffu, s, 8));
+  s = __fadd_rn(s, __shfl_xor_sync(0xffffffffu, s, 4));
+  s = __fadd_rn(s, __shfl_xor_sync(0xffffffffu, s, 2));
+  return __fadd_rn(s, __shfl_xor_sync(0xffffffffu, s, 1));
+}
+
+}
diff --git a/dinov3-jax_b200/csrc/d3_internal.h b/dinov3-jax_b200/csrc/d3_internal.h
--- a/dinov3-jax_b200/csrc/d3_internal.h
+++ b/dinov3-jax_b200/csrc/d3_internal.h
@@ -20,6 +20,21 @@
   EP_GELU_ERF = D3_EP_GELU_ERF,
   EP_SLOW = 1 << 30,
   EP_SLABS = 1 << 27,
+  EP_ROPE = 1 << 28,
+  EP_DELTA = 1 << 29,
+};
+
+constexpr int ATTN_EPI_SETS = 4;
+struct AttnEpilogue {
+  struct Set {
+    int row0, rows, N;
+    const float* sin_t;
+    const float* cos_t;
+    float* delta;
+  } set[ATTN_EPI_SETS];
+  int op;
+  int n_sets, D, H, head_dim, prefix;
+  const __nv_bfloat16* o;
 };
 
 struct GemmEpilogue {
@@ -35,6 +50,7 @@
   float* sc_peer[8];
   long long sc_off;
   int sc_shard, sc_world;
+  AttnEpilogue at;
 };
 
 int set_error(int code, const char* msg);
diff --git a/dinov3-jax_b200/csrc/elementwise.cu b/dinov3-jax_b200/csrc/elementwise.cu
--- a/dinov3-jax_b200/csrc/elementwise.cu
+++ b/dinov3-jax_b200/csrc/elementwise.cu
@@ -1,4 +1,5 @@
 #include "ptx.cuh"
+#include "attn_epi.cuh"
 #include "d3_internal.h"
 #include "layernorm.cuh"
 
@@ -562,26 +563,11 @@
     *reinterpret_cast<float4*>(cs) = *reinterpret_cast<const float4*>(cp);
     *reinterpret_cast<float4*>(cs + 4) = *reinterpret_cast<const float4*>(cp + 4);
     __nv_bfloat16* base = qkv + row * (long)(3 * D) + which * D + head * hd + i0;
-    const uint4 lo = *reinterpret_cast<const uint4*>(base);
-    const uint4 hi = *reinterpret_cast<const uint4*>(base + half);
-    const uint32_t lw[4] = {lo.x, lo.y, lo.z, lo.w}, hw[4] = {hi.x, hi.y, hi.z, hi.w};
-    uint32_t ol[4], oh[4];
-#pragma unroll
-    for (int j = 0; j < 4; ++j) {
-      const float2 a = unpack_bf16(lw[j]), b = unpack_bf16(hw[j]);
-      float y1a, y1b, y2a, y2b;
-      if (!inverse) {
-        y1a = a.x * cs[2 * j] - b.x * sn[2 * j];          y2a = b.x * cs[2 * j] + a.x * sn[2 * j];
-        y1b = a.y * cs[2 * j + 1] - b.y * sn[2 * j + 1];  y2b = b.y * cs[2 * j + 1] + a.y * sn[2 * j + 1];
-      } else {
-        y1a = a.x * cs[2 * j] + b.x * sn[2 * j];          y2a = b.x * cs[2 * j] - a.x * sn[2 * j];
-        y1b = a.y * cs[2 * j + 1] + b.y * sn[2 * j + 1];  y2b = b.y * cs[2 * j + 1] - a.y * sn[2 * j + 1];
-      }
-      ol[j] = pack_bf16(y1a, y1b);
-      oh[j] = pack_bf16(y2a, y2b);
-    }
-    *reinterpret_cast<uint4*>(base) = make_uint4(ol[0], ol[1], ol[2], ol[3]);
-    *reinterpret_cast<uint4*>(base + half) = make_uint4(oh[0], oh[1], oh[2], oh[3]);
+    uint4 lo = *reinterpret_cast<const uint4*>(base);
+    uint4 hi = *reinterpret_cast<const uint4*>(base + half);
+    rope_rotate8(lo, hi, sn, cs, inverse != 0);
+    *reinterpret_cast<uint4*>(base) = lo;
+    *reinterpret_cast<uint4*>(base + half) = hi;
   }
 }
 
diff --git a/dinov3-jax_b200/csrc/gemm_tc.cu b/dinov3-jax_b200/csrc/gemm_tc.cu
--- a/dinov3-jax_b200/csrc/gemm_tc.cu
+++ b/dinov3-jax_b200/csrc/gemm_tc.cu
@@ -1,6 +1,7 @@
 #include <cstdlib>
 #include <cstring>
 #include "ptx.cuh"
+#include "attn_epi.cuh"
 #include "d3_internal.h"
 
 namespace d3 {
@@ -11,7 +12,7 @@
 
 constexpr int EPI_RUNTIME = -1;
 constexpr int EPI_FLAGS = EP_BIAS | EP_GELU | EP_STORE_PRE | EP_MUL_DGELU | EP_GAMMA | EP_RESID | EP_OUT_F32 | EP_ACCUM |
-                          EP_SLABS | EP_GELU_ERF;
+                          EP_SLABS | EP_GELU_ERF | EP_ROPE | EP_DELTA;
 
 template <int EF>
 constexpr bool kStaged = EF != EPI_RUNTIME && (EF & (EP_SLABS | EP_ACCUM)) == 0;
@@ -35,7 +36,8 @@
 template <int EF>
 __device__ __forceinline__ float epi_value(const GemmEpilogue& ep, float acc, float bias, float u, float gamma,
                                            float resid, float old, float& pre) {
-  float v = __fmul_rn(acc, ep.alpha);
+  constexpr bool ALPHA_ONE = EF != EPI_RUNTIME && (EF & (EP_ROPE | EP_DELTA)) != 0;
+  float v = ALPHA_ONE ? acc : __fmul_rn(acc, ep.alpha);
   if (epi_has<EF>(ep, EP_BIAS)) v = __fadd_rn(v, bias);
   pre = v;
   if (epi_has<EF>(ep, EP_GELU)) v = gelu_tanh_fast(v);
@@ -121,11 +123,104 @@
   return r * 128 + ((((byte >> 4) ^ r) & 7) << 4) + (byte & 15);
 }
 
+
+__device__ __forceinline__ AttnEpilogue::Set attn_set_of(const AttnEpilogue& at, int row, int& rel, bool& in) {
+  AttnEpilogue::Set s{};
+  in = false;
+  rel = 0;
+#pragma unroll
+  for (int i = 0; i < ATTN_EPI_SETS; ++i)
+    if (i < at.n_sets && row >= at.set[i].row0 && row - at.set[i].row0 < at.set[i].rows) {
+      s = at.set[i];
+      rel = row - at.set[i].row0;
+      in = true;
+    }
+  return s;
+}
+
+template <int MH, int BN>
+struct AttnRegs {
+  float2 sn[MH][2][4], cs[MH][2][4];
+  bool on[MH][2];
+  uint4 o[MH][BN / 64][4];
+};
+
+template <int EF, int MH, int BN>
+__device__ __forceinline__ void attn_prefetch(const AttnEpilogue& at, AttnRegs<MH, BN>& ar, int m0, int n0, int M,
+                                              int N, int t, int r_in, int c_in) {
+  if constexpr ((EF & EP_ROPE) != 0) {
+#pragma unroll
+    for (int mh = 0; mh < MH; ++mh)
+#pragma unroll
+      for (int h = 0; h < 2; ++h) {
+        const int row = m0 + mh * 64 + r_in + 8 * h;
+        int rel;
+        bool in;
+        const AttnEpilogue::Set s = attn_set_of(at, row, rel, in);
+        const int tok = in ? rel % s.N : 0;
+        ar.on[mh][h] = n0 < 2 * at.D && in && row < M && tok >= at.prefix;
+        if (ar.on[mh][h]) {
+          const size_t off = (size_t)(tok - at.prefix) * 64 + c_in;
+#pragma unroll
+          for (int i = 0; i < 4; ++i) {
+            ar.sn[mh][h][i] = __ldg(reinterpret_cast<const float2*>(s.sin_t + off + 8 * i));
+            ar.cs[mh][h][i] = __ldg(reinterpret_cast<const float2*>(s.cos_t + off + 8 * i));
+          }
+        }
+      }
+  }
+  if constexpr ((EF & EP_DELTA) != 0) {
+#pragma unroll
+    for (int mh = 0; mh < MH; ++mh)
+#pragma unroll
+      for (int cb = 0; cb < BN / 64; ++cb)
+#pragma unroll
+        for (int k = 0; k < 4; ++k) {
+          const int row = m0 + mh * 64 + (t >> 3) + 16 * k, col = n0 + cb * 64 + 8 * (t & 7);
+          if (row < M && col < N) ar.o[mh][cb][k] = __ldg(reinterpret_cast<const uint4*>(at.o + (size_t)row * at.D + col));
+        }
+  }
+}
+
+__device__ __forceinline__ void rope_fragment(uint32_t (&pk)[8], const float2 (&sn)[4], const float2 (&cs)[4],
+                                              int c_in) {
+#pragma unroll
+  for (int i = 0; i < 4; ++i) rope_rotate2(pk[i], pk[i + 4], sn[i], cs[i], false, c_in == 0);
+}
+
+__device__ __forceinline__ void delta_rows(const AttnEpilogue& at, float* (&dst)[4], int (&n)[4], int t, int row0,
+                                           int M) {
+#pragma unroll
+  for (int k = 0; k < 4; ++k) {
+    const int row = row0 + (t >> 3) + 16 * k;
+    int rel;
+    bool in;
+    const AttnEpilogue::Set cs = attn_set_of(at, row, rel, in);
+    dst[k] = in && row < M ? cs.delta + (size_t)(rel / cs.N) * at.H * cs.N + rel % cs.N : nullptr;
+    n[k] = cs.N;
+  }
+}
+
+__device__ __forceinline__ void delta_chunk(const uint4 (&o)[4], float* const (&dst)[4], const int (&n)[4],
+                                            const uint8_t* buf, int bar, int t, int row0, int col0, int M) {
+  named_bar_sync(bar, 128);
+  const int c8 = t & 7;
+#pragma unroll
+  for (int k = 0; k < 4; ++k) {
+    const int r = (t >> 3) + 16 * k;
+    float s = 0.f;
+    if (row0 + r < M) s = delta_dot8(o[k], *reinterpret_cast<const uint4*>(buf + sw128(r, 16 * c8)));
+    s = delta_lane_sum<8>(s);
+    if (dst[k] && c8 == 0) dst[k][(size_t)(col0 >> 6) * n[k]] = s;
+  }
+}
+
 template <int MH, int BN, int EF>
 __device__ __forceinline__ void epilogue_tile(const GemmEpilogue& ep, const CUtensorMap* tm_out,
                                               const CUtensorMap* tm_pre, float (&acc)[MH][BN / 2], const float* s_bias,
                                               const float* s_gamma, uint8_t* stg, int& seq, int bar, int t, int m0,
-                                              int n0, int M, int N, size_t slab_row0, int r_in, int c_in) {
+                                              int n0, int M, int N, size_t slab_row0, int r_in, int c_in,
+                                              const AttnRegs<MH, BN>& ar) {
   constexpr bool STAGED = kStaged<EF>;
   constexpr bool F32 = (EF & EP_OUT_F32) != 0;
   constexpr int OUT_BOXES = F32 ? 2 : 1;
@@ -135,7 +230,10 @@
   float* const out_f = reinterpret_cast<float*>(ep.out);
   __nv_bfloat16* const out_h = reinterpret_cast<__nv_bfloat16*>(ep.out);
 #pragma unroll
-  for (int mh = 0; mh < MH; ++mh)
+  for (int mh = 0; mh < MH; ++mh) {
+    float* d_dst[4];
+    int d_n[4];
+    if constexpr ((EF & EP_DELTA) != 0) delta_rows(ep.at, d_dst, d_n, t, m0 + mh * 64, M);
 #pragma unroll
     for (int cb = 0; cb < BN / 64; ++cb) {
       const int row0 = m0 + mh * 64, col0 = n0 + cb * 64;
@@ -167,34 +265,53 @@
       for (int h = 0; h < 2; ++h) {
         const int r = r_in + 8 * h;
         const size_t row = (size_t)row0 + r;
-#pragma unroll
-        for (int i = 0; i < 8; ++i) {
-          const int cl = cb * 64 + 8 * i + c_in;
-          const int n = n0 + cl;
-          const float2 b = epi_has<EF>(ep, EP_BIAS) ? *reinterpret_cast<const float2*>(s_bias + cl) : float2{};
-          const float2 g = epi_has<EF>(ep, EP_GAMMA) ? *reinterpret_cast<const float2*>(s_gamma + cl) : float2{};
-          const float2 u = epi_has<EF>(ep, EP_MUL_DGELU) ? unpack_bf16(xu[h][i]) : float2{};
-          float p0, p1;
-          const float v0 = epi_value<EF>(ep, acc[mh][4 * (cl >> 3) + 2 * h], b.x, u.x, g.x, xr[h][i].x, xo[h][i].x, p0);
-          const float v1 = epi_value<EF>(ep, acc[mh][4 * (cl >> 3) + 2 * h + 1], b.y, u.y, g.y, xr[h][i].y, xo[h][i].y,
-                                         p1);
-          if constexpr (STAGED) {
-            if (epi_has<EF>(ep, EP_STORE_PRE))
-              *reinterpret_cast<uint32_t*>(buf + OUT_BOXES * STG_BOX + sw128(r, 16 * i + 2 * c_in)) = pack_bf16(p0, p1);
-            if constexpr (F32) {
-              *reinterpret_cast<float2*>(buf + (i >> 2) * STG_BOX + sw128(r, 32 * (i & 3) + 4 * c_in)) =
-                  make_float2(v0, v1);
-            } else {
-              *reinterpret_cast<uint32_t*>(buf + sw128(r, 16 * i + 2 * c_in)) = pack_bf16(v0, v1);
+        if constexpr ((EF & EP_ROPE) != 0) {
+          uint32_t pk[8];
+#pragma unroll
+          for (int i = 0; i < 8; ++i) {
+            const int cl = cb * 64 + 8 * i + c_in;
+            const float2 b = epi_has<EF>(ep, EP_BIAS) ? *reinterpret_cast<const float2*>(s_bias + cl) : float2{};
+            float p0, p1;
+            const float v0 = epi_value<EF>(ep, acc[mh][4 * (cl >> 3) + 2 * h], b.x, 0.f, 0.f, 0.f, 0.f, p0);
+            const float v1 = epi_value<EF>(ep, acc[mh][4 * (cl >> 3) + 2 * h + 1], b.y, 0.f, 0.f, 0.f, 0.f, p1);
+            pk[i] = pack_bf16(v0, v1);
+          }
+          if (ar.on[mh][h] && col0 < 2 * ep.at.D) rope_fragment(pk, ar.sn[mh][h], ar.cs[mh][h], c_in);
+#pragma unroll
+          for (int i = 0; i < 8; ++i) *reinterpret_cast<uint32_t*>(buf + sw128(r, 16 * i + 2 * c_in)) = pk[i];
+        } else {
+#pragma unroll
+          for (int i = 0; i < 8; ++i) {
+            const int cl = cb * 64 + 8 * i + c_in;
+            const int n = n0 + cl;
+            const float2 b = epi_has<EF>(ep, EP_BIAS) ? *reinterpret_cast<const float2*>(s_bias + cl) : float2{};
+            const float2 g = epi_has<EF>(ep, EP_GAMMA) ? *reinterpret_cast<const float2*>(s_gamma + cl) : float2{};
+            const float2 u = epi_has<EF>(ep, EP_MUL_DGELU) ? unpack_bf16(xu[h][i]) : float2{};
+            float p0, p1;
+            const float v0 = epi_value<EF>(ep, acc[mh][4 * (cl >> 3) + 2 * h], b.x, u.x, g.x, xr[h][i].x, xo[h][i].x,
+                                           p0);
+            const float v1 = epi_value<EF>(ep, acc[mh][4 * (cl >> 3) + 2 * h + 1], b.y, u.y, g.y, xr[h][i].y,
+                                           xo[h][i].y, p1);
+            if constexpr (STAGED) {
+              if (epi_has<EF>(ep, EP_STORE_PRE))
+                *reinterpret_cast<uint32_t*>(buf + OUT_BOXES * STG_BOX + sw128(r, 16 * i + 2 * c_in)) =
+                    pack_bf16(p0, p1);
+              if constexpr (F32) {
+                *reinterpret_cast<float2*>(buf + (i >> 2) * STG_BOX + sw128(r, 32 * (i & 3) + 4 * c_in)) =
+                    make_float2(v0, v1);
+              } else {
+                *reinterpret_cast<uint32_t*>(buf + sw128(r, 16 * i + 2 * c_in)) = pack_bf16(v0, v1);
+              }
+            } else if (row < (size_t)M && n < N) {
+              if (epi_has<EF>(ep, EP_STORE_PRE)) st_pair(ep.aux_out + row * ep.ld_aux + n, p0, p1, true, true);
+              if constexpr (F32) st_pair(out_f + (slab_row0 + row) * ep.ld_out + n, v0, v1, true, true);
+              else st_pair(out_h + (slab_row0 + row) * ep.ld_out + n, v0, v1, true, true);
             }
-          } else if (row < (size_t)M && n < N) {
-            if (epi_has<EF>(ep, EP_STORE_PRE)) st_pair(ep.aux_out + row * ep.ld_aux + n, p0, p1, true, true);
-            if constexpr (F32) st_pair(out_f + (slab_row0 + row) * ep.ld_out + n, v0, v1, true, true);
-            else st_pair(out_h + (slab_row0 + row) * ep.ld_out + n, v0, v1, true, true);
           }
         }
       }
       if constexpr (STAGED) {
+        if constexpr ((EF & EP_DELTA) != 0) delta_chunk(ar.o[mh][cb], d_dst, d_n, buf, bar, t, row0, col0, M);
         fence_proxy_async_smem();
         named_bar_sync(bar, 128);
         if (t == 0) {
@@ -206,6 +323,7 @@
         ++seq;
       }
     }
+  }
 }
 
 template <int BN, bool STAGED>
@@ -397,6 +515,9 @@
           if constexpr ((EF & EP_GAMMA) != 0) cp_async_4(s_gamma + vt, ep.gamma + wr.n0 + vt);
         }
       }
+      AttnRegs<MH, BN> ar;
+      if constexpr (EF != EPI_RUNTIME && (EF & (EP_ROPE | EP_DELTA)) != 0)
+        attn_prefetch<EF, MH, BN>(ep.at, ar, wr.m0 + (WIDE ? cw * 64 : 0), wr.n0, M, N, t, r_in, c_in);
       if (!WIDE && j > 0) named_bar_sync(1 + cw, 256);
       float acc[MH][BN / 2];
 #pragma unroll
@@ -473,7 +594,7 @@
         epilogue_tile_runtime<BN>(ep, acc, wr.m0, wr.n0, M, N, slab_row0, r_in, c_in);
       } else {
         epilogue_tile<MH, BN, EF>(ep, &tmO, &tmP, acc, s_bias, s_gamma, stg, stg_seq, 5 + cw, t,
-                                  wr.m0 + (WIDE ? cw * 64 : 0), wr.n0, M, N, slab_row0, r_in, c_in);
+                                  wr.m0 + (WIDE ? cw * 64 : 0), wr.n0, M, N, slab_row0, r_in, c_in, ar);
       }
     }
     if (staged && t == 0) tma_store_wait_all();
@@ -561,6 +682,11 @@
     D3_EPI(0, 0, EP_OUT_F32)
     D3_EPI(1, 1, EP_OUT_F32 | EP_SLABS)
     D3_EPI(1, 1, EP_OUT_F32 | EP_ACCUM)
+    if constexpr (BN != 256) {
+      D3_EPI(0, 1, EP_BIAS | EP_ROPE)
+      D3_EPI(0, 1, EP_ROPE)
+      D3_EPI(0, 0, EP_DELTA)
+    }
 #undef D3_EPI
   }
   if constexpr (BN == 256) {
@@ -628,6 +754,14 @@
   if (ep.flags & EP_STORE_PRE) aligned = aligned && ((uintptr_t)ep.aux_out % 16 == 0) && (ep.ld_aux % 8 == 0);
   if (ep.flags & EP_MUL_DGELU) aligned = aligned && ((uintptr_t)ep.aux_in % 16 == 0) && (ep.ld_aux % 8 == 0);
   if (!aligned) ep.flags |= EP_SLOW;
+  bool at_fused = false;
+  if (ep.at.op) {
+    const int f = ep.flags & EPI_FLAGS;
+    at_fused = ep.at.head_dim == 64 && bn != 256 && splits == 1 && ep.alpha == 1.f &&
+               !(ep.flags & (EP_SLOW | EP_SCATTER)) &&
+               (ep.at.op == D3_ATTN_ROPE ? !a_mn && b_mn && (f & ~EP_BIAS) == 0 : !a_mn && !b_mn && f == 0);
+    if (at_fused) ep.flags |= ep.at.op == D3_ATTN_ROPE ? EP_ROPE : EP_DELTA;
+  }
 
   CUtensorMap ta, tb;
   int rc = make_operand_map(&ta, A, M, K, lda, a_mn, 64);
@@ -652,6 +786,16 @@
   if (ws) {
     if (!rc) rc = slab_combine(ws, splits, (long long)M * N, M, N, reinterpret_cast<float*>(out_ep.out), out_ep.ld_out, stream);
     slab_release(ws, stream);
+  }
+  if (ep.at.op && !at_fused) {
+    const AttnEpilogue& at = ep.at;
+    for (int s = 0; s < at.n_sets && !rc; ++s) {
+      const AttnEpilogue::Set& cs = at.set[s];
+      void* rows = reinterpret_cast<__nv_bfloat16*>(ep.out) + (size_t)cs.row0 * ep.ld_out;
+      rc = at.op == D3_ATTN_ROPE
+               ? d3_rope(rows, cs.sin_t, cs.cos_t, cs.rows, cs.N, at.prefix, at.D, at.head_dim, 0, stream)
+               : d3_attn_delta(at.o + (size_t)cs.row0 * at.D, rows, cs.delta, cs.rows / cs.N, cs.N, at.D, at.H, stream);
+    }
   }
   return rc;
 }
diff --git a/dinov3-jax_b200/dinov3_jax/_native.py b/dinov3-jax_b200/dinov3_jax/_native.py
--- a/dinov3-jax_b200/dinov3_jax/_native.py
+++ b/dinov3-jax_b200/dinov3_jax/_native.py
@@ -29,10 +29,25 @@
     ]
 
 
+ATTN_ROPE, ATTN_DELTA = 1, 2
+ATTN_MAX_SETS = 4
+
+
+class CropSet(C.Structure):
+    _fields_ = [("row0", C.c_int), ("n_crops", C.c_int), ("tokens_per_crop", C.c_int),
+                ("sin_t", C.c_void_p), ("cos_t", C.c_void_p), ("delta", C.c_void_p)]
+
+
+class AttnEpilogue(C.Structure):
+    _fields_ = [("op", C.c_int), ("D", C.c_int), ("head_dim", C.c_int), ("prefix", C.c_int), ("o", C.c_void_p),
+                ("n_sets", C.c_int), ("sets", CropSet * ATTN_MAX_SETS)]
+
+
 P, I, LL, F = C.c_void_p, C.c_int, C.c_longlong, C.c_float
 SIGNATURES = {
     "d3_init": [I],
     "d3_gemm_bf16": [P, I, I, P, I, I, I, I, I, C.POINTER(GemmEpilogue), I, I, P],
+    "d3_gemm_bf16_attn": [P, I, I, P, I, I, I, I, I, C.POINTER(GemmEpilogue), C.POINTER(AttnEpilogue), I, P],
     "d3_quant_rows_e4m3": [P, I, I, I, P, I, P, P],
     "d3_quant_cols_e4m3_t": [P, I, I, I, P, I, P, P],
     "d3_gemm_e4m3": [P, I, P, P, I, P, I, I, I, C.POINTER(GemmEpilogue), P],
@@ -48,6 +63,8 @@
     "d3_rope": [P, P, P, LL, I, I, I, I, I, P],
     "d3_attn_fwd": [P, P, P, I, I, I, I, P],
     "d3_attn_bwd": [P, P, P, P, P, P, I, I, I, I, P, P, I, P],
+    "d3_attn_delta": [P, P, P, I, I, I, I, P],
+    "d3_attn_bwd_given_delta": [P, P, P, P, P, I, I, I, I, P, P, I, P],
     "d3_token_rows": [P, P, I, I, I, I, P],
     "d3_gather_rows": [P, P, P, P, I, I, P],
     "d3_scatter_add_rows": [P, I, P, P, I, I, P],
diff --git a/dinov3-jax_b200/dinov3_jax/engine/core.py b/dinov3-jax_b200/dinov3_jax/engine/core.py
--- a/dinov3-jax_b200/dinov3_jax/engine/core.py
+++ b/dinov3-jax_b200/dinov3_jax/engine/core.py
@@ -311,11 +311,13 @@
                 ops.ls_gamma_from_wgrad(w("attn/proj/kernel"), gw("attn/proj/kernel"), v("attn/proj/bias"),
                                         gv("attn/proj/bias"), v("ls1/gamma"), gv("ls1/gamma"))
         on_wstream(2, proj_wgrad)
-        dg(dP, "attn/proj/kernel", self.dO)
+        O = st.b(st.O, i)
+        dg(dP, "attn/proj/kernel", self.dO,
+           delta=(O, D, cfg.head_dim, [(cs.row0, cs.n, cs.N, d) for cs, d in zip(st.sets, self.delta)]))
         for cs, lse, delta in zip(st.sets, st.b(st.LSE, i), self.delta):
             sl = slice(cs.row0, cs.row0 + cs.T)
-            ops.attn_bwd(st.b(st.QKV, i)[sl], st.b(st.O, i)[sl], self.dO[sl], lse, delta, dQKV[sl], cs.n, cs.N, D, H,
-                         rope_sin=cs.sin, rope_cos=cs.cos, rope_prefix=cfg.prefix)
+            ops.attn_bwd(st.b(st.QKV, i)[sl], O[sl], self.dO[sl], lse, delta, dQKV[sl], cs.n, cs.N, D, H,
+                         rope_sin=cs.sin, rope_cos=cs.cos, rope_prefix=cfg.prefix, delta_ready=True)
         wgrad(3, st.b(st.Y, i), dQKV, "attn/qkv/kernel")
 
         def qkv_bias_grad():
diff --git a/dinov3-jax_b200/dinov3_jax/engine/forward.py b/dinov3-jax_b200/dinov3_jax/engine/forward.py
--- a/dinov3-jax_b200/dinov3_jax/engine/forward.py
+++ b/dinov3-jax_b200/dinov3_jax/engine/forward.py
@@ -120,21 +120,36 @@
     return ops.quant_rows(x, net.scratch("q" + which, (R, C), u8, x.device), net.scratch("s" + which, (R,), f32, x.device))
 
 
-def linear(net: Net, x, W, out, **ep):
+def linear(net: Net, x, W, out, rope=None, **ep):
     if not net.fp8:
-        return ops.gemm(x, W, out, b_mn=True, **ep)
+        return ops.gemm(x, W, out, b_mn=True, rope=rope, **ep)
     qx, sx = _e4m3_rows(net, "a", x)
     K, Nn = W.shape
     qw, sw = ops.quant_cols_t(W, net.scratch("qb", (Nn, K), u8, W.device), net.scratch("sb", (Nn,), f32, W.device))
-    return ops.gemm_e4m3(qx, sx, qw, sw, out, **ep)
-
-
-def dgrad(net: Net, dy, W, out, **ep):
+    ops.gemm_e4m3(qx, sx, qw, sw, out, **ep)
+    if rope is not None:
+        D, hd, prefix, sets = rope
+        for row0, n, Ntok, sin_t, cos_t in sets:
+            ops.rope(out[row0: row0 + n * Ntok], sin_t, cos_t, Ntok, prefix, D, hd)
+    return out
+
+
+def dgrad(net: Net, dy, W, out, delta=None, **ep):
     if not net.fp8:
-        return ops.gemm(dy, W, out, **ep)
+        return ops.gemm(dy, W, out, delta=delta, **ep)
     qd, sd = _e4m3_rows(net, "a", dy)
     qw, sw = _e4m3_rows(net, "b", W)
-    return ops.gemm_e4m3(qd, sd, qw, sw, out, **ep)
+    ops.gemm_e4m3(qd, sd, qw, sw, out, **ep)
+    if delta is not None:
+        O, D, hd, sets = delta
+        for row0, n, Ntok, d in sets:
+            rows = slice(row0, row0 + n * Ntok)
+            ops.attn_delta(O[rows], out[rows], d, n, Ntok, D, D // hd)
+    return out
+
+
+def rope_sets(cfg: EngineConfig, st: Stream):
+    return (cfg.embed_dim, cfg.head_dim, cfg.prefix, [(cs.row0, cs.n, cs.N, cs.sin, cs.cos) for cs in st.sets])
 
 
 def embed(net: Net, st: Stream, images, masks_list):
@@ -162,12 +177,11 @@
     Y, QKV, O, Z, Hh = st.b(st.Y, i), st.b(st.QKV, i), st.b(st.O, i), st.b(st.Z, i), st.b(st.Hh, i)
     stats = st.b(st.stats, i) if st.stash else [None] * 4
     ops.layernorm_fwd(X, v("norm1/scale"), v("norm1/bias"), Y, stats[0], stats[1], cfg.ln_eps)
-    lin(Y, "attn/qkv/kernel", QKV, bias=v("attn/qkv/bias") if cfg.qkv_bias else None)
+    lin(Y, "attn/qkv/kernel", QKV, bias=v("attn/qkv/bias") if cfg.qkv_bias else None, rope=rope_sets(cfg, st))
     lses = st.b(st.LSE, i)
     for cs, lse in zip(st.sets, lses):
-        q = QKV[cs.row0: cs.row0 + cs.T]
-        ops.rope(q, cs.sin, cs.cos, cs.N, cfg.prefix, D, cfg.head_dim)
-        ops.attn_fwd(q, O[cs.row0: cs.row0 + cs.T], lse if st.stash else None, cs.n, cs.N, D, H)
+        rows = slice(cs.row0, cs.row0 + cs.T)
+        ops.attn_fwd(QKV[rows], O[rows], lse if st.stash else None, cs.n, cs.N, D, H)
     lin(O, "attn/proj/kernel", Xmid, bias=v("attn/proj/bias"), gamma=v("ls1/gamma"), resid=X,
         store_pre=st.b(st.Pa, i) if st.Pa is not None else None)
     ops.layernorm_fwd(Xmid, v("norm2/scale"), v("norm2/bias"), Z, stats[2], stats[3], cfg.ln_eps)
diff --git a/dinov3-jax_b200/dinov3_jax/ops.py b/dinov3-jax_b200/dinov3_jax/ops.py
--- a/dinov3-jax_b200/dinov3_jax/ops.py
+++ b/dinov3-jax_b200/dinov3_jax/ops.py
@@ -58,12 +58,29 @@
     return ep
 
 
+def _attn_epilogue(op, D, head_dim, prefix, o, sets):
+    assert 1 <= len(sets) <= N.ATTN_MAX_SETS
+    at = N.AttnEpilogue()
+    at.op, at.D, at.head_dim, at.prefix, at.n_sets = op, D, head_dim, prefix, len(sets)
+    at.o = o.data_ptr() if o is not None else None
+    for i, (row0, n, Ntok, sin_t, cos_t, delta) in enumerate(sets):
+        s = at.sets[i]
+        s.row0, s.n_crops, s.tokens_per_crop = row0, n, Ntok
+        if sin_t is not None:
+            assert sin_t.dtype == f32 and cos_t.dtype == f32 and sin_t.is_contiguous() and cos_t.is_contiguous()
+            s.sin_t, s.cos_t = sin_t.data_ptr(), cos_t.data_ptr()
+        if delta is not None:
+            assert delta.dtype == f32 and delta.is_contiguous() and delta.numel() == n * (D // head_dim) * Ntok
+            s.delta = delta.data_ptr()
+    return at
+
+
 def gemm(A: torch.Tensor, B: torch.Tensor, out: torch.Tensor, *, a_mn: bool = False, b_mn: bool = False,
          bias: torch.Tensor | None = None, gelu: bool = False, gelu_erf: bool = False,
          store_pre: torch.Tensor | None = None,
          dgelu_of: torch.Tensor | None = None, gamma: torch.Tensor | None = None,
          resid: torch.Tensor | None = None, accum: bool = False, alpha: float = 1.0, tile_n: int = 0,
-         split_k: int = 0, scatter=None) -> torch.Tensor:
+         split_k: int = 0, scatter=None, rope=None, delta=None) -> torch.Tensor:
     l = N.init()
     assert A.dtype == bf16 and B.dtype == bf16
     M, K = (A.shape[1], A.shape[0]) if a_mn else (A.shape[0], A.shape[1])
@@ -71,11 +88,25 @@
     assert K == Kb, f"contraction mismatch {K} vs {Kb}"
     assert out.shape[0] == M and out.shape[1] == Nn and out.dtype in (bf16, f32)
     ep = _epilogue(out, Nn, bias, gelu, gelu_erf, store_pre, dgelu_of, gamma, resid, accum, alpha, scatter)
+    at = None
+    if rope is not None:
+        assert delta is None
+        D, hd, prefix, sets = rope
+        at = _attn_epilogue(N.ATTN_ROPE, D, hd, prefix, None, [(*s, None) for s in sets])
+    elif delta is not None:
+        O, D, hd, sets = delta
+        assert O.dtype == bf16 and O.is_contiguous() and O.shape == out.shape
+        at = _attn_epilogue(N.ATTN_DELTA, D, hd, 0, O, [(r, n, t, None, None, d) for r, n, t, d in sets])
     if PROFILE is not None:
         e0, e1 = torch.cuda.Event(enable_timing=True), torch.cuda.Event(enable_timing=True)
         e0.record()
-    N.check(l.d3_gemm_bf16(N.ptr(A), _ld(A), int(a_mn), N.ptr(B), _ld(B), int(b_mn), M, Nn, K, C.byref(ep),
-                           int(tile_n), int(split_k), N.stream_ptr()), "d3_gemm_bf16")
+    if at is None:
+        N.check(l.d3_gemm_bf16(N.ptr(A), _ld(A), int(a_mn), N.ptr(B), _ld(B), int(b_mn), M, Nn, K, C.byref(ep),
+                               int(tile_n), int(split_k), N.stream_ptr()), "d3_gemm_bf16")
+    else:
+        assert split_k == 0 and scatter is None
+        N.check(l.d3_gemm_bf16_attn(N.ptr(A), _ld(A), int(a_mn), N.ptr(B), _ld(B), int(b_mn), M, Nn, K, C.byref(ep),
+                                    C.byref(at), int(tile_n), N.stream_ptr()), "d3_gemm_bf16_attn")
     if PROFILE is not None:
         e1.record()
         PROFILE.append(("gemm", 2.0 * M * Nn * K, e0, e1, (M, Nn, K, int(a_mn), int(b_mn))))
@@ -276,11 +307,23 @@
     return o
 
 
-def attn_bwd(qkv, o, do, lse, delta, dqkv, n_crops, Ntok, D, H, rope_sin=None, rope_cos=None, rope_prefix=0):
+def attn_bwd(qkv, o, do, lse, delta, dqkv, n_crops, Ntok, D, H, rope_sin=None, rope_cos=None, rope_prefix=0,
+             delta_ready=False):
     assert all(t.dtype == bf16 and t.is_contiguous() for t in (qkv, o, do, dqkv))
+    if delta_ready:
+        N.check(N.init().d3_attn_bwd_given_delta(_p(qkv), _p(do), _p(lse), _p(delta), _p(dqkv), n_crops, Ntok, D, H,
+                                                 _p(rope_sin), _p(rope_cos), rope_prefix, _s()),
+                "d3_attn_bwd_given_delta")
+        return dqkv
     N.check(N.init().d3_attn_bwd(_p(qkv), _p(o), _p(do), _p(lse), _p(delta), _p(dqkv), n_crops, Ntok, D, H,
                                  _p(rope_sin), _p(rope_cos), rope_prefix, _s()), "d3_attn_bwd")
     return dqkv
+
+
+def attn_delta(o, do, delta, n_crops, Ntok, D, H):
+    assert o.dtype == bf16 and do.dtype == bf16 and o.is_contiguous() and do.is_contiguous() and delta.dtype == f32
+    N.check(N.init().d3_attn_delta(_p(o), _p(do), _p(delta), n_crops, Ntok, D, H, _s()), "d3_attn_delta")
+    return delta
 
 
 def token_rows(mask_indices, rows, count, P, mode, prefix=1):
diff --git a/include/dinov3_b200.h b/include/dinov3_b200.h
--- a/include/dinov3_b200.h
+++ b/include/dinov3_b200.h
@@ -45,6 +45,22 @@
 } d3_gemm_epilogue;
 int d3_gemm_bf16(const void* A, int lda, int a_major, const void* B, int ldb, int b_major, int M, int N, int K,
                  const d3_gemm_epilogue* ep, int tile_n, int split_k, void* stream);
+enum { D3_ATTN_ROPE = 1, D3_ATTN_DELTA = 2 };
+typedef struct {
+  int row0, n_crops, tokens_per_crop;
+  const float* sin_t;
+  const float* cos_t;
+  float* delta;
+} d3_crop_set;
+typedef struct {
+  int op;
+  int D, head_dim, prefix;
+  const void* o;
+  int n_sets;
+  d3_crop_set sets[4];
+} d3_attn_epilogue;
+int d3_gemm_bf16_attn(const void* A, int lda, int a_major, const void* B, int ldb, int b_major, int M, int N, int K,
+                      const d3_gemm_epilogue* ep, const d3_attn_epilogue* at, int tile_n, void* stream);
 
 int d3_quant_rows_e4m3(const void* src_bf16, int ld, int R, int C, void* dst_u8, int ld_dst, float* scale,
                        void* stream);
@@ -90,6 +106,11 @@
 int d3_attn_bwd(const void* qkv_bf16, const void* o_bf16, const void* do_bf16, const float* lse,
                 float* delta_scratch , void* dqkv_bf16 , int n_crops, int N, int D, int H,
                 const float* rope_sin, const float* rope_cos, int rope_prefix, void* stream);
+int d3_attn_delta(const void* o_bf16 , const void* do_bf16, float* delta , int n_crops, int N,
+                  int D, int H, void* stream);
+int d3_attn_bwd_given_delta(const void* qkv_bf16, const void* do_bf16, const float* lse, const float* delta,
+                            void* dqkv_bf16, int n_crops, int N, int D, int H, const float* rope_sin,
+                            const float* rope_cos, int rope_prefix, void* stream);
 
 int d3_token_rows(const long long* mask_indices , int* rows , int count,
                   int P, int prefix ,
```
